# zhen6618/EPRecon

Measured on AMD Instinct MI355X. Metric: fragments_per_sec, higher is better.
Workload: dtype f32

## Files before the change

### eprecon_amd/_lib.py

```python
import ctypes
import os

import torch

_HERE = os.path.dirname(os.path.abspath(__file__))
LIB_PATH = os.environ.get("EPRECON_LIB_PATH") or os.path.join(_HERE, "libeprecon_hip.so")

_c = ctypes
_vp, _i, _i64, _f, _sz = _c.c_void_p, _c.c_int, _c.c_int64, _c.c_float, _c.c_size_t

SIGNATURES = {
    "eprecon_abi_version": (_i, []),
    "eprecon_build_arch": (_c.c_char_p, []),
    "eprecon_back_project_workspace_bytes": (_sz, [_i64, _i, _i, _i, _i, _i, _i]),
    "eprecon_back_project_async": (_i, [_vp, _i64, _vp, _i, _f, _vp, _i, _vp, _i, _i, _i, _i, _i, _i,
                                        _vp, _vp, _vp, _vp, _vp, _vp, _vp, _vp, _sz, _vp]),
    "eprecon_back_project": (_i, [_vp, _i64, _vp, _i, _f, _vp, _i, _vp, _i, _i, _i, _i, _i, _i, _i,
                                  _vp, _vp, _vp, _vp, _vp, _vp, _vp, _vp, _vp, _sz, _vp]),
    "eprecon_profile_gather_kernel": (_c.c_char_p, []),
    "eprecon_hash_capacity": (_c.c_uint32, [_i64]),
    "eprecon_hash_table_bytes": (_sz, [_c.c_uint32]),
    "eprecon_hash_build_async": (_i, [_vp, _i64, _i, _vp, _c.c_uint32, _vp]),
    "eprecon_hash_build_dn_async": (_i, [_vp, _i64, _vp, _i, _vp, _c.c_uint32, _vp]),
    "eprecon_hash_query_async": (_i, [_vp, _c.c_uint32, _vp, _i64, _i, _vp, _vp]),
    "eprecon_hash_status": (_i, [_vp, _vp]),
    "eprecon_unique_workspace_bytes": (_sz, [_i64]),
    "eprecon_unique_coords_async": (_i, [_vp, _i64, _i, _vp, _c.c_uint32, _vp, _vp, _vp, _vp, _sz, _vp]),
    "eprecon_unique_coords_dn_async": (_i, [_vp, _i64, _vp, _i, _vp, _c.c_uint32, _vp, _vp, _vp, _vp, _sz, _vp]),
    "eprecon_unique_hierarchy_dn_async": (_i, [_vp, _i64, _vp, _i, _vp, _vp, _vp, _vp, _vp, _vp, _sz, _vp]),
    "eprecon_point_quantize_dn_async": (_i, [_vp, _i64, _vp, _f, _vp, _vp, _vp]),
    "eprecon_spvcnn_points_dn_async": (_i, [_vp, _i64, _vp, _i, _i, _vp, _i, _f, _vp, _f, _vp, _vp, _vp, _vp, _vp, _vp]),
    "eprecon_gru_stage_capacity": (_i64, [_vp, _i64, _i]),
    "eprecon_gru_stage_workspace_bytes": (_sz, [_i64]),
    "eprecon_gru_stage_begin_async": (_i, [_vp, _vp]),
    "eprecon_gru_stage_commit_async": (_i, [_vp, _vp, _vp, _vp]),
    "eprecon_kernel_map_async": (_i, [_vp, _c.c_uint32, _vp, _i64, _i, _i, _vp, _vp]),
    "eprecon_kernel_map_self_async": (_i, [_vp, _c.c_uint32, _vp, _i64, _i, _vp, _vp]),
    "eprecon_transpose_map_async": (_i, [_vp, _i64, _vp, _i, _vp, _vp]),
    "eprecon_sparse_conv_async": (_i, [_vp, _i64, _i, _vp, _i, _i64, _vp, _i, _i, _vp, _vp, _i, _i, _i, _vp]),
    "eprecon_conv_bn_partial_bytes": (_sz, [_i64, _i]),
    "eprecon_sparse_conv_fused_async": (_i, [_vp, _i64, _i, _vp, _i, _i64, _vp, _i, _i, _vp, _vp, _i, _vp, _i, _i, _i,
                                             _vp, _vp]),
    "eprecon_conv_desc_async": (_i, [_vp, _vp]),
    "eprecon_exclusive_scan_async": (_i, [_vp, _i64, _vp, _vp, _vp, _vp]),
    "eprecon_conv_desc_partial_rows": (_i64, [_vp]),
    "eprecon_bn_acc_words": (_sz, [_i]),
    "eprecon_conv_desc_takes_bn_acc": (_i, [_vp]),
    "eprecon_batchnorm_acc_affine_async": (_i, [_vp, _i, _i, _i, _f, _vp, _vp, _vp]),
    "eprecon_affine_rows_acc_async": (_i, [_vp, _i64, _i, _i, _vp, _i, _i, _f, _i, _vp, _i, _vp]),
    "eprecon_affine_rows_res_async": (_i, [_vp, _i64, _i, _i, _vp, _vp, _vp, _i, _i, _vp, _i, _vp]),
    "eprecon_batchnorm_finalize_affine_async": (_i, [_vp, _i64, _i64, _i, _vp, _vp, _f, _vp, _vp, _vp]),
    "eprecon_affine_rows_async": (_i, [_vp, _i64, _i, _i, _vp, _vp, _i, _vp, _i, _vp]),
    "eprecon_pixel_map_async": (_i, [_i, _i, _i, _i, _vp, _vp]),
    "eprecon_batchnorm_apply_workspace_bytes": (_sz, [_i]),
    "eprecon_batchnorm_apply_partials_async": (_i, [_vp, _i64, _i, _i, _vp, _i64, _i64, _vp, _vp, _f, _vp, _i, _i, _vp, _i,
                                                    _vp, _vp, _vp, _sz, _vp]),
    "eprecon_batchnorm_apply_partials_res_async": (_i, [_vp, _i64, _i, _i, _vp, _i64, _i64, _vp, _vp, _f, _vp, _i, _vp, _vp, _i,
                                                        _vp, _i, _vp, _sz, _vp]),
    "eprecon_batchnorm_workspace_bytes": (_sz, [_i64, _i]),
    "eprecon_batchnorm_train_async": (_i, [_vp, _i64, _i, _i, _vp, _vp, _f, _vp, _i, _i, _vp, _i, _vp, _vp,
                                           _vp, _sz, _vp]),
    "eprecon_rowwise_layernorm_async": (_i, [_vp, _i64, _i, _i, _vp, _i, _vp, _vp, _f, _i, _i, _vp, _i, _vp]),
    "eprecon_init_select_workspace_bytes": (_sz, [_i, _i]),
    "eprecon_init_select_async": (_i, [_vp, _vp, _i64, _f, _i, _i, _i, _vp, _vp, _vp, _sz, _vp]),
    "eprecon_upsample_async": (_i, [_vp, _i, _vp, _i64, _i, _i, _vp, _vp, _vp]),
    "eprecon_aligned_coords_async": (_i, [_vp, _i64, _vp, _i, _f, _vp, _vp, _vp]),
    "eprecon_point_quantize_async": (_i, [_vp, _i64, _f, _vp, _vp, _vp]),
    "eprecon_segment_workspace_bytes": (_sz, [_i64, _i64]),
    "eprecon_segment_lists_async": (_i, [_vp, _i64, _i64, _vp, _vp, _vp, _sz, _vp]),
    "eprecon_segment_mean_async": (_i, [_vp, _i, _vp, _vp, _i64, _i, _vp, _i, _vp]),
    "eprecon_sphash_async": (_i, [_vp, _i64, _vp, _vp]),
    "eprecon_sphash_order_workspace_bytes": (_sz, [_i64]),
    "eprecon_sphash_order_async": (_i, [_vp, _i64, _vp, _vp, _vp, _sz, _vp]),
    "eprecon_remap_index_async": (_i, [_vp, _i64, _vp, _vp, _i64, _vp, _vp]),
    "eprecon_trilinear_map_async": (_i, [_vp, _c.c_uint32, _vp, _i64, _i, _vp, _vp, _vp]),
    "eprecon_devoxelize_async": (_i, [_vp, _i, _vp, _vp, _i64, _i, _vp, _i, _i, _vp]),
    "eprecon_sparse_conv_wgrad_workspace_bytes": (_sz, [_i, _i64, _i, _i]),
    "eprecon_sparse_conv_wgrad_async": (_i, [_vp, _i, _vp, _i, _vp, _i, _i64, _i, _i, _vp, _vp, _sz, _vp]),
    "eprecon_invert_map_async": (_i, [_vp, _i, _i64, _i64, _vp, _vp]),
    "eprecon_devoxelize_backward_async": (_i, [_vp, _i, _vp, _vp, _i64, _i, _i64, _vp, _i, _vp]),
    "eprecon_gather_rows_scaled_async": (_i, [_vp, _i, _vp, _vp, _i64, _i, _vp, _i, _vp]),
    "eprecon_back_project_backward_async": (_i, [_vp, _i64, _vp, _i, _f, _vp, _vp, _i, _i, _i, _i, _i, _vp, _i, _vp, _vp, _vp]),
    "eprecon_back_project_backward_workspace_bytes": (_sz, [_i, _i, _i, _i, _i]),
    "eprecon_back_project_backward_det_async": (_i, [_vp, _i64, _vp, _i, _f, _vp, _vp, _i, _i, _i, _i, _i, _vp, _i, _vp, _vp, _vp, _sz,
                                                     _vp]),
    "eprecon_devoxelize_backward_csr_async": (_i, [_vp, _i, _vp, _vp, _vp, _i64, _i, _vp, _i, _vp]),
    "eprecon_devoxelize_gate_async": (_i, [_vp, _i, _vp, _vp, _i64, _i, _vp, _i, _i, _vp, _i, _vp, _i, _vp, _i, _vp]),
    "eprecon_devoxelize_gate_tail_async": (_i, [_vp, _i, _vp, _vp, _i64, _i, _vp, _i, _i, _vp, _i, _vp, _i, _vp, _i, _vp, _i, _vp, _i,
                                                _i, _vp]),
    "eprecon_fbv_union_workspace_bytes": (_sz, [_i]),
    "eprecon_fbv_union_async": (_i, [_vp, _vp, _i64, _i, _vp, _vp, _i64, _i, _i, _i, _i, _i, _vp, _vp, _vp, _vp, _vp,
                                     _vp, _vp, _sz, _vp]),
    "eprecon_map_set_fragment": (_i, [_vp, _i]),
    "eprecon_map_stamps_async": (_i, [_vp, _vp, _vp, _i, _c.c_int32, _vp]),
    "eprecon_map_select_boundary_async": (_i, [_vp, _vp, _i, _i, _i, _vp, _vp]),
    "eprecon_map_pack_boundary_async": (_i, [_vp, _vp, _i64, _vp]),
    "eprecon_map_merge_boundary": (_i, [_vp, _vp, _i64, _vp, _i, _vp, _vp]),
    "eprecon_map_create": (_i, [_i, _c.POINTER(_vp)]),
    "eprecon_map_destroy": (_i, [_vp]),
    "eprecon_map_reset": (_i, [_vp]),
    "eprecon_map_size": (_i64, [_vp]),
    "eprecon_map_channels": (_i, [_vp]),
    "eprecon_map_export_async": (_i, [_vp, _vp, _vp, _vp]),
    "eprecon_map_import_async": (_i, [_vp, _vp, _vp, _i64, _vp]),
    "eprecon_map_crop_union": (_i, [_vp, _vp, _vp, _i64, _i, _i, _i, _i, _vp, _vp, _vp, _vp, _vp, _vp]),
    "eprecon_map_gather_async": (_i, [_vp, _vp, _i64, _i, _i, _f, _vp, _i, _vp]),
    "eprecon_map_update_async": (_i, [_vp, _vp, _i64, _vp, _i, _vp]),
    "eprecon_map_target_fuse": (_i, [_vp, _vp, _vp, _i, _vp, _vp, _i64, _vp, _vp]),
    "eprecon_gather_rows_async": (_i, [_vp, _i, _vp, _i64, _i, _f, _vp, _i, _vp]),
    "eprecon_tsdf_integrate_async": (_i, [_vp, _vp, _vp, _vp, _f, _vp, _i, _i, _i, _vp, _vp, _f, _f, _i, _vp, _vp]),
    "eprecon_marching_cubes_table": (_i, [_vp]),
    "eprecon_marching_cubes_workspace_bytes": (_sz, [_i, _i, _i]),
    "eprecon_marching_cubes_count": (_i, [_vp, _i, _i, _i, _f, _vp, _vp, _sz, _vp]),
    "eprecon_marching_cubes_emit_async": (_i, [_vp, _i, _i, _i, _f, _vp, _vp, _vp, _vp, _vp, _vp, _vp, _vp, _vp]),
    "eprecon_marching_cubes_count_masked": (_i, [_vp, _vp, _i, _i, _i, _f, _vp, _vp, _sz, _vp]),
    "eprecon_marching_cubes_emit_masked_async": (_i, [_vp, _vp, _i, _i, _i, _f, _vp, _vp, _vp, _vp, _vp, _vp, _vp, _vp, _vp]),
    "eprecon_render_depth_workspace_bytes": (_sz, [_i64]),
    "eprecon_render_depth_async": (_i, [_vp, _i64, _vp, _i64, _vp, _i, _i, _i, _f, _f, _f, _i, _vp, _i64, _vp, _sz, _vp]),
    "eprecon_depth_metrics_workspace_bytes": (_sz, [_i]),
    "eprecon_depth_metrics_async": (_i, [_vp, _vp, _i, _i64, _vp, _vp, _sz, _vp]),
    "eprecon_point_bounds_async": (_i, [_vp, _i64, _vp, _vp, _vp]),
    "eprecon_voxel_down_sample_workspace_bytes": (_sz, [_i64, _i64]),
    "eprecon_voxel_down_sample": (_i, [_vp, _i64, _vp, _c.c_double, _vp, _vp, _vp, _i64, _vp, _sz, _vp]),
    "eprecon_nn_search_workspace_bytes": (_sz, [_i64, _i64]),
    "eprecon_nn_search_async": (_i, [_vp, _i64, _vp, _i64, _vp, _c.c_double, _vp, _vp, _vp, _vp, _sz, _vp]),
    "eprecon_nearest_voxel_async": (_i, [_vp, _c.c_uint32, _vp, _i64, _vp, _i64, _i, _vp, _vp]),
    "eprecon_upsample2x_nhwc_async": (_i, [_vp, _vp, _i, _i, _i, _i, _vp]),
    "eprecon_decoder_keys_async": (_i, [_vp, _i, _vp, _i, _vp, _vp, _vp, _i64, _i, _vp, _vp, _vp]),
    "eprecon_decoder_query_side_async": (_i, [_vp, _vp]),
    "eprecon_panoptic_stats_async": (_i, [_vp, _i64, _vp, _vp, _i, _i64, _vp, _vp, _vp, _vp]),
    "eprecon_panoptic_assign_async": (_i, [_vp, _vp, _vp, _i64, _vp, _vp]),
    "eprecon_masked_attention_workspace_bytes": (_sz, [_i64, _i, _i, _i]),
    "eprecon_masked_attention_async": (_i, [_vp, _i, _i, _vp, _i, _vp, _i, _i64, _vp, _i, _vp, _i64, _i, _i, _i, _f, _vp, _vp, _sz, _vp]),
    "eprecon_profile_enable": (_i, [_i]),
    "eprecon_profile_gather_ms": (_f, []),
    "eprecon_profile_conv_arm": (_i, [_i, _i, _i, _i64]),
    "eprecon_profile_conv_ms": (_f, [_c.POINTER(_i64), _c.POINTER(_c.c_char_p)]),
    "eprecon_profile_conv_pairs": (_i64, []),
    "eprecon_mlp4x_supported": (_i, [_i, _i]),
    "eprecon_spvcnn_forward_workspace_bytes": (_sz, [_vp]),
    "eprecon_spvcnn_forward_async": (_i, [_vp, _vp]),
    "eprecon_spvcnn_geometry_workspace_bytes": (_sz, [_i64, _i64, _i64]),
    "eprecon_spvcnn_geometry_async": (_i, [_vp, _vp]),
    "eprecon_gru_stage_finish_workspace_bytes": (_sz, [_i64, _i64, _i64]),
    "eprecon_gru_stage_finish_async": (_i, [_vp, _vp]),
    "eprecon_bn2d_views_chunks": (_i, [_i64, _i]),
    "eprecon_bn2d_views_workspace_bytes": (_sz, [_i, _i64, _i]),
    "eprecon_bn2d_views_stats_async": (_i, [_vp, _i, _i64, _i, _vp, _vp, _f, _vp, _vp, _sz, _vp]),
    "eprecon_bn2d_views_apply_async": (_i, [_vp, _i, _i64, _i, _vp, _i, _vp, _vp, _vp]),
    "eprecon_dwconv2d_nhwc_async": (_i, [_vp, _i, _i, _i, _i, _vp, _i, _i, _vp, _i, _i, _vp, _vp]),
    "eprecon_mlp4x_async": (_i, [_vp, _vp]),
    "eprecon_profile_conv_executed_pairs": (_i64, []),
    "eprecon_profile_last_conv_kernel": (_c.c_char_p, []),
    "eprecon_profile_mark_async": (_i, [_i, _vp]),
    "eprecon_conv_desc_workspace_bytes": (_sz, [_vp]),
    "eprecon_sparsify_workspace_bytes": (_sz, [_i64]),
    "eprecon_sparsify_async": (_i, [_vp, _i, _f, _vp, _vp, _vp, _i, _vp, _i, _i, _i, _i64, _i, _vp, _vp, _vp, _vp, _vp, _vp, _vp,
                                    _sz, _vp]),
    "eprecon_grid_rank_async": (_i, [_vp, _i64, _i, _i, _i, _i, _vp, _vp]),
    "eprecon_conv_pack_weight_floats": (_sz, [_i, _i, _i]),
    "eprecon_conv_pack_weight_async": (_i, [_vp, _i, _i, _i, _vp, _vp]),
    "eprecon_conv_pack_weight16_floats": (_sz, [_i, _i, _i]),
    "eprecon_conv_pack_weight16_async": (_i, [_vp, _i, _i, _i, _vp, _vp]),
    "eprecon_conv_pack_many_async": (_i, [_vp, _i, _vp]),
    "eprecon_nchw_to_nhwc_async": (_i, [_vp, _vp, _i, _i, _i, _vp]),
    "eprecon_views_to_rows_async": (_i, [_vp, _vp]),
}

EPRECON_OK, EPRECON_EMPTY = 0, 1
ABI_VERSION = 1


class EpreconError(RuntimeError):
    pass


_lib = None


def load():
    global _lib
    if _lib is not None:
        return _lib
    if not os.path.exists(LIB_PATH):
        raise EpreconError(
            f"{LIB_PATH} not found: build it with `python -m eprecon_amd.build` "
            "(hipcc --offload-arch=gfx950). eprecon_amd has no CPU fallback.")
    lib = ctypes.CDLL(LIB_PATH)
    for name, (res, args) in SIGNATURES.items():
        fn = getattr(lib, name)
        fn.restype = res
        fn.argtypes = args
    if lib.eprecon_abi_version() != ABI_VERSION:
        raise EpreconError("libeprecon_hip.so ABI version mismatch; rebuild")
    _lib = lib
    return lib


def check(rc, what):
    if rc == EPRECON_OK:
        return True
    if rc == EPRECON_EMPTY:
        return False
    if rc <= -1000:
        raise EpreconError(f"{what}: HIP error {-(rc + 1000)}")
    raise EpreconError(f"{what}: error {rc} "
                       "(-1 bad argument, -2 workspace too small, -3 unsupported size)")


def ptr(t):
    return None if t is None else t.data_ptr()


_raw_stream = getattr(torch._C, "_cuda_getCurrentRawStream", None)
_raw_device = getattr(torch._C, "_cuda_getDevice", None)


def current_stream():
    if _raw_stream is not None and _raw_device is not None:
        return _raw_stream(_raw_device()) or None
    return torch.cuda.current_stream().cuda_stream or None


class ViewsDesc(ctypes.Structure):
    _fields_ = [("src", (ctypes.c_void_p * 16) * 3), ("dst", ctypes.c_void_p * 3), ("channels", ctypes.c_int32 * 3),
                ("hw", ctypes.c_int32 * 3), ("levels", ctypes.c_int32), ("n_views", ctypes.c_int32)]


class ConvDesc(ctypes.Structure):
    _fields_ = [("x", ctypes.c_void_p), ("n_in", ctypes.c_int64), ("ld_x", ctypes.c_int),
                ("nbr", ctypes.c_void_p), ("kvol", ctypes.c_int), ("n_out", ctypes.c_int64),
                ("weight", ctypes.c_void_p), ("cin", ctypes.c_int), ("cout", ctypes.c_int),
                ("bias", ctypes.c_void_p),
                ("residual", ctypes.c_void_p), ("ld_res", ctypes.c_int),
                ("out", ctypes.c_void_p), ("ld_out", ctypes.c_int),
                ("relu", ctypes.c_int), ("accumulate", ctypes.c_int),
                ("in_scale", ctypes.c_void_p), ("in_shift", ctypes.c_void_p), ("in_relu", ctypes.c_int),
                ("res_scale", ctypes.c_void_p), ("res_shift", ctypes.c_void_p), ("res_relu", ctypes.c_int),
                ("bn_partial", ctypes.c_void_p), ("bn_ld", ctypes.c_int),
                ("ln", ctypes.c_int), ("ln_gamma", ctypes.c_void_p), ("ln_beta", ctypes.c_void_p),
                ("ln_eps", ctypes.c_float), ("ln_post_relu", ctypes.c_int),
                ("img_h", ctypes.c_int), ("img_w", ctypes.c_int), ("img_maps", ctypes.c_int),
                ("vox_rank", ctypes.c_void_p), ("grid_x", ctypes.c_int), ("grid_y", ctypes.c_int), ("grid_z", ctypes.c_int),
                ("packed_weight", ctypes.c_void_p), ("packed_weight16", ctypes.c_void_p),
                ("workspace", ctypes.c_void_p), ("workspace_bytes", ctypes.c_size_t),
                ("bn_acc", ctypes.c_void_p), ("bn_acc_ld", ctypes.c_int), ("bn_acc_c0", ctypes.c_int),
                ("bn_gamma", ctypes.c_void_p), ("bn_beta", ctypes.c_void_p),
                ("in_acc", ctypes.c_void_p), ("in_acc_ld", ctypes.c_int), ("in_acc_c0", ctypes.c_int),
                ("in_eps", ctypes.c_float), ("in_affine_scratch", ctypes.c_void_p)]


class GruStageDesc(ctypes.Structure):
    _fields_ = [("map", ctypes.c_void_p), ("target_map", ctypes.c_void_p),
                ("cur_coords", ctypes.c_void_p), ("cur_feat", ctypes.c_void_p), ("n_cur", ctypes.c_int64), ("ld_cur", ctypes.c_int),
                ("dim", ctypes.c_int), ("interval", ctypes.c_int), ("activity_mode", ctypes.c_int),
                ("rel", ctypes.c_int32 * 3),
                ("tsdf_gt", ctypes.c_void_p), ("occ_gt", ctypes.c_void_p),
                ("origin", ctypes.c_void_p), ("w2ac", ctypes.c_void_p),
                ("voxel_size", ctypes.c_float), ("resolution", ctypes.c_float),
                ("ch_voxel", ctypes.c_int), ("batch_index", ctypes.c_int),
                ("capacity", ctypes.c_int64),
                ("updated", ctypes.c_void_p), ("out_coords", ctypes.c_void_p), ("r_coords", ctypes.c_void_p),
                ("hx_voxel", ctypes.c_void_p), ("hx_image", ctypes.c_void_p), ("tsdf_target", ctypes.c_void_p),
                ("scaled1", ctypes.c_void_p), ("vox1", ctypes.c_void_p), ("inverse1", ctypes.c_void_p), ("uniq1", ctypes.c_void_p),
                ("table1", ctypes.c_void_p),
                ("scaled2", ctypes.c_void_p), ("vox2", ctypes.c_void_p), ("inverse2", ctypes.c_void_p), ("uniq2", ctypes.c_void_p),
                ("table2", ctypes.c_void_p),
                ("table_capacity", ctypes.c_uint32),
                ("counts", ctypes.c_void_p),
                ("workspace", ctypes.c_void_p), ("workspace_bytes", ctypes.c_size_t)]


class DecoderLayerDesc(ctypes.Structure):
    _PTRS_A = ["o_attn", "state_in", "query_pos", "cross_out_wt", "cross_out_b", "cross_ln_g", "cross_ln_b", "self_in_wt", "self_in_b",
               "self_out_wt", "self_out_b", "self_ln_g", "self_ln_b", "ffn1_wt", "ffn1_b", "ffn2_wt", "ffn2_b", "ffn_ln_g", "ffn_ln_b",
               "dec_ln_g", "dec_ln_b", "cls_wt", "cls_b", "m1_wt", "m1_b", "m2_wt", "m2_b", "m3_wt", "m3_b", "next_q_wt", "next_q_b"]
    _PTRS_B = ["state_out", "cls_out", "mask_embed_out", "next_q_out", "workspace"]
    _fields_ = ([(n, ctypes.c_int) for n in ("n_queries", "channels", "n_heads", "ffn_dim", "n_class_logits", "mask_hidden")]
                + [(n, ctypes.c_void_p) for n in _PTRS_A] + [("ln_eps", ctypes.c_float)] + [(n, ctypes.c_void_p) for n in _PTRS_B])


class GruFinishDesc(ctypes.Structure):
    _fields_ = ([(n, ctypes.c_int64) for n in ("n", "m1", "m2")]
                + [(n, ctypes.c_void_p) for n in ("inverse1", "inverse2", "uniq1", "uniq2", "table1", "table2")]
                + [("table_capacity", ctypes.c_uint32)] + [(n, ctypes.c_void_p) for n in ("scaled1", "scaled2")]
                + [("literal", ctypes.c_int)]
                + [(n, ctypes.c_void_p) for n in ("offsets1", "order1", "offsets2", "order2", "nbr1", "nbr2", "idx8_1", "weight8_1",
                                                  "idx8_2", "weight8_2", "perm1", "rank1", "perm2", "rank2", "workspace")]
                + [("workspace_bytes", ctypes.c_size_t)])


class SpvcnnGeometryDesc(ctypes.Structure):
    _fields_ = ([(n, ctypes.c_int64) for n in ("n", "n1", "n2", "n4")]
                + [(n, ctypes.c_void_p) for n in ("scaled", "vox", "inverse1", "coords1", "coords2", "coords4", "parent2", "parent4",
                                                  "table1", "table2", "table4")]
                + [(n, ctypes.c_uint32) for n in ("capacity1", "capacity2", "capacity4")]
                + [(n, ctypes.c_void_p) for n in ("offsets1", "order1", "idx4", "offsets4", "order4", "down12", "up21", "down24", "up42",
                                                  "k1", "k2", "k4", "idx8_1", "weight8_1", "idx8_4", "weight8_4", "workspace")]
                + [("workspace_bytes", ctypes.c_size_t)])


SPVCNN_CONVS = 27


class SpvcnnConv(ctypes.Structure):
    _fields_ = [(n, ctypes.c_void_p) for n in ("weight", "packed_weight", "packed_weight16")] + [(n, ctypes.c_int) for n in ("kvol", "cin", "cout")]


class SpvcnnBn(ctypes.Structure):
    _fields_ = [("gamma", ctypes.c_void_p), ("beta", ctypes.c_void_p), ("eps", ctypes.c_float)]


class SpvcnnForwardDesc(ctypes.Structure):
    _fields_ = ([(n, ctypes.c_int64) for n in ("n", "n1", "n2", "n4")] + [("cin", ctypes.c_int), ("cs", ctypes.c_int * 5)]
                + [("feat", ctypes.c_void_p), ("ld_feat", ctypes.c_int)]
                + [(n, ctypes.c_void_p) for n in ("offsets1", "order1", "offsets4", "order4", "k1", "k2", "k4", "down12", "up21", "down24",
                                                  "up42", "idx8_1", "weight8_1", "idx8_4", "weight8_4")]
                + [("conv", SpvcnnConv * SPVCNN_CONVS), ("bn", SpvcnnBn * SPVCNN_CONVS)]
                + [("out", ctypes.c_void_p), ("ld_out", ctypes.c_int), ("workspace", ctypes.c_void_p), ("workspace_bytes", ctypes.c_size_t)])


class Mlp4xHead(ctypes.Structure):
    _fields_ = ([(n, ctypes.c_void_p) for n in ("w1", "b1", "g1", "be1", "w2", "b2", "g2", "be2", "w3", "b3", "y")]
                + [("ld_y", ctypes.c_int64)])


class Mlp4xDesc(ctypes.Structure):
    _fields_ = [("x", ctypes.c_void_p), ("ld_x", ctypes.c_int64), ("n", ctypes.c_int64), ("channels", ctypes.c_int),
                ("out_channels", ctypes.c_int), ("heads", ctypes.c_int), ("residual", ctypes.c_int), ("eps1", ctypes.c_float),
                ("eps2", ctypes.c_float), ("head", Mlp4xHead * 2)]


SIDE_PAIR, SIDE_BRANCH_A, SIDE_BRANCH_B, SIDE_PANOPTIC, SIDE_EXCHANGE, SIDE_SETUP = range(6)
_SIDE_STREAMS = {}


def side_stream(device, role):
    index = device.index if device.index is not None else torch.cuda.current_device()
    key = (index, role)
    st = _SIDE_STREAMS.get(key)
    if st is None:
        st = _SIDE_STREAMS[key] = torch.cuda.Stream(device=torch.device("cuda", index))
    return st


_WORKSPACES = {}


def workspace(nbytes, device):
    key = (device.type, device.index, current_stream())
    buf = _WORKSPACES.get(key)
    if buf is None or buf.numel() < nbytes:
        buf = torch.empty(int(nbytes * 1.25) + 4096, dtype=torch.uint8, device=device)
        _WORKSPACES[key] = buf
    return buf


_DEFERRED = []
_DEFERRED_LOCK = __import__("threading").Lock()
_DEFERRED_MAX = 64


def defer_check(dev_value, expected, what):
    item = (dev_value, int(expected), what, current_stream())
    evicted = None
    with _DEFERRED_LOCK:
        _DEFERRED.append(item)
        if len(_DEFERRED) > _DEFERRED_MAX:
            evicted = _DEFERRED.pop(0)
    if evicted is not None:
        count_host_read()
        verify_deferred([evicted], evicted[0].to(torch.int32).tolist())


def requeue_deferred(items):
    if items:
        with _DEFERRED_LOCK:
            _DEFERRED[:0] = items


def take_deferred(stream="current"):
    st = current_stream() if stream == "current" else stream
    with _DEFERRED_LOCK:
        out = [it for it in _DEFERRED if stream is None or it[3] == st]
        _DEFERRED[:] = [it for it in _DEFERRED if not (stream is None or it[3] == st)]
    return out


def verify_deferred(items, host_values):
    for (_, expected, what, *_rest), got in zip(items, host_values):
        if int(got) != expected:
            raise EpreconError(f"{what}: expected {expected}, the device reports {int(got)} (EPRECON_ERR_ARG)")


def read_counts(counts):
    count_host_read()
    pending = take_deferred()
    flat = counts.reshape(-1)
    if pending:
        host = torch.cat([flat] + [t.reshape(1).to(flat.dtype) for t, *_ in pending]).tolist()
        verify_deferred(pending, host[flat.numel():])
        return host[:flat.numel()]
# ... 49 lines not shown
```

### eprecon_amd/csrc/conv_common.hpp

```cpp
#pragma once
#include "common.hpp"

namespace epconv {

struct ConvParams {
    const float *x;
    const int32_t *nbr;
    const float *w;
    const float *bias;
    float *out;
    int n_out, K, Cin, Cout, ld_x, ld_out;
    int64_t x_bytes;
    int relu;
    int accumulate;
    const float *res;
    int ld_res;
    float *bn_partial;
    int bn_ld;
    const float *in_scale, *in_shift;
    int in_relu;
    const float *res_scale, *res_shift;
    int res_relu;
    int ln;
    const float *ln_gamma, *ln_beta;
    float ln_eps;
    int ln_post_relu;
    int img_h, img_w, img_maps;
    int flex_partial;
    const int32_t *vox_rank;
    int gx, gy, gz;
    const float *wq;
    const float *wq16;
    int debug;
    int splitk_pipe;
    void *ws;
    size_t ws_bytes;
    long long *bn_acc;
    int bn_acc_ld, bn_acc_c0;
    const float *bn_gamma, *bn_beta;
    const long long *in_acc;
    int in_acc_ld, in_acc_c0;
    float in_eps;
};

constexpr int kBnCopies = 8, kBnWords = 7;
#ifndef EP_BN_ABL
#define EP_BN_ABL 0
#endif

__device__ __forceinline__ void bn_limbs(double x, long long &l0, long long &l1, long long &l2)
{
    const double v = x * 1099511627776.0;
    const double hi = floor(v * (1.0 / 1099511627776.0));
    l0 = (long long)(v - hi * 1099511627776.0);
    const long long h = (long long)hi;
    l1 = h & ((1ll << 40) - 1);
    l2 = h >> 40;
}

__device__ __forceinline__ void bn_acc_add(long long *acc, int ld, int c, int copy, float n, float mean, float m2)
{
    if (n <= 0.0f || (EP_BN_ABL & 1)) return;
    unsigned long long *a = reinterpret_cast<unsigned long long *>(acc) + ((size_t)copy * ld + c) * kBnWords;
    const double dn = (double)n, dm = (double)mean;
    long long l0, l1, l2;
    bn_limbs(dn * dm, l0, l1, l2);
    atomicAdd(a + 0, (unsigned long long)l0);
    if (EP_BN_ABL & 4) return;
    atomicAdd(a + 1, (unsigned long long)l1); atomicAdd(a + 2, (unsigned long long)l2);
    bn_limbs((double)m2 + dn * dm * dm, l0, l1, l2);
    atomicAdd(a + 3, (unsigned long long)l0); atomicAdd(a + 4, (unsigned long long)l1); atomicAdd(a + 5, (unsigned long long)l2);
    atomicAdd(a + 6, (unsigned long long)(long long)n);
}

__device__ __forceinline__ void bn_acc_affine(const long long *acc, int ld, int c, float eps, float &scale, float &shift)
{
    if (EP_BN_ABL & 2) { scale = 1.0f; shift = 0.0f; return; }
    long long w[kBnWords] = {0, 0, 0, 0, 0, 0, 0};
#pragma unroll 1
    for (int k = 0; k < kBnCopies; ++k) {
        const long long *a = acc + ((size_t)k * ld + c) * kBnWords;
#pragma unroll
        for (int j = 0; j < kBnWords; ++j) w[j] += a[j];
    }
    const double two40 = 1099511627776.0;
    const double s1 = ((double)w[2] * two40 + (double)w[1]) + (double)w[0] * (1.0 / two40);
    const double s2 = ((double)w[5] * two40 + (double)w[4]) + (double)w[3] * (1.0 / two40);
    const double n = (double)w[6];
    const float *gb = reinterpret_cast<const float *>(acc + (size_t)kBnCopies * ld * kBnWords);
    const double mean = n > 0.0 ? s1 / n : 0.0;
    double var = n > 0.0 ? s2 / n - mean * mean : 0.0;
    if (var < 0.0) var = 0.0;
    const float sc = gb[c] / sqrtf((float)var + eps);
    scale = sc;
    shift = gb[ld + c] - (float)mean * sc;
}

template <int THREADS, bool ACC = true>
__device__ __forceinline__ void stage_in_affine(const ConvParams &p, float *sAff, int cpad, int tid)
{
    if (!p.in_scale) return;
    for (int c = tid; c < cpad; c += THREADS) {
        float sc = 0.0f, sh = 0.0f;
        if (c < p.Cin) {
            if (ACC && p.in_acc) bn_acc_affine(p.in_acc, p.in_acc_ld, p.in_acc_c0 + c, p.in_eps, sc, sh);
            else { sc = p.in_scale[c]; sh = p.in_shift[c]; }
        }
        sAff[c] = sc;
        sAff[cpad + c] = sh;
    }
}

__device__ __forceinline__ void bn_acc_publish(const ConvParams &p, int col, int copy, bool first, float n, float mean, float m2)
{
    bn_acc_add(p.bn_acc, p.bn_acc_ld, p.bn_acc_c0 + col, copy & (kBnCopies - 1), n, mean, m2);
    if (first) {
        float *gb = reinterpret_cast<float *>(p.bn_acc + (size_t)kBnCopies * p.bn_acc_ld * kBnWords);
        gb[p.bn_acc_c0 + col] = p.bn_gamma ? p.bn_gamma[col] : 1.0f;
        gb[p.bn_acc_ld + p.bn_acc_c0 + col] = p.bn_beta ? p.bn_beta[col] : 0.0f;
    }
}

constexpr int kWaves = 4;
typedef float f32x4 __attribute__((ext_vector_type(4)));
typedef unsigned int u32x4 __attribute__((ext_vector_type(4)));

__device__ __forceinline__ void chan_merge(float &n_a, float &mean_a, float &m2_a, float n_b, float mean_b, float m2_b)
{
    if (n_b == 0.0f) return;
    if (n_a == 0.0f) {
        n_a = n_b; mean_a = mean_b; m2_a = m2_b;
        return;
    }
    const float n = n_a + n_b;
    const float d = mean_b - mean_a;
    mean_a = mean_a + d * (n_b / n);
    m2_a = m2_a + m2_b + d * d * (n_a * n_b / n);
    n_a = n;
}

__device__ __forceinline__ void bn_partial_store(const ConvParams &p, int row, int col, float n, float mean, float m2)
{
    const size_t plane = (size_t)p.Cout * p.bn_ld;
    float *dst = p.bn_partial + (size_t)col * p.bn_ld + row;
    dst[0] = n; dst[plane] = mean; dst[2 * plane] = m2;
}

template <int CT, bool ACC = false, int NW = kWaves>
__device__ __forceinline__ void tile16_epilogue(const ConvParams &p, const f32x4 (&acc)[CT], const int (&orow)[4], float *sStat,
                                                int partial_row)
{
    const int tid = threadIdx.x;
    const int lane = tid & 63, wave = tid >> 6;
    const int l16 = lane & 15, q = lane >> 4;
    float v[CT][4];
    bool colok[CT];
#pragma unroll
    for (int t = 0; t < CT; ++t) {
        const int col = 16 * t + l16;
        colok[t] = col < p.Cout;
        const float b = (p.bias && colok[t]) ? p.bias[col] : 0.0f;
        const float rs = (p.res_scale && colok[t]) ? p.res_scale[col] : 1.0f;
        const float rb = (p.res_scale && colok[t]) ? p.res_shift[col] : 0.0f;
#pragma unroll
        for (int j = 0; j < 4; ++j) {
            float val = 0.0f;
            if (colok[t] && orow[j] >= 0) {
                val = acc[t][j] + b;
                if (p.relu) val = fmaxf(val, 0.0f);
                if (p.res) {
                    float rv = p.res[(size_t)orow[j] * p.ld_res + col];
                    if (p.res_scale) {
                        rv = fmaf(rv, rs, rb);
                        if (p.res_relu) rv = fmaxf(rv, 0.0f);
                    }
                    val += rv;
                }
            }
            v[t][j] = val;
        }
    }
    if (p.ln) {
        const float inv_c = 1.0f / (float)p.Cout;
#pragma unroll
        for (int j = 0; j < 4; ++j) {
            float sum = 0.0f;
#pragma unroll
            for (int t = 0; t < CT; ++t) sum += v[t][j];
#pragma unroll
            for (int m = 8; m > 0; m >>= 1) sum += __shfl_xor(sum, m);
            const float mean = sum * inv_c;
            float sq = 0.0f;
#pragma unroll
            for (int t = 0; t < CT; ++t) {
                const float d = colok[t] ? v[t][j] - mean : 0.0f;
                v[t][j] = d;
                sq = fmaf(d, d, sq);
            }
#pragma unroll
            for (int m = 8; m > 0; m >>= 1) sq += __shfl_xor(sq, m);
            const float inv = 1.0f / sqrtf(sq * inv_c + p.ln_eps);
#pragma unroll
            for (int t = 0; t < CT; ++t) {
                const int col = 16 * t + l16;
                float y = fmaf(v[t][j] * inv, (p.ln_gamma && colok[t]) ? p.ln_gamma[col] : 1.0f, (p.ln_beta && colok[t]) ? p.ln_beta[col] : 0.0f);
                if (p.ln_post_relu) y = fmaxf(y, 0.0f);
                v[t][j] = y;
            }
        }
    }
#pragma unroll
    for (int t = 0; t < CT; ++t)
#pragma unroll
        for (int j = 0; j < 4; ++j)
            if (colok[t] && orow[j] >= 0) p.out[(size_t)orow[j] * p.ld_out + 16 * t + l16] = v[t][j];
    if (p.bn_partial || (ACC && p.bn_acc)) {
#pragma unroll
        for (int t = 0; t < CT; ++t) {
            float n = 0.0f, sum = 0.0f;
#pragma unroll
            for (int j = 0; j < 4; ++j)
                if (orow[j] >= 0) { n += 1.0f; sum += v[t][j]; }
            float mean = n > 0.0f ? sum / n : 0.0f, m2 = 0.0f;
#pragma unroll
            for (int j = 0; j < 4; ++j)
                if (orow[j] >= 0) { const float d = v[t][j] - mean; m2 = fmaf(d, d, m2); }
#pragma unroll
            for (int m = 16; m < 64; m <<= 1) {
                const float on = __shfl_xor(n, m), om = __shfl_xor(mean, m), oq = __shfl_xor(m2, m);
                const bool lower = (lane & m) == 0;
                float a_n = lower ? n : on, a_mean = lower ? mean : om, a_m2 = lower ? m2 : oq;
                chan_merge(a_n, a_mean, a_m2, lower ? on : n, lower ? om : mean, lower ? oq : m2);
                n = a_n; mean = a_mean; m2 = a_m2;
            }
            if (q == 0) {
                float *d = sStat + (wave * 3) * 16 * CT + 16 * t + l16;
                d[0] = n; d[16 * CT] = mean; d[2 * 16 * CT] = m2;
            }
        }
        __syncthreads();
        if (tid < 16 * CT && tid < p.Cout) {
            float a_n = 0.0f, a_mean = 0.0f, a_m2 = 0.0f;
#pragma unroll
            for (int w = 0; w < NW; ++w)
                chan_merge(a_n, a_mean, a_m2, sStat[(w * 3) * 16 * CT + tid], sStat[(w * 3 + 1) * 16 * CT + tid], sStat[(w * 3 + 2) * 16 * CT + tid]);
            if (p.bn_partial) bn_partial_store(p, partial_row, tid, a_n, a_mean, a_m2);
            if (ACC && p.bn_acc) bn_acc_publish(p, tid, partial_row, partial_row == 0, a_n, a_mean, a_m2);
        }
    }
}

bool direct16_ok(const ConvParams &p);
constexpr int kDirectRows = 128;
int launch_direct16(const ConvParams &p, hipStream_t st);
int direct16_partial_block_rows(const ConvParams &p);

constexpr int kT2MinRows = 40000;
bool tile2d16_ok(const ConvParams &p);
int64_t tile2d16_partial_rows(const ConvParams &p);
int launch_tile2d16(const ConvParams &p, hipStream_t st);

constexpr int kT2ShortMaxRows = 20000;
bool tile2d_short_list(const ConvParams &p);
bool tile2d_short_ok(const ConvParams &p);
int64_t tile2d_short_partial_rows(const ConvParams &p);
int launch_tile2d_short(const ConvParams &p, hipStream_t st);


}
```

### eprecon_amd/csrc/grid_ops.hip

```cpp
#include "common.hpp"

namespace {
using namespace ep;

constexpr int kSelThreads = 1024;

__global__ __launch_bounds__(256) void init_mark_kernel(const float *logit, const int4 *coords, int n, float thr,
                                                        int batch, int D, int cell, unsigned char *marks)
{
    const int i = blockIdx.x * 256 + threadIdx.x;
    if (i >= n) return;
    const int4 c = coords[i];
    if (c.x < 0 || c.x >= batch) return;
    const float sig = 1.0f / (1.0f + expf(-logit[i]));
    if (sig > thr) {
        const int x = c.y / cell, y = c.z / cell, z = c.w / cell;
        if (x >= 0 && x < D && y >= 0 && y < D && z >= 0 && z < D) marks[(size_t)c.x * D * D * D + (x * D + y) * D + z] = 1;
    }
}

__device__ __forceinline__ uint32_t box_columns(const uint32_t *vol, int D, int x, int y, bool erode, uint32_t zmask)
{
    uint32_t r = erode ? zmask : 0u;
    for (int dx = -1; dx <= 1; ++dx)
// ... 36 lines not shown
#pragma unroll
        for (int d = 1; d < kWave; d <<= 1) {
            const int t = __shfl_up(s, d);
            if (lane >= d) s += t;
        }
        if (lane == kWave - 1) sWave[wid] = s;
        __syncthreads();
        int off = written + s - mine, tot = 0;
        for (int k = 0; k < kSelThreads / kWave; ++k) {
            const int c = sWave[k];
            if (k < wid) off += c;
            tot += c;
        }
        uint32_t bits = fin;
        while (bits) {
            const int z = __ffs(bits) - 1;
            bits &= bits - 1;
            out_coords[off++] = make_int4(b, x * out_scale, y * out_scale, z * out_scale);
        }
        if (tid == 0) n_out_dev[1 + b] = tot;
        written += tot;
        __syncthreads();
    }
    if (tid == 0) n_out_dev[0] = written;
}

__global__ __launch_bounds__(256) void upsample_coords_kernel(const int4 *coords, int n, int interval,
                                                              int4 *up)
{
    const int e = blockIdx.x * 256 + threadIdx.x;
    if (e >= n * 8) return;
    const int i = e >> 3, k = e & 7;
    const int dx = (0xB2 >> k) & 1;
    const int dy = (0xD4 >> k) & 1;
    const int dz = (0xE8 >> k) & 1;
    int4 c = coords[i];
    c.y += dx * interval;
    c.z += dy * interval;
    c.w += dz * interval;
    up[e] = c;
}

__global__ __launch_bounds__(256) void upsample_feat_kernel(const float *feat, int n, int C, int ld,
                                                            float *up)
{
    const size_t e = (size_t)blockIdx.x * 256 + threadIdx.x;
    const size_t total = (size_t)n * 8 * C;
    if (e >= total) return;
    const int c = (int)(e % C);
    const size_t row = e / C;
    up[e] = feat[(row >> 3) * ld + c];
}

}

extern "C" {

size_t eprecon_init_select_workspace_bytes(int batch, int dim)
{
    return align_up((size_t)batch * dim * dim * dim, 256);
}

int eprecon_init_select_async(const float *logit, const int32_t *coords, int64_t n, float threshold,
                              int batch, int dim, int cell, int32_t *out_coords, int32_t *n_out_dev,
                              void *workspace, size_t workspace_bytes, void *stream)
{
    if (n < 0 || batch <= 0 || dim <= 0 || dim > 32 || cell <= 0 || !out_coords || !n_out_dev || !workspace ||
        (n > 0 && (!logit || !coords)))
        return EPRECON_ERR_ARG;
    if (workspace_bytes < eprecon_init_select_workspace_bytes(batch, dim)) return EPRECON_ERR_WORKSPACE;
    hipStream_t st = (hipStream_t)stream;
    const int cells = dim * dim * dim;
    unsigned char *marks = reinterpret_cast<unsigned char *>(workspace);
    EP_HIP_CHECK(hipMemsetAsync(marks, 0, (size_t)batch * cells, st));
    if (n > 0) {
        hipLaunchKernelGGL(init_mark_kernel, dim3((unsigned)ceil_div(n, 256)), dim3(256), 0, st, logit,
                           reinterpret_cast<const int4 *>(coords), (int)n, threshold, batch, dim, cell, marks);
        EP_LAUNCH_CHECK();
    }
    hipLaunchKernelGGL(init_select_kernel, dim3(1), dim3(kSelThreads), 0, st, (const unsigned char *)marks, batch,
                       dim, cell, reinterpret_cast<int4 *>(out_coords), n_out_dev);
    EP_LAUNCH_CHECK();
    return EPRECON_OK;
}

int eprecon_upsample_async(const float *feat, int ld_feat, const int32_t *coords, int64_t n, int channels,
                           int interval, float *up_feat, int32_t *up_coords, void *stream)
{
    if (n < 0 || channels < 0 || interval <= 0 || (n > 0 && (!coords || (!up_coords && channels == 0)))) return EPRECON_ERR_ARG;
    if (n == 0) return EPRECON_OK;
    hipStream_t st = (hipStream_t)stream;
    if (up_coords) {
        hipLaunchKernelGGL(upsample_coords_kernel, dim3((unsigned)ceil_div(n * 8, 256)), dim3(256), 0, st,
                           reinterpret_cast<const int4 *>(coords), (int)n, interval,
                           reinterpret_cast<int4 *>(up_coords));
        EP_LAUNCH_CHECK();
    }
    if (channels > 0) {
        if (!feat || !up_feat || ld_feat < channels) return EPRECON_ERR_ARG;
        const size_t total = (size_t)n * 8 * channels;
        hipLaunchKernelGGL(upsample_feat_kernel, dim3((unsigned)ceil_div((int64_t)total, 256)), dim3(256), 0,
                           st, feat, (int)n, channels, ld_feat, up_feat);
        EP_LAUNCH_CHECK();
    }
    return EPRECON_OK;
}

}

namespace {
__global__ __launch_bounds__(256) void upsample2x_nhwc_kernel(const float4 *in, float4 *out, int n, int h, int w,
                                                              int c4)
{
    const size_t e = (size_t)blockIdx.x * 256 + threadIdx.x;
    const size_t total = (size_t)n * 4 * h * w * c4;
    if (e >= total) return;
    const int c = (int)(e % c4);
    size_t r = e / c4;
    const int ox = (int)(r % (2 * w));
    r /= 2 * w;
    const int oy = (int)(r % (2 * h));
    const int img = (int)(r / (2 * h));
    const float sx = fmaxf(((float)ox + 0.5f) * 0.5f - 0.5f, 0.0f);
    const float sy = fmaxf(((float)oy + 0.5f) * 0.5f - 0.5f, 0.0f);
    const int x0 = (int)sx, y0 = (int)sy;
    const int x1 = min(x0 + 1, w - 1), y1 = min(y0 + 1, h - 1);
    const float lx = sx - (float)x0, ly = sy - (float)y0;
    const float4 *base = in + (size_t)img * h * w * c4;
    const float4 a = base[((size_t)y0 * w + x0) * c4 + c], b = base[((size_t)y0 * w + x1) * c4 + c];
    const float4 d = base[((size_t)y1 * w + x0) * c4 + c], f = base[((size_t)y1 * w + x1) * c4 + c];
    const float w00 = (1.0f - ly) * (1.0f - lx), w01 = (1.0f - ly) * lx, w10 = ly * (1.0f - lx), w11 = ly * lx;
    float4 o;
    o.x = w00 * a.x + w01 * b.x + w10 * d.x + w11 * f.x;
    o.y = w00 * a.y + w01 * b.y + w10 * d.y + w11 * f.y;
    o.z = w00 * a.z + w01 * b.z + w10 * d.z + w11 * f.z;
    o.w = w00 * a.w + w01 * b.w + w10 * d.w + w11 * f.w;
    out[e] = o;
}
}

extern "C" int eprecon_upsample2x_nhwc_async(const float *in, float *out, int n, int h, int w, int channels,
                                             void *stream)
{
    if (!in || !out || n <= 0 || h <= 0 || w <= 0 || channels <= 0 || channels % 4) return EPRECON_ERR_ARG;
    const size_t total = (size_t)n * 4 * h * w * (channels / 4);
    hipLaunchKernelGGL(upsample2x_nhwc_kernel, dim3((unsigned)ceil_div((int64_t)total, 256)), dim3(256), 0,
                       (hipStream_t)stream, reinterpret_cast<const float4 *>(in), reinterpret_cast<float4 *>(out), n, h,
                       w, channels / 4);
    EP_LAUNCH_CHECK();
    return EPRECON_OK;
}

namespace {
constexpr int kSpTile = 256;
constexpr int kSpMaxBatch = 32;

__global__ __launch_bounds__(kSpTile) void sparsify_count_kernel(const float *occ, int ld_occ, float thr, const unsigned char *tgt,
                                                                const int4 *coords, int n, int batch, int *tile_tot, int *counts)
{
    const int row = blockIdx.x * kSpTile + threadIdx.x;
    const bool keep = row < n && occ[(size_t)row * ld_occ] > thr;
    const unsigned long long m = __ballot(keep);
    __shared__ int sTot[kSpTile / 64];
    __shared__ int sCnt[2 * kSpMaxBatch];
    if (threadIdx.x < 2 * kSpMaxBatch) sCnt[threadIdx.x] = 0;
    if ((threadIdx.x & 63) == 0) sTot[threadIdx.x >> 6] = __popcll(m);
    __syncthreads();
    const int b = keep ? coords[row].x : -1;
    const bool t = keep && (!tgt || tgt[row]);
    for (int bb = 0; bb < batch; ++bb) {
        const unsigned long long mb = __ballot(b == bb), mt = __ballot(b == bb && t);
        if ((threadIdx.x & 63) == 0 && mb) {
            atomicAdd(&sCnt[bb], __popcll(mb));
            if (mt) atomicAdd(&sCnt[kSpMaxBatch + bb], __popcll(mt));
        }
    }
    __syncthreads();
    if (threadIdx.x < batch) {
        if (sCnt[threadIdx.x]) atomicAdd(counts + 1 + threadIdx.x, sCnt[threadIdx.x]);
        if (sCnt[kSpMaxBatch + threadIdx.x]) atomicAdd(counts + 1 + batch + threadIdx.x, sCnt[kSpMaxBatch + threadIdx.x]);
    }
    if (threadIdx.x == 0) tile_tot[blockIdx.x] = sTot[0] + sTot[1] + sTot[2] + sTot[3];
}

__global__ __launch_bounds__(1024) void sparsify_scan_kernel(int *tile_tot, int ntiles, int *counts)
{
    __shared__ int sWave[16];
    __shared__ int sCarry;
    const int tid = threadIdx.x, lane = tid & 63, wave = tid >> 6;
    if (tid == 0) sCarry = 0;
    __syncthreads();
    for (int base = 0; base < ntiles; base += 1024) {
        const int i = base + tid;
        const int v = i < ntiles ? tile_tot[i] : 0;
        int incl = v;
#pragma unroll
        for (int d = 1; d < 64; d <<= 1) {
            const int o = __shfl_up(incl, d);
            if (lane >= d) incl += o;
        }
        if (lane == 63) sWave[wave] = incl;
        __syncthreads();
        int woff = 0;
        for (int w = 0; w < wave; ++w) woff += sWave[w];
        const int carry = sCarry;
        if (i < ntiles) tile_tot[i] = carry + woff + incl - v;
        __syncthreads();
        if (tid == 1023) sCarry = carry + woff + incl;
        __syncthreads();
    }
    if (tid == 0) counts[0] = sCarry;
}

__global__ __launch_bounds__(kSpTile) void sparsify_compact_kernel(const float *occ, int ld_occ, float thr, const int4 *coords,
                                                                  const float *tsdf, int ld_tsdf, const float *feat, int ld_feat,
                                                                  int c_all, int c_feat, int n, const int *tile_off, int4 *out_coords,
                                                                  float *out_tsdf, float *out_occ, float *out_all, float *out_feat)
{
    const int row = blockIdx.x * kSpTile + threadIdx.x;
    const int lane = threadIdx.x & 63, wave = threadIdx.x >> 6;
    const float o = row < n ? occ[(size_t)row * ld_occ] : 0.0f;
    const bool keep = row < n && o > thr;
    const unsigned long long m = __ballot(keep);
    __shared__ int sTot[kSpTile / 64];
    if (lane == 0) sTot[wave] = __popcll(m);
    __syncthreads();
    int base = tile_off[blockIdx.x];
    for (int w = 0; w < wave; ++w) base += sTot[w];
    const int dst = base + __popcll(m & ((1ull << lane) - 1ull));
    const float t = keep ? tsdf[(size_t)row * ld_tsdf] : 0.0f;
    if (keep) {
        out_coords[dst] = coords[row];
        out_tsdf[dst] = t;
        out_occ[dst] = o;
        out_feat[(size_t)dst * (c_feat + 2) + c_feat] = t;
        out_feat[(size_t)dst * (c_feat + 2) + c_feat + 1] = o;
    }
    unsigned long long rest = m;
    while (rest) {
        const int l = __ffsll((long long)rest) - 1;
        rest &= rest - 1;
        const int src = blockIdx.x * kSpTile + wave * 64 + l;
        const int d = __shfl(dst, l);
        for (int c = lane; c < c_all; c += 64) {
            const float v = feat[(size_t)src * ld_feat + c];
            out_all[(size_t)d * c_all + c] = v;
            if (c < c_feat) out_feat[(size_t)d * (c_feat + 2) + c] = v;
        }
    }
}
}

extern "C" size_t eprecon_sparsify_workspace_bytes(int64_t n)
{
    return align_up((size_t)(ceil_div(n > 0 ? n : 1, (int64_t)kSpTile) + 1) * sizeof(int), 256);
}

extern "C" int eprecon_sparsify_async(const float *occ, int ld_occ, float threshold, const unsigned char *target,
                                      const int32_t *coords, const float *tsdf, int ld_tsdf, const float *feat_all, int ld_feat,
                                      int c_all, int c_feat, int64_t n, int batch, int32_t *out_coords, float *out_tsdf,
                                      float *out_occ, float *out_all, float *out_feat, int32_t *counts, void *workspace,
                                      size_t workspace_bytes, void *stream)
{
    if (n < 0 || n > 0x7fffffff || batch <= 0 || batch > kSpMaxBatch || c_all <= 0 || c_feat < 0 || c_feat > c_all || ld_occ < 1 || ld_tsdf < 1 ||
        ld_feat < c_all || !counts || !workspace || (n > 0 && (!occ || !coords || !tsdf || !feat_all || !out_coords || !out_tsdf ||
                                                               !out_occ || !out_all || !out_feat)))
        return EPRECON_ERR_ARG;
    if (workspace_bytes < eprecon_sparsify_workspace_bytes(n)) return EPRECON_ERR_WORKSPACE;
    hipStream_t st = (hipStream_t)stream;
    EP_HIP_CHECK(hipMemsetAsync(counts, 0, (size_t)(1 + 2 * batch) * sizeof(int32_t), st));
    if (n == 0) return EPRECON_OK;
    int *tile_tot = reinterpret_cast<int *>(workspace);
    const int ntiles = (int)ceil_div(n, (int64_t)kSpTile);
    hipLaunchKernelGGL(sparsify_count_kernel, dim3(ntiles), dim3(kSpTile), 0, st, occ, ld_occ, threshold, target,
                       reinterpret_cast<const int4 *>(coords), (int)n, batch, tile_tot, counts);
    EP_LAUNCH_CHECK();
    hipLaunchKernelGGL(sparsify_scan_kernel, dim3(1), dim3(1024), 0, st, tile_tot, ntiles, counts);
    EP_LAUNCH_CHECK();
    hipLaunchKernelGGL(sparsify_compact_kernel, dim3(ntiles), dim3(kSpTile), 0, st, occ, ld_occ, threshold,
                       reinterpret_cast<const int4 *>(coords), tsdf, ld_tsdf, feat_all, ld_feat, c_all, c_feat, (int)n,
                       (const int *)tile_tot, reinterpret_cast<int4 *>(out_coords), out_tsdf, out_occ, out_all, out_feat);
    EP_LAUNCH_CHECK();
    return EPRECON_OK;
}
```

### eprecon_amd/csrc/sparse_conv.hip

```cpp
#include <stdio.h>
#include <stdlib.h>
#include <string.h>

#include "common.hpp"
#include "conv_common.hpp"

namespace {
using namespace ep;
using namespace epconv;

typedef float f32x16 __attribute__((ext_vector_type(16)));


template <int TN>
__device__ __forceinline__ void stage_weights(float *dst, const float *w, int row0, int row_end, int stride,
                                              int ncols, int rows, int tid)
{
    const int total = rows * TN;
    if (stride == TN && ncols >= TN && (reinterpret_cast<uintptr_t>(w) & 15) == 0) {
        const float4 *src = reinterpret_cast<const float4 *>(w + (size_t)row0 * stride);
        float4 *d4 = reinterpret_cast<float4 *>(dst);
        const int valid4 = max(0, min(rows, row_end - row0)) * (TN / 4);
#pragma unroll 4
        for (int e = tid; e < total / 4; e += 256) d4[e] = e < valid4 ? src[min(e, max(valid4 - 1, 0))] : make_float4(0.f, 0.f, 0.f, 0.f);
// ... 1725 lines not shown
    }
    conv_epilogue<1>(p, acc, LinearRows{(int)blockIdx.x * kWideRows + wave * 32, p.n_out}, 32 * t, r32, half, wave, sStat,
                     (int)blockIdx.x, (int)gridDim.y);
}

size_t wide_workspace_bytes(const ConvParams &p)
{
    const int ntt = (p.Cout + 31) / 32;
    return (size_t)wide_splits(p.n_out) * (size_t)ceil_div(p.n_out, kWideRows) * kWaves * ntt * 1024 * sizeof(float);
}

bool wide_shape_ok(const ConvParams &p)
{
    const char *e = getenv("EPRECON_CONV_WIDEK");
    if (e && e[0] == '0') return false;
    if (p.K != 27 || !p.nbr || !p.wq || (reinterpret_cast<uintptr_t>(p.wq) & 15) != 0) return false;
    if (p.Cin < 96 || p.Cin % 4 != 0 || p.Cout <= 64 || p.Cout > 128) return false;
    if (p.ld_x % 4 != 0 || (reinterpret_cast<uintptr_t>(p.x) & 15) != 0) return false;
    if (p.in_scale && ((reinterpret_cast<uintptr_t>(p.in_scale) & 15) != 0 || (reinterpret_cast<uintptr_t>(p.in_shift) & 15) != 0))
        return false;
    if (p.accumulate || p.ln) return false;
    return p.n_out >= 4096 && p.n_out <= 40000;
}
bool wide_ok(const ConvParams &p) { return wide_shape_ok(p) && p.ws && p.ws_bytes >= wide_workspace_bytes(p); }

template <int NTT>
int launch_wide_t(const ConvParams &p, hipStream_t st)
{
    const int nsplit = wide_splits(p.n_out);
    const int blocks = (int)ceil_div(p.n_out, kWideRows);
    const int kmax = (p.K + nsplit - 1) / nsplit + 1;
    const size_t lds = (size_t)2 * kWideSlabF4 * sizeof(float4) + (size_t)kmax * kWideRows * sizeof(int) +
                       (size_t)2 * ((p.Cin + 3) & ~3) * sizeof(float) + 16;
    float *partial = reinterpret_cast<float *>(p.ws);
    hipLaunchKernelGGL((spconv_wide_kernel<NTT>), dim3((unsigned)blocks, (unsigned)nsplit), dim3(256), lds, st, p, nsplit, partial);
    EP_LAUNCH_CHECK();
    const size_t lds2 = (size_t)max(kWaves * 3 * 32 * NTT, 3 * 256) * sizeof(float);
    hipLaunchKernelGGL((spconv_wide_reduce_kernel<NTT>), dim3((unsigned)blocks, (unsigned)NTT), dim3(256), lds2, st, p, nsplit, (const float *)partial);
    EP_LAUNCH_CHECK();
    return EPRECON_OK;
}
int launch_wide(const ConvParams &p, hipStream_t st) { return (p.Cout + 31) / 32 == 3 ? launch_wide_t<3>(p, st) : launch_wide_t<4>(p, st); }

bool splitk_ok(const ConvParams &p)
{
    const char *e = getenv("EPRECON_CONV_SPLITK");
    if ((e && e[0] == '0') || p.accumulate) return false;
    if (p.bn_partial && !p.flex_partial) return false;
    const int nt_full = (p.Cout + 31) / 32;
    if (p.ln && nt_full > 1) return false;
    const int cin_pad = (p.Cin + 7) / 8 * 8;
    const int64_t wg128 = ceil_div(p.n_out, kRowsPerBlock) * nt_full;
    const int stages = p.K * ((p.Cin + 31) / 32);
    constexpr int max_wg = 256, narrow_wg = 256;
    if (cin_pad <= 64) return wg128 <= narrow_wg && stages >= 8;
    return wg128 <= max_wg && stages >= 8;
}

struct ConvProf {
    bool armed = false, recorded = false;
    int K = 0, cin = 0, cout = 0;
    int64_t min_rows = 0, rows = 0;
    const char *kernel = "";
    hipEvent_t start = nullptr, stop = nullptr;
    unsigned long long *pairs_dev = nullptr;
} g_conv_prof;

__global__ void count_map_pairs_kernel(const int32_t *nbr, size_t total, unsigned long long *out)
{
    unsigned long long c = 0;
    for (size_t e = (size_t)blockIdx.x * blockDim.x + threadIdx.x; e < total; e += (size_t)gridDim.x * blockDim.x) c += nbr[e] >= 0;
    for (int m = 32; m > 0; m >>= 1) c += __shfl_xor(c, m);
    if ((threadIdx.x & 63) == 0 && c) atomicAdd(out, c);
}
__global__ void count_grid_pairs_kernel(const int32_t *rank, int gx, int gy, int gz, unsigned long long *out)
{
    unsigned long long c = 0;
    const int total = gx * gy * gz;
    for (int e = blockIdx.x * blockDim.x + threadIdx.x; e < total; e += gridDim.x * blockDim.x) {
        if (rank[e] < 0) continue;
        const int z = e % gz, y = (e / gz) % gy, x = e / (gz * gy);
        for (int k = 0; k < 27; ++k) {
            const int xx = x + k % 3 - 1, yy = y + (k / 3) % 3 - 1, zz = z + k / 9 - 1;
            if (xx >= 0 && xx < gx && yy >= 0 && yy < gy && zz >= 0 && zz < gz) c += rank[(xx * gy + yy) * gz + zz] >= 0;
        }
    }
    for (int m = 32; m > 0; m >>= 1) c += __shfl_xor(c, m);
    if ((threadIdx.x & 63) == 0 && c) atomicAdd(out, c);
}
__global__ void count_map_groups_kernel(const int32_t *nbr, int n, int K, unsigned long long *out)
{
    const int groups = (n + 31) / 32;
    unsigned long long c = 0;
    for (int e = blockIdx.x * blockDim.x + threadIdx.x; e < K * groups; e += gridDim.x * blockDim.x) {
        const int k = e / groups, g = e - k * groups;
        const int rows = min(32, n - 32 * g);
        bool any = false;
        for (int i = 0; i < rows; ++i) any |= nbr[(size_t)k * n + 32 * g + i] >= 0;
        if (any) c += rows;
    }
    for (int m = 32; m > 0; m >>= 1) c += __shfl_xor(c, m);
    if ((threadIdx.x & 63) == 0 && c) atomicAdd(out, c);
}
const char *g_last_conv_kernel = "";

int conv_dispatch_inner(ConvParams &p, int64_t n_in, hipStream_t st);

int conv_dispatch(ConvParams &p, int64_t n_in, hipStream_t st)
{
    ConvProf &g = g_conv_prof;
    const bool hit = g.armed && p.K == g.K && p.Cin == g.cin && p.Cout == g.cout && p.n_out >= g.min_rows;
    static FILE *const layer_log = getenv("EPRECON_CONV_LOG") ? fopen(getenv("EPRECON_CONV_LOG"), "a") : nullptr;
    if (layer_log) {
        const int rc = conv_dispatch_inner(p, n_in, st);
        fprintf(layer_log, "%d %d %d %d %s ln=%d stats=%d acc=%d\n", p.n_out, p.K, p.Cin, p.Cout, g_last_conv_kernel, p.ln ? 1 : 0,
                p.bn_partial ? 1 : 0, p.accumulate ? 1 : 0);
        fflush(layer_log);
        return rc;
    }
    if (!hit) return conv_dispatch_inner(p, n_in, st);
    EP_HIP_CHECK(hipEventRecord(g.start, st));
    const int rc = conv_dispatch_inner(p, n_in, st);
    EP_HIP_CHECK(hipEventRecord(g.stop, st));
    g.armed = false;
    g.recorded = rc == EPRECON_OK;
    g.rows = p.n_out;
    g.kernel = g_last_conv_kernel;
    if (g.pairs_dev) {
        EP_HIP_CHECK(hipMemsetAsync(g.pairs_dev, 0, 2 * sizeof(unsigned long long), st));
        bool narrow;
        if (conv3d_tile_ok(p, &narrow))
            hipLaunchKernelGGL(count_grid_pairs_kernel, dim3(256), dim3(256), 0, st, p.vox_rank, p.gx, p.gy, p.gz, g.pairs_dev);
        else if (p.nbr) {
            hipLaunchKernelGGL(count_map_pairs_kernel, dim3(256), dim3(256), 0, st, p.nbr, (size_t)p.K * p.n_out, g.pairs_dev);
            if (!strcmp(g.kernel, "spconv_direct16_kernel"))
                hipLaunchKernelGGL(count_map_groups_kernel, dim3(256), dim3(256), 0, st, p.nbr, p.n_out, p.K, g.pairs_dev + 1);
        } else
            EP_HIP_CHECK(hipMemcpyAsync(g.pairs_dev, &g.rows, sizeof(unsigned long long), hipMemcpyHostToDevice, st));
        EP_LAUNCH_CHECK();
    }
    return rc;
}

int conv_dispatch_inner(ConvParams &p, int64_t n_in, hipStream_t st)
{
    {
        const int kind = conv3d_kind(p);
        if (kind != kD3None) {
            g_last_conv_kernel = kind == kD3Narrow ? "conv3d_tile_narrow_kernel" : "conv3d_tile16_kernel";
            return kind == kD3Tile16 ? launch_conv3d_16(p, st) : launch_conv3d_single_column(p, st);
        }
        if (!p.nbr && p.K != 1) return EPRECON_ERR_ARG;
    }
    if (tile2d16_ok(p)) {
        g_last_conv_kernel = "conv2d_tile16_kernel";
        return launch_tile2d16(p, st);
    }
    if (tile2d_short_ok(p)) {
        g_last_conv_kernel = "conv2d_tile_short_kernel";
        return launch_tile2d_short(p, st);
    }
    const bool direct2d = p.K == 9 && direct16_ok(p) && !tile2d_short_list(p);
    if (!direct2d) {
        int nt, nch;
        int64_t blocks;
        if (conv2d_tile_ok(p, &nt, &nch, &blocks)) {
            g_last_conv_kernel = "conv2d_tile_kernel";
            switch (nch) {
                case 1: return launch_conv2d_tile<1>(p, st);
                case 2: return launch_conv2d_tile<2>(p, st);
                case 3: return launch_conv2d_tile<3>(p, st);
                case 4: return launch_conv2d_tile<4>(p, st);
                default: return launch_conv2d_tile<5>(p, st);
            }
        }
    }
    const bool vec4 = (p.ld_x % 4 == 0) && ((reinterpret_cast<uintptr_t>(p.x) & 15) == 0) &&
                      (p.Cin % 4 == 0 || p.ld_x >= ((p.Cin + 3) & ~3));
    const int nblk = (int)ceil_div(p.n_out, kRowsPerBlock);
    const int nt_full = (p.Cout + 31) / 32;
    if (p.ln && (nt_full > 4 || p.bn_partial || p.accumulate)) return EPRECON_ERR_UNSUPPORTED;
    if (wide_ok(p)) {
        g_last_conv_kernel = "spconv_wide_kernel";
        return launch_wide(p, st);
    }
    if (!direct2d && splitk_ok(p)) {
        g_last_conv_kernel = "spconv_splitk_kernel";
        return vec4 ? launch_splitk_v<true>(p, st) : launch_splitk_v<false>(p, st);
    }
    if (direct16_ok(p) && !tile2d_short_list(p)) {
        g_last_conv_kernel = "spconv_direct16_kernel";
        return launch_direct16(p, st);
    }
    const bool split = nblk < 256 && nt_full > 1 && !p.ln;
    const int cin_pad = (p.Cin + 7) / 8 * 8;
    if (cin_pad <= 64 && (p.Cout <= 64 || split)) {
        g_last_conv_kernel = "spconv_resident_kernel";
        return (nt_full == 1 || split) ? launch_resident<1>(p, vec4, cin_pad, st) : launch_resident<2>(p, vec4, cin_pad, st);
    }
    if (cin_pad > 64 && vec4 && (p.K == 27 || p.K == 8) && !(p.ln && nt_full > 2)) {
        g_last_conv_kernel = "spconv_resident_kernel(wide)";
        const bool two = nt_full >= 2 && (p.ln || (int64_t)nblk * ((nt_full + 1) / 2) >= 256);
        return two ? launch_resident<2>(p, vec4, cin_pad, st) : launch_resident<1>(p, vec4, cin_pad, st);
    }
    g_last_conv_kernel = "spconv_mfma_kernel";
    if (nt_full == 1 || split) return launch_conv<1>(p, vec4, st);
    if (nt_full == 2) return launch_conv<2>(p, vec4, st);
    if (nt_full == 3) return launch_conv<3>(p, vec4, st);
    return launch_conv<4>(p, vec4, st);
}

}

__global__ void profile_mark_kernel() {}
extern "C" int eprecon_profile_mark_async(int id, void *stream)
{
    hipStream_t st = static_cast<hipStream_t>(stream);
    hipLaunchKernelGGL(profile_mark_kernel, dim3((unsigned)id + 1), dim3(64), 0, st);
    EP_LAUNCH_CHECK();
    return EPRECON_OK;
}

extern "C" int eprecon_profile_conv_arm(int kvol, int cin, int cout, int64_t min_rows)
{
    ConvProf &g = g_conv_prof;
    if (!g.start) {
        EP_HIP_CHECK(hipEventCreate(&g.start));
        EP_HIP_CHECK(hipEventCreate(&g.stop));
        EP_HIP_CHECK(hipMalloc(&g.pairs_dev, 2 * sizeof(unsigned long long)));
    }
    g.K = kvol; g.cin = cin; g.cout = cout; g.min_rows = min_rows;
    g.armed = true;
    g.recorded = false;
    return EPRECON_OK;
}

extern "C" float eprecon_profile_conv_ms(int64_t *rows_out, const char **kernel_out)
{
    ConvProf &g = g_conv_prof;
    if (!g.recorded || hipEventSynchronize(g.stop) != hipSuccess) return -1.0f;
    float ms = -1.0f;
    if (hipEventElapsedTime(&ms, g.start, g.stop) != hipSuccess) return -1.0f;
    if (rows_out) *rows_out = g.rows;
    if (kernel_out) *kernel_out = g.kernel;
    return ms;
}

extern "C" const char *eprecon_profile_last_conv_kernel(void) { return g_last_conv_kernel; }

extern "C" int64_t eprecon_profile_conv_pairs(void)
{
    ConvProf &g = g_conv_prof;
    if (!g.recorded || !g.pairs_dev || hipEventSynchronize(g.stop) != hipSuccess) return -1;
    unsigned long long v = 0;
    if (hipMemcpy(&v, g.pairs_dev, sizeof(v), hipMemcpyDeviceToHost) != hipSuccess) return -1;
    return (int64_t)v;
}

extern "C" int64_t eprecon_profile_conv_executed_pairs(void)
{
    ConvProf &g = g_conv_prof;
    if (!g.recorded || !g.pairs_dev || hipEventSynchronize(g.stop) != hipSuccess) return -1;
    unsigned long long v = 0;
    if (hipMemcpy(&v, g.pairs_dev + 1, sizeof(v), hipMemcpyDeviceToHost) != hipSuccess) return -1;
    return (int64_t)v;
}

extern "C" size_t eprecon_conv_pack_weight_floats(int kvol, int cin, int cout)
{
    if (kvol <= 0 || cin <= 0 || cout <= 0) return 0;
    int nt, ncb;
    d3_columns(cout, &nt, &ncb);
    return (size_t)ncb * kvol * ((cin + 7) / 8) * 2 * nt * 32 * 4;
}

extern "C" int eprecon_conv_pack_weight_async(const float *weight, int kvol, int cin, int cout, float *packed, void *stream)
{
    if (!weight || !packed || kvol <= 0 || cin <= 0 || cout <= 0) return EPRECON_ERR_ARG;
    int nt, ncb;
    d3_columns(cout, &nt, &ncb);
    const size_t total = eprecon_conv_pack_weight_floats(kvol, cin, cout);
    hipLaunchKernelGGL(pack_weights_kernel, dim3((unsigned)min((size_t)1024, (total + 255) / 256)), dim3(256), 0, (hipStream_t)stream,
                       weight, kvol, cin, cout, (cin + 7) / 8, nt, ncb, packed);
    EP_LAUNCH_CHECK();
    return EPRECON_OK;
}

extern "C" size_t eprecon_conv_pack_weight16_floats(int kvol, int cin, int cout)
{
    if (kvol <= 0 || cin <= 0 || cout <= 0 || cout > 80) return 0;
    const int rem = cout - 16 * ((cout + 15) / 16 - 1);
    return (size_t)kvol * ((cin + 15) / 16) * ((cout + 15) / 16) * 256 + (rem <= 8 ? (size_t)kvol * ((cin + 15) / 16) * 128 : 0);
}

extern "C" int eprecon_conv_pack_weight16_async(const float *weight, int kvol, int cin, int cout, float *packed, void *stream)
{
    if (!weight || !packed || kvol <= 0 || cin <= 0 || cout <= 0 || cout > 80) return EPRECON_ERR_ARG;
    const size_t total = eprecon_conv_pack_weight16_floats(kvol, cin, cout);
    hipLaunchKernelGGL(pack_weights16_kernel, dim3((unsigned)min((size_t)1024, (total + 255) / 256)), dim3(256), 0, (hipStream_t)stream,
                       weight, kvol, cin, cout, (cin + 15) / 16, (cout + 15) / 16, packed);
    EP_LAUNCH_CHECK();
    return EPRECON_OK;
}

extern "C" int eprecon_conv_pack_many_async(const eprecon_pack_job *jobs_dev, int njobs, void *stream)
{
    if (njobs < 0 || (njobs > 0 && !jobs_dev) || njobs > 65535) return EPRECON_ERR_ARG;
    if (njobs == 0) return EPRECON_OK;
    hipLaunchKernelGGL(pack_many_kernel, dim3(32, (unsigned)njobs), dim3(256), 0, (hipStream_t)stream, jobs_dev);
    EP_LAUNCH_CHECK();
    return EPRECON_OK;
}

extern "C" size_t eprecon_conv_bn_partial_bytes(int64_t n_out, int cout)
{
    return (size_t)ep::ceil_div(n_out > 0 ? n_out : 1, (int64_t)128) * 3 * (size_t)(cout > 0 ? cout : 1) * sizeof(float);
}

static int conv_check_and_run(ConvParams &p, int64_t n_in, int64_t n_out, void *stream)
{
    if (!p.x || !p.w || !p.out || n_in < 0 || n_out < 0 || p.K <= 0 || p.K > 64 || p.Cin <= 0 || p.Cout <= 0 ||
        p.ld_x < p.Cin || p.ld_out < p.Cout || (p.res && p.ld_res < p.Cout))
        return EPRECON_ERR_ARG;
    if (!p.nbr && !p.vox_rank && p.K != 1) return EPRECON_ERR_ARG;
    if (!p.nbr && n_in != n_out) return EPRECON_ERR_ARG;
    if ((p.in_scale == nullptr) != (p.in_shift == nullptr) || (p.res_scale == nullptr) != (p.res_shift == nullptr))
        return EPRECON_ERR_ARG;
    if (p.Cout > 4096 || n_out > 0x7fffffff) return EPRECON_ERR_UNSUPPORTED;
    if (n_out == 0) return EPRECON_OK;
    p.n_out = (int)n_out;
    p.x_bytes = n_in > 0 ? ((n_in - 1) * (int64_t)p.ld_x + ((p.Cin + 3) & ~3)) * 4 : 0;
    return conv_dispatch(p, n_in, (hipStream_t)stream);
}

static void params_from_desc(ConvParams &p, const eprecon_conv_desc *d)
{
    p.x = d->x; p.nbr = d->nbr; p.w = d->weight; p.bias = d->bias; p.out = d->out;
    p.K = d->kvol; p.Cin = d->cin; p.Cout = d->cout; p.ld_x = d->ld_x; p.ld_out = d->ld_out;
    p.relu = d->relu; p.accumulate = d->accumulate;
    p.res = d->residual; p.ld_res = d->ld_res; p.bn_partial = d->bn_partial; p.bn_ld = d->bn_ld;
    p.in_scale = d->in_scale; p.in_shift = d->in_shift; p.in_relu = d->in_relu;
    p.res_scale = d->res_scale; p.res_shift = d->res_shift; p.res_relu = d->res_relu;
    p.ln = d->ln; p.ln_gamma = d->ln_gamma; p.ln_beta = d->ln_beta; p.ln_eps = d->ln_eps;
    p.ln_post_relu = d->ln_post_relu;
    p.img_h = d->img_h; p.img_w = d->img_w; p.img_maps = d->img_maps;
    p.vox_rank = d->vox_rank; p.gx = d->grid_x; p.gy = d->grid_y; p.gz = d->grid_z; p.wq = d->packed_weight;
    p.wq16 = d->packed_weight16;
    p.ws = d->workspace; p.ws_bytes = d->workspace_bytes;
    p.flex_partial = 1;
    p.bn_acc = d->bn_acc; p.bn_acc_ld = d->bn_acc_ld; p.bn_acc_c0 = d->bn_acc_c0; p.bn_gamma = d->bn_gamma; p.bn_beta = d->bn_beta;
    p.in_acc = d->in_acc; p.in_acc_ld = d->in_acc_ld; p.in_acc_c0 = d->in_acc_c0; p.in_eps = d->in_eps;
}

extern "C" int eprecon_batchnorm_acc_affine_async(const long long *acc, int acc_ld, int acc_c0, int channels, float eps,
                                                  float *scale_out, float *shift_out, void *stream);

static bool bn_acc_family(const ConvParams &p) { return conv3d_kind(p) == 0; }

extern "C" size_t eprecon_bn_acc_words(int ld)
{
    return ld > 0 ? (size_t)epconv::kBnCopies * ld * epconv::kBnWords + (size_t)(2 * ld + 1) / 2 : 0;
}

extern "C" int eprecon_conv_desc_takes_bn_acc(const eprecon_conv_desc *d)
{
    if (!d || d->n_out <= 0) return 0;
    ConvParams p = {};
    params_from_desc(p, d);
    p.n_out = (int)d->n_out;
    return !p.ln && !p.accumulate && bn_acc_family(p) ? 1 : 0;
}

extern "C" int64_t eprecon_conv_desc_partial_rows(const eprecon_conv_desc *d);

extern "C" int eprecon_conv_desc_async(const eprecon_conv_desc *d, void *stream)
{
    if (!d) return EPRECON_ERR_ARG;
    ConvParams p = {};
    params_from_desc(p, d);
    p.n_out = (int)(d->n_out > 0 && d->n_out <= 0x7fffffff ? d->n_out : 0);
    if (p.bn_partial) {
        const int64_t rows = eprecon_conv_desc_partial_rows(d);
        if (p.bn_ld == 0) p.bn_ld = (int)(rows > 0 ? rows : 1);
        if (p.bn_ld < rows) return EPRECON_ERR_ARG;
    }
    if (p.bn_acc && (p.bn_acc_ld <= 0 || p.bn_acc_c0 < 0 || p.bn_acc_c0 + p.Cout > p.bn_acc_ld || p.ln || p.accumulate || !bn_acc_family(p)))
        return EPRECON_ERR_ARG;
    if (p.in_acc) {
        if (p.in_scale || p.in_shift || p.in_acc_ld <= 0 || p.in_acc_c0 < 0 || p.in_acc_c0 + p.Cin > p.in_acc_ld) return EPRECON_ERR_ARG;
        if (bn_acc_family(p)) {
            p.in_scale = p.in_shift = reinterpret_cast<const float *>(p.in_acc);
        } else {
            if (!d->in_affine_scratch) return EPRECON_ERR_ARG;
            const int rc = eprecon_batchnorm_acc_affine_async(p.in_acc, p.in_acc_ld, p.in_acc_c0, p.Cin, p.in_eps, d->in_affine_scratch,
                                                              d->in_affine_scratch + p.Cin, stream);
            if (rc != EPRECON_OK) return rc;
            p.in_scale = d->in_affine_scratch;
            p.in_shift = d->in_affine_scratch + p.Cin;
            p.in_acc = nullptr;
        }
    }
    return conv_check_and_run(p, d->n_in, d->n_out, stream);
}

extern "C" size_t eprecon_conv_desc_workspace_bytes(const eprecon_conv_desc *d)
{
    if (!d || d->n_out <= 0 || d->n_out > 0x7fffffff) return 0;
    ConvParams p = {};
    params_from_desc(p, d);
    p.n_out = (int)d->n_out;
    return wide_shape_ok(p) ? wide_workspace_bytes(p) : 0;
}

extern "C" int64_t eprecon_conv_desc_partial_rows(const eprecon_conv_desc *d)
{
    if (!d || d->n_out <= 0) return 0;
    ConvParams p = {};
    params_from_desc(p, d);
    p.n_out = (int)d->n_out;
    int nt, nch;
    int64_t blocks;
    if (const int kind = conv3d_kind(p)) return d3_tiles_kind(p, kind);
    p.x_bytes = d->n_in > 0 ? ((d->n_in - 1) * (int64_t)p.ld_x + ((p.Cin + 3) & ~3)) * 4 : 0;
    if (tile2d16_ok(p)) return tile2d16_partial_rows(p);
    if (tile2d_short_ok(p)) return tile2d_short_partial_rows(p);
    if (p.K == 9 && direct16_ok(p) && !tile2d_short_list(p)) return ep::ceil_div(d->n_out, (int64_t)direct16_partial_block_rows(p));
    if (conv2d_tile_ok(p, &nt, &nch, &blocks)) return blocks;
    if (wide_ok(p)) return ep::ceil_div(d->n_out, (int64_t)kWideRows);
    if (splitk_ok(p)) return ep::ceil_div(d->n_out, (int64_t)32);
    if (direct16_ok(p) && !tile2d_short_list(p)) return ep::ceil_div(d->n_out, (int64_t)direct16_partial_block_rows(p));
    return ep::ceil_div(d->n_out, (int64_t)kRowsPerBlock);
}

extern "C" int eprecon_sparse_conv_fused_async(const float *x, int64_t n_in, int ld_x, const int32_t *nbr,
                                               int kvol, int64_t n_out, const float *weight, int cin,
                                               int cout, const float *bias, const float *residual,
                                               int ld_res, float *out, int ld_out, int relu,
                                               int accumulate, float *bn_partial, void *stream)
{
    ConvParams p = {};
    p.x = x; p.nbr = nbr; p.w = weight; p.bias = bias; p.out = out;
    p.K = kvol; p.Cin = cin; p.Cout = cout; p.ld_x = ld_x; p.ld_out = ld_out;
    p.relu = relu; p.accumulate = accumulate;
    p.res = residual; p.ld_res = ld_res; p.bn_partial = bn_partial;
    p.bn_ld = (int)ep::ceil_div(n_out > 0 ? n_out : 1, (int64_t)kRowsPerBlock);
    return conv_check_and_run(p, n_in, n_out, stream);
}

extern "C" int eprecon_sparse_conv_async(const float *x, int64_t n_in, int ld_x, const int32_t *nbr,
                                         int kvol, int64_t n_out, const float *weight, int cin,
                                         int cout, const float *bias, float *out, int ld_out,
                                         int relu, int accumulate, void *stream)
{
    return eprecon_sparse_conv_fused_async(x, n_in, ld_x, nbr, kvol, n_out, weight, cin, cout, bias, nullptr, 0,
                                           out, ld_out, relu, accumulate, nullptr, stream);
}
```

### eprecon_amd/csrc/sparse_conv_direct_impl.hpp

```cpp
#pragma once
#include <stdlib.h>

#include <atomic>
#include <type_traits>

#include "common.hpp"
#include "conv_common.hpp"

namespace epconv {
namespace {
using namespace ep;

constexpr int kRT = 2;

#ifndef EP_DIRECT_ABL
#define EP_DIRECT_ABL 0
#endif

__device__ __forceinline__ float relu_nc(float x)
{
    float r;
    asm("v_max_f32 %0, 0, %1" : "=v"(r) : "v"(x));
    return r;
}
__device__ __forceinline__ float relu_sel(float x, unsigned mask)
{
    const unsigned r = __float_as_uint(relu_nc(x)), b = __float_as_uint(x);
    return __uint_as_float((r & mask) | (b & ~mask));
}

typedef __bf16 bf16x8 __attribute__((ext_vector_type(8)));
typedef __bf16 bf16x2 __attribute__((ext_vector_type(2)));
typedef short s16x4 __attribute__((ext_vector_type(4)));
typedef float f32x2 __attribute__((ext_vector_type(2)));
struct BfQuad { unsigned hi[2], lo[2]; };
__device__ __forceinline__ BfQuad bf_split(const float4 &v)
{
    const unsigned b0 = __float_as_uint(v.x), b1 = __float_as_uint(v.y), b2 = __float_as_uint(v.z), b3 = __float_as_uint(v.w);
    BfQuad r;
    r.hi[0] = __builtin_amdgcn_perm(b1, b0, 0x07060302u);
    r.hi[1] = __builtin_amdgcn_perm(b3, b2, 0x07060302u);
    const f32x2 r01 = {v.x - __uint_as_float(b0 & 0xffff0000u), v.y - __uint_as_float(b1 & 0xffff0000u)};
    const f32x2 r23 = {v.z - __uint_as_float(b2 & 0xffff0000u), v.w - __uint_as_float(b3 & 0xffff0000u)};
    r.lo[0] = __builtin_bit_cast(unsigned, __builtin_convertvector(r01, bf16x2));
    r.lo[1] = __builtin_bit_cast(unsigned, __builtin_convertvector(r23, bf16x2));
    return r;
}
__device__ __forceinline__ f32x4 bf_mfma32(const unsigned (&a0)[2], const unsigned (&a1)[2], const unsigned (&b0)[2],
                                           const unsigned (&b1)[2], f32x4 acc)
{
    union { bf16x8 v; unsigned u[4]; } a, b;
    a.u[0] = a0[0]; a.u[1] = a0[1]; a.u[2] = a1[0]; a.u[3] = a1[1];
    b.u[0] = b0[0]; b.u[1] = b0[1]; b.u[2] = b1[0]; b.u[3] = b1[1];
    return __builtin_amdgcn_mfma_f32_16x16x32_bf16(a.v, b.v, acc, 0, 0, 0);
}
__device__ __forceinline__ f32x4 bf_mfma16(const unsigned (&a0)[2], const unsigned (&b0)[2], f32x4 acc)
{
    union { s16x4 v; unsigned u[2]; } a, b;
    a.u[0] = a0[0]; a.u[1] = a0[1];
    b.u[0] = b0[0]; b.u[1] = b0[1];
    return __builtin_amdgcn_mfma_f32_16x16x16bf16_1k(a.v, b.v, acc, 0, 0, 0);
}

template <int CT, bool PERWAVE = false>
__device__ __forceinline__ void direct_epilogue(const ConvParams &p, f32x4 (&acc)[kRT][CT], int row0, float *sStat, int block = 0)
{
    constexpr int RT = kRT, NR = 4 * kRT;
    const int tid = threadIdx.x;
    const int lane = tid & 63, wave = PERWAVE ? 0 : tid >> 6;
    const int l16 = lane & 15, q = lane >> 4;
    int orow[NR];
#pragma unroll
    for (int rt = 0; rt < RT; ++rt)
#pragma unroll
        for (int j = 0; j < 4; ++j) {
            const int row = row0 + wave * 16 * RT + 16 * rt + 4 * q + j;
            orow[4 * rt + j] = row < p.n_out ? row : -1;
        }
    float v[CT][NR];
    bool colok[CT];
#pragma unroll
    for (int t = 0; t < CT; ++t) {
        const int col = 16 * t + l16;
        colok[t] = col < p.Cout;
        const float b = (p.bias && colok[t]) ? p.bias[col] : 0.0f;
        const float rs = (p.res_scale && colok[t]) ? p.res_scale[col] : 1.0f;
        const float rb = (p.res_scale && colok[t]) ? p.res_shift[col] : 0.0f;
#pragma unroll
        for (int r = 0; r < NR; ++r) {
            float val = 0.0f;
            if (colok[t] && orow[r] >= 0) {
                val = acc[r >> 2][t][r & 3] + b;
                if (p.relu) val = fmaxf(val, 0.0f);
                if (p.res) {
                    float rv = p.res[(size_t)orow[r] * p.ld_res + col];
                    if (p.res_scale) {
                        rv = fmaf(rv, rs, rb);
                        if (p.res_relu) rv = fmaxf(rv, 0.0f);
                    }
                    val += rv;
                }
            }
            v[t][r] = val;
        }
    }
    if (p.ln) {
        const float inv_c = 1.0f / (float)p.Cout;
#pragma unroll
        for (int r = 0; r < NR; ++r) {
            float sum = 0.0f;
#pragma unroll
            for (int t = 0; t < CT; ++t) sum += v[t][r];
#pragma unroll
            for (int m = 8; m > 0; m >>= 1) sum += __shfl_xor(sum, m);
            const float mean = sum * inv_c;
            float sq = 0.0f;
#pragma unroll
            for (int t = 0; t < CT; ++t) {
                const float d = colok[t] ? v[t][r] - mean : 0.0f;
                v[t][r] = d;
                sq = fmaf(d, d, sq);
            }
#pragma unroll
            for (int m = 8; m > 0; m >>= 1) sq += __shfl_xor(sq, m);
            const float inv = 1.0f / sqrtf(sq * inv_c + p.ln_eps);
#pragma unroll
            for (int t = 0; t < CT; ++t) {
                const int col = 16 * t + l16;
                float y = fmaf(v[t][r] * inv, (p.ln_gamma && colok[t]) ? p.ln_gamma[col] : 1.0f, (p.ln_beta && colok[t]) ? p.ln_beta[col] : 0.0f);
                if (p.ln_post_relu) y = fmaxf(y, 0.0f);
                v[t][r] = y;
            }
        }
    }
#pragma unroll
    for (int t = 0; t < CT; ++t)
#pragma unroll
        for (int r = 0; r < NR; ++r)
            if (colok[t] && orow[r] >= 0) p.out[(size_t)orow[r] * p.ld_out + 16 * t + l16] = v[t][r];
    if (p.bn_partial || p.bn_acc) {
#pragma unroll
        for (int t = 0; t < CT; ++t) {
            float n = 0.0f, sum = 0.0f;
#pragma unroll
            for (int r = 0; r < NR; ++r)
                if (orow[r] >= 0) { n += 1.0f; sum += v[t][r]; }
            float mean = n > 0.0f ? sum / n : 0.0f, m2 = 0.0f;
#pragma unroll
            for (int r = 0; r < NR; ++r)
                if (orow[r] >= 0) { const float d = v[t][r] - mean; m2 = fmaf(d, d, m2); }
#pragma unroll
            for (int m = 16; m < 64; m <<= 1) {
                const float on = __shfl_xor(n, m), om = __shfl_xor(mean, m), oq = __shfl_xor(m2, m);
                const bool lower = (lane & m) == 0;
                float a_n = lower ? n : on, a_mean = lower ? mean : om, a_m2 = lower ? m2 : oq;
                chan_merge(a_n, a_mean, a_m2, lower ? on : n, lower ? om : mean, lower ? oq : m2);
                n = a_n; mean = a_mean; m2 = a_m2;
            }
            if constexpr (PERWAVE) {
                if (q == 0 && colok[t]) {
                    if (p.bn_partial) bn_partial_store(p, block, 16 * t + l16, n, mean, m2);
                    if (p.bn_acc) bn_acc_publish(p, 16 * t + l16, block, block == 0, n, mean, m2);
                }
                continue;
            }
            if (q == 0) {
                float *d = sStat + (wave * 3) * 16 * CT + 16 * t + l16;
                d[0] = n; d[16 * CT] = mean; d[2 * 16 * CT] = m2;
            }
        }
        if constexpr (PERWAVE) return;
        __syncthreads();
        if (tid < 16 * CT && tid < p.Cout) {
            float a_n = 0.0f, a_mean = 0.0f, a_m2 = 0.0f;
#pragma unroll
            for (int w = 0; w < kWaves; ++w)
                chan_merge(a_n, a_mean, a_m2, sStat[(w * 3) * 16 * CT + tid], sStat[(w * 3 + 1) * 16 * CT + tid], sStat[(w * 3 + 2) * 16 * CT + tid]);
            if (p.bn_partial) bn_partial_store(p, (int)blockIdx.x, tid, a_n, a_mean, a_m2);
            if (p.bn_acc) bn_acc_publish(p, tid, (int)blockIdx.x, blockIdx.x == 0, a_n, a_mean, a_m2);
        }
    }
}
// ... 923 lines not shown
```

### eprecon_amd/dense2d.py

```python
import ctypes
import os

import torch

from . import _lib
from . import sparse as SP


class PixelGrid:
    _cache = {}

    def __init__(self, maps, height, width, device):
        self.maps, self.height, self.width, self.device = maps, height, width, device
        self.n = maps * height * width
        self._nbr = {}

    @classmethod
    def get(cls, maps, height, width, device):
        key = (maps, height, width, str(device))
        g = cls._cache.get(key)
        if g is None:
            g = cls._cache[key] = cls(maps, height, width, device)
        return g

    def kernel_map(self, ksize):
        if ksize == 1:
            return None
        nbr = self._nbr.get(ksize)
        if nbr is None:
            nbr = torch.empty((ksize * ksize, self.n), dtype=torch.int32, device=self.device)
            _lib.check(_lib.load().eprecon_pixel_map_async(self.maps, self.height, self.width, ksize,
                                                           _lib.ptr(nbr), _lib.current_stream()),
                       "eprecon_pixel_map_async")
            self._nbr[ksize] = nbr
        return nbr


def rows_of(x):
    v, c, h, w = x.shape
    return x.permute(0, 2, 3, 1).reshape(v * h * w, c)


def maps_of(rows, maps, height, width):
    return rows.view(maps, height, width, rows.shape[1]).permute(0, 3, 1, 2)


def packed_weight(conv):
    w = conv.weight
    tag = (w._version, w.data_ptr(), w.device)
    cached = getattr(conv, "_eprecon_packed", None)
    if cached is None or cached[0] != tag:
        co, ci, kh, kw = w.shape
        assert kh == kw and kh % 2 == 1 and conv.stride == (1, 1) and conv.dilation == (1, 1) and conv.groups == 1
        cached = (tag, w.detach().permute(2, 3, 1, 0).reshape(kh * kw, ci, co).contiguous())
        conv._eprecon_packed = cached
    return cached[1]


DIRECT_2D_MIN_ROWS = 40000
K1_DIRECT_2D_MIN_ROWS = 20000
SHORT_2D_MAX_ROWS = 20000
SHORT_2D_MAX_COUT = 80


BN_ACC = os.environ.get("EPRECON_BN_ACC", "0") == "1"


class BnArena:

    def __init__(self, device, words=1 << 19):
        self.buf = torch.zeros(words, dtype=torch.int64, device=device)
        self.offset = 0
        self.high = words

    def begin(self):
        if self.high:
            self.buf[:self.high].zero_()
        self.offset = 0
        self.high = 0

    def take(self, words):
        words = (words + 1) & ~1
        if self.offset + words > self.buf.numel():
            raise _lib.EpreconError("BatchNorm accumulator arena exhausted (eprecon_amd.dense2d.BnArena)")
        t = self.buf[self.offset:self.offset + words]
        self.offset += words
        self.high = max(self.high, self.offset)
        return t


_ARENA = None


class bn_pass:

    def __init__(self, arena):
        self.arena = arena

    def __enter__(self):
        global _ARENA
        self.prev, _ARENA = _ARENA, self.arena
        if self.arena is not None:
            self.arena.begin()
        return self.arena

    def __exit__(self, *exc):
        global _ARENA
        _ARENA = self.prev
        return False


class AccSlice:
    __slots__ = ("block", "ld", "c0", "c")

    def __init__(self, block, ld, c0, c):
        self.block, self.ld, self.c0, self.c = block, ld, c0, c

    @classmethod
    def new(cls, channels):
        words = int(_lib.load().eprecon_bn_acc_words(channels))
        return cls(_ARENA.take(words), channels, 0, channels)

    def part(self, a, b):
        return AccSlice(self.block, self.ld, self.c0 + a, b - a)


class Act:
    __slots__ = ("rows", "scale", "shift", "relu", "acc", "eps")

    def __init__(self, rows, scale=None, shift=None, relu=False, acc=None, eps=1e-5):
        self.rows, self.scale, self.shift, self.relu, self.acc, self.eps = rows, scale, shift, relu, acc, eps

    def affine(self):
        if self.acc is not None and self.scale is None:
            a = torch.empty((2, self.acc.c), dtype=torch.float32, device=self.rows.device)
            _lib.check(_lib.load().eprecon_batchnorm_acc_affine_async(
                self.acc.block.data_ptr(), self.acc.ld, self.acc.c0, self.acc.c, float(self.eps), a[0].data_ptr(), a[1].data_ptr(),
                _lib.current_stream()), "eprecon_batchnorm_acc_affine_async")
            self.scale, self.shift = a[0], a[1]
        return self.scale, self.shift


def _dptr(t):
    return None if t is None else t.data_ptr()


def conv_bn_act(conv, bn, x, grid, out=None, aff=None, relu=True, pre_relu=False, residual=None):
    return conv_bn_launch(packed_weight(conv), conv.bias, bn.weight, bn.bias, bn.eps, conv.kernel_size[0], x, grid,
                          out=out, aff=aff, relu=relu, pre_relu=pre_relu, residual=residual)


def conv_bn_launch(w, bias, gamma, beta, eps, k, x, grid, out=None, aff=None, relu=True, pre_relu=False,
                   residual=None):
    lib = _lib.load()
    kvol, cin, cout = w.shape
    rows = x.rows
    n = rows.shape[0]
    dev = rows.device
    assert rows.shape[1] == cin and rows.dtype == torch.float32 and rows.stride(1) == 1
    nbr = grid.kernel_map(k)
    if out is None:
        out = torch.empty((n, cout), dtype=torch.float32, device=dev)
    d = _lib.ConvDesc()
    d.x, d.n_in, d.ld_x = rows.data_ptr(), n, rows.stride(0)
    d.nbr, d.kvol, d.n_out = _dptr(nbr), kvol, n
    d.weight, d.cin, d.cout = w.data_ptr(), cin, cout
    d.bias = _dptr(bias)
    if residual is not None:
        assert residual.rows.shape == (n, cout)
        d.residual, d.ld_res = residual.rows.data_ptr(), residual.rows.stride(0)
        r_scale, r_shift = residual.affine()
        d.res_scale, d.res_shift, d.res_relu = _dptr(r_scale), _dptr(r_shift), int(residual.relu)
    d.out, d.ld_out = out.data_ptr(), out.stride(0)
    d.relu, d.accumulate = int(pre_relu), 0
    if x.acc is not None and x.scale is None:
        assert x.acc.c == cin
        d.in_acc, d.in_acc_ld, d.in_acc_c0, d.in_eps = x.acc.block.data_ptr(), x.acc.ld, x.acc.c0, float(x.eps)
    else:
        d.in_scale, d.in_shift = _dptr(x.scale), _dptr(x.shift)
    d.in_relu = int(x.relu)
    if k == 3:
        d.img_h, d.img_w, d.img_maps = grid.height, grid.width, grid.maps
        if n < DIRECT_2D_MIN_ROWS:
            pq = SP.packed_weight(w)
            d.packed_weight = pq.data_ptr()
            if n < SHORT_2D_MAX_ROWS and cout <= SHORT_2D_MAX_COUT:
                d.packed_weight16 = SP.packed_weight16(w).data_ptr()
        if cout <= SP.DIRECT_MAX_COUT and n >= DIRECT_2D_MIN_ROWS:
            pw = SP.packed_weight16(w)
            d.packed_weight16 = pw.data_ptr()
    elif k == 1 and cout <= SP.DIRECT_MAX_COUT and n >= K1_DIRECT_2D_MIN_ROWS:
        pw = SP.packed_weight16(w)
        d.packed_weight16 = pw.data_ptr()
    if _ARENA is not None and (aff is None or isinstance(aff, AccSlice)) and lib.eprecon_conv_desc_takes_bn_acc(ctypes.byref(d)):
        acc = aff if aff is not None else AccSlice.new(cout)
        assert acc.c == cout
        d.bn_acc, d.bn_acc_ld, d.bn_acc_c0 = acc.block.data_ptr(), acc.ld, acc.c0
        d.bn_gamma, d.bn_beta = _dptr(gamma), _dptr(beta)
        _lib.check(lib.eprecon_conv_desc_async(ctypes.byref(d), _lib.current_stream()), "eprecon_conv_desc_async")
        return Act(out, relu=relu, acc=acc, eps=eps)
    if aff is None:
        a = torch.empty((2, cout), dtype=torch.float32, device=dev)
        aff = (a[0], a[1])
    assert not isinstance(aff, AccSlice), "an accumulator slice was handed to a launch that cannot produce into it"
    partial = SP.bn_summaries(lib.eprecon_conv_desc_partial_rows(ctypes.byref(d)), cout, dev)
    nblk, ld = SP.summary_layout(partial)
    d.bn_partial, d.bn_ld = partial.data_ptr(), ld
    _lib.check(lib.eprecon_conv_desc_async(ctypes.byref(d), _lib.current_stream()), "eprecon_conv_desc_async")
    _lib.check(lib.eprecon_batchnorm_finalize_affine_async(
        partial.data_ptr(), nblk, ld, cout, _dptr(gamma), _dptr(beta), float(eps),
        aff[0].data_ptr(), aff[1].data_ptr(), _lib.current_stream()), "eprecon_batchnorm_finalize_affine_async")
    return Act(out, aff[0], aff[1], relu)


def materialize(act, out=None):
    if act.scale is None and act.acc is None:
        if out is not None and out.data_ptr() != act.rows.data_ptr():
            out.copy_(act.rows)
            return out
        return act.rows
    rows = act.rows
    n, c = rows.shape
    if out is None:
        out = torch.empty((n, c), dtype=torch.float32, device=rows.device)
    if act.scale is None and c <= 512:
        _lib.check(_lib.load().eprecon_affine_rows_acc_async(
            rows.data_ptr(), n, c, rows.stride(0), act.acc.block.data_ptr(), act.acc.ld, act.acc.c0, float(act.eps), int(act.relu),
            out.data_ptr(), out.stride(0), _lib.current_stream()), "eprecon_affine_rows_acc_async")
        return out
    act.affine()
    _lib.check(_lib.load().eprecon_affine_rows_async(
        rows.data_ptr(), n, c, rows.stride(0), act.scale.data_ptr(), act.shift.data_ptr(), int(act.relu),
        out.data_ptr(), out.stride(0), _lib.current_stream()), "eprecon_affine_rows_async")
    return out


def conv_bn(conv, bn, x, grid, out=None, relu=True, pre_relu=False, pre_residual=None):
    res = Act(pre_residual) if pre_residual is not None else None
    return materialize(conv_bn_act(conv, bn, Act(x), grid, relu=relu, pre_relu=pre_relu, residual=res), out=out)
```

### eprecon_amd/modules.py

```python
import math

import torch
import torch.nn as nn
import torch.nn.functional as F

from . import autograd as AG
from . import dense2d as D2
from . import sparse as SP


def recording():
    return torch.is_grad_enabled()

_SET_CACHE = []
_SET_CACHE_MAX = 8
_SET_CACHE_LOCK = __import__("threading").Lock()


def voxel_set_for(coords, stride=1):
    key = (coords.data_ptr(), coords.shape[0], coords._version, int(stride), coords.device)
    with _SET_CACHE_LOCK:
        for k, ref, vs in _SET_CACHE:
            if k == key and ref is coords:
                return vs
# ... 105 lines not shown
class Spares3dELAN(nn.Module):

    def __init__(self, dim):
        super().__init__()
        h = dim // 2
        self.conv1 = SubMconv3dBlock(dim, dim, 1, 1, 0)
        self.conv2 = SubMconv3dBlock(dim, dim, 1, 1, 0)
        self.conv3 = SubMconv3dBlock(dim, h, 3, 1, 1)
        self.conv4 = SubMconv3dBlock(h, h, 3, 1, 1)
        self.conv5 = SubMconv3dBlock(h, h, 3, 1, 1)
        self.conv6 = SubMconv3dBlock(h, h, 3, 1, 1)
        self.conv7 = SubMconv3dBlock(dim * 4, dim, 1, 1, 0)
        self.dim = dim

    def run(self, x, vset):
        d, h = self.dim, self.dim // 2
        n = x.shape[0]
        if recording():
            x1, x2 = self.conv1.run(x, vset), self.conv2.run(x, vset)
            x3 = self.conv3.run(x2, vset)
            x4 = self.conv4.run(x3, vset)
            x5 = self.conv5.run(x4, vset)
            x6 = self.conv6.run(x5, vset)
            return self.conv7.run(torch.cat([x1, x2, x3, x4, x5, x6], dim=1), vset)
        cat = torch.empty((n, 4 * d), dtype=torch.float32, device=x.device)
        self.conv1.run(x, vset, out=cat[:, 0:d])
        self.conv2.run(x, vset, out=cat[:, d:2 * d])
        self.conv3.run(cat[:, d:2 * d], vset, out=cat[:, 2 * d:2 * d + h])
        self.conv4.run(cat[:, 2 * d:2 * d + h], vset, out=cat[:, 2 * d + h:3 * d])
        self.conv5.run(cat[:, 2 * d + h:3 * d], vset, out=cat[:, 3 * d:3 * d + h])
        self.conv6.run(cat[:, 3 * d:3 * d + h], vset, out=cat[:, 3 * d + h:4 * d])
        return self.conv7.run(cat, vset)

    def forward(self, voxel_features_o, voxel_coords_bxyz, batch_size, spitial_shape):
        return self.run(voxel_features_o.contiguous(), voxel_set_for(voxel_coords_bxyz))


class SparseConv3d_Residual(nn.Module):

    def __init__(self, dim, Kernel):
        super().__init__()
        self.SConv3d = SparseSubMConv3d(dim, dim, Kernel)
        self.norm = _RowLayerNorm(dim)

    def run(self, x, vset):
        return self.SConv3d.run_ln(x, vset, self.norm, relu=True, residual=x)

    def forward(self, x, coords, spitial_shape, bs):
        return self.run(x.contiguous(), voxel_set_for(coords))


class TrainBatchNorm1d(nn.BatchNorm1d):

    def run(self, x, residual=None, relu=False, out=None):
        if recording():
            y = F.batch_norm(x, self.running_mean, self.running_var, self.weight, self.bias, True, self.momentum, self.eps)
            y = y + residual if residual is not None else y
            y = F.relu(y) if relu else y
            return y if out is None else out.copy_(y)
        return SP.batchnorm_train(x, self.weight, self.bias, self.eps, residual, relu, out)

    def run_partials(self, x, partial, residual=None, relu=False, out=None):
        return SP.batchnorm_apply_partials(x, partial, self.weight, self.bias, self.eps, residual, relu, out)

    def pending_affine(self, partial):
        return SP.bn_affine(partial, self.weight, self.bias, self.eps)


def _rows(x):
    n, c, h, w = x.shape
    return x.permute(0, 2, 3, 1).reshape(n * h * w, c)


def _hip_bn_ok(x):
    return (x.is_cuda and not torch.is_grad_enabled() and x.dim() == 4 and x.shape[1] <= 256
            and x.is_contiguous(memory_format=torch.channels_last) and x.dtype == torch.float32)


def bn2d_train(bn, x, relu=False):
    if _hip_bn_ok(x):
        rows = _rows(x)
        SP.batchnorm_train(rows, bn.weight, bn.bias, bn.eps, relu=relu, out=rows)
        return x
    y = bn(x)
    return F.relu(y) if relu else y


def upsample2x_bilinear(x):
    if x.is_cuda and not torch.is_grad_enabled() and x.shape[1] % 4 == 0 and x.dtype == torch.float32 \
            and x.is_contiguous(memory_format=torch.channels_last):
        from . import _lib
        n, c, h, w = x.shape
        out = torch.empty((n, c, 2 * h, 2 * w), dtype=x.dtype, device=x.device,
                          memory_format=torch.channels_last)
        _lib.check(_lib.load().eprecon_upsample2x_nhwc_async(_lib.ptr(x), _lib.ptr(out), n, h, w, c,
                                                             _lib.current_stream()), "eprecon_upsample2x_nhwc_async")
        return out
    return F.interpolate(x, scale_factor=2, mode="bilinear")
class Conv2d_Block(nn.Module):

    def __init__(self, C_in, C_out, Kernel):
        super().__init__()
        self.conv = nn.Conv2d(C_in, C_out, Kernel, padding="same")
        self.bn = nn.BatchNorm2d(C_out)
        self.act = nn.ReLU()

    def forward(self, x):
        return bn2d_train(self.bn, self.conv(x), relu=True)

    def run_act(self, x, grid, out=None, aff=None):
        return D2.conv_bn_act(self.conv, self.bn, x, grid, out=out, aff=aff, relu=True)

    def run_rows(self, x, grid, out=None):
        return D2.materialize(self.run_act(D2.Act(x), grid), out=out)


class Conv2d_Residual_Block(nn.Module):

    def __init__(self, C, Kernel):
        super().__init__()
        self.conv = nn.Conv2d(C, C, Kernel, padding="same")
        self.bn = nn.BatchNorm2d(C)
        self.relu = nn.ReLU()

    def forward(self, x):
        return bn2d_train(self.bn, x + self.relu(self.conv(x)))

    def run_act(self, x, grid):
        return D2.conv_bn_act(self.conv, self.bn, x, grid, relu=False, pre_relu=True, residual=x)

    def run_rows(self, x, grid, out=None):
        return D2.materialize(self.run_act(D2.Act(x), grid), out=out)


class ELAN(nn.Module):

    def __init__(self, dim):
        super().__init__()
        h = dim // 2
        self.conv1 = Conv2d_Block(dim, dim, 1)
        self.conv2 = Conv2d_Block(dim, dim, 1)
        self.conv3 = Conv2d_Block(dim, h, 3)
        self.conv4 = Conv2d_Block(h, h, 3)
        self.conv5 = Conv2d_Block(h, h, 3)
        self.conv6 = Conv2d_Block(h, h, 3)
        self.conv7 = Conv2d_Block(dim * 4, dim, 1)

    def forward(self, x):
        parts = [self.conv1(x), self.conv2(x)]
        for layer in (self.conv3, self.conv4, self.conv5, self.conv6):
            parts.append(layer(parts[-1]))
        return self.conv7(torch.cat(parts, dim=1))

    def run_act(self, x, grid):
        d = x.rows.shape[1]
        h = d // 2
        dev = x.rows.device
        cat = torch.empty((x.rows.shape[0], 4 * d), dtype=torch.float32, device=dev)
        if D2._ARENA is not None:
            acc = D2.AccSlice.new(4 * d)
            eps = self.conv1.bn.eps
            part = lambda a, b: D2.Act(cat[:, a:b], relu=True, acc=acc.part(a, b), eps=eps)
            sl = lambda a, b: dict(out=cat[:, a:b], aff=acc.part(a, b))
        else:
            aff = torch.empty((2, 4 * d), dtype=torch.float32, device=dev)
            part = lambda a, b: D2.Act(cat[:, a:b], aff[0, a:b], aff[1, a:b], True)
            sl = lambda a, b: dict(out=cat[:, a:b], aff=(aff[0, a:b], aff[1, a:b]))
        self.conv1.run_act(x, grid, **sl(0, d))
        self.conv2.run_act(x, grid, **sl(d, 2 * d))
        self.conv3.run_act(part(d, 2 * d), grid, **sl(2 * d, 2 * d + h))
        self.conv4.run_act(part(2 * d, 2 * d + h), grid, **sl(2 * d + h, 3 * d))
        self.conv5.run_act(part(2 * d + h, 3 * d), grid, **sl(3 * d, 3 * d + h))
        self.conv6.run_act(part(3 * d, 3 * d + h), grid, **sl(3 * d + h, 4 * d))
        return self.conv7.run_act(part(0, 4 * d), grid)

    def run_rows(self, x, grid, out=None):
        return D2.materialize(self.run_act(D2.Act(x), grid), out=out)


class Fusion_Block(nn.Module):

    def __init__(self, C):
        super().__init__()
        self.conv1 = nn.Conv2d(C, C, 3, padding="same")
        self.bn1 = nn.BatchNorm2d(C)
        self.relu = nn.ReLU()
        self.conv2 = nn.Conv2d(C, C, 1, padding="same")
        self.bn2 = nn.BatchNorm2d(C)
        self.ELAN = ELAN(C)

    def forward(self, x):
        x = bn2d_train(self.bn1, self.conv1(x), relu=True)
        x = bn2d_train(self.bn2, self.conv2(x), relu=True)
        return self.ELAN(x)

    def run_rows(self, x, grid, out=None):
        a = D2.conv_bn_act(self.conv1, self.bn1, D2.Act(x), grid, relu=True)
        a = D2.conv_bn_act(self.conv2, self.bn2, a, grid, relu=True)
        return D2.materialize(self.ELAN.run_act(a, grid), out=out)


def _ln_rows(norm, y, residual=None, pre_relu=False, post_relu=False):
    if y.is_cuda and not torch.is_grad_enabled() and y.dim() == 2 and y.dtype == torch.float32 and y.is_contiguous() \
            and (residual is None or (residual.is_contiguous() and residual.dtype == torch.float32)):
        return SP.rowwise_layernorm(y, norm.weight, norm.bias, norm.eps, residual, pre_relu, post_relu, out=y)
    t = F.relu(y) if pre_relu else y
    if residual is not None:
        t = t + residual
    t = norm(t)
    return F.relu(t) if post_relu else t


_FUSED_HEADS = __import__("os").environ.get("EPRECON_FUSED_HEADS", "1") == "1"


def fused_heads_ok(mod, x):
    return (_FUSED_HEADS and not torch.is_grad_enabled() and x.is_cuda and x.dim() == 2 and x.dtype == torch.float32
            and x.stride(1) == 1 and x.shape[1] == mod.linear1.in_features
            and SP.mlp4x_supported(mod.linear1.in_features, mod.linear3.out_features))


def linear4x_pair(mod_a, mod_b, x):
    if fused_heads_ok(mod_a, x) and mod_a.linear3.out_features == mod_b.linear3.out_features \
            and mod_a.linear1.in_features == mod_b.linear1.in_features:
        ya, yb = SP.mlp4x([mod_a, mod_b], x)
        return ya, yb
    return mod_a(x), mod_b(x)


class Linear4xTrans(nn.Module):

    def __init__(self, C_in, C_out):
        super().__init__()
        self.linear1 = nn.Linear(C_in, C_in * 4)
        self.norm1 = nn.LayerNorm(C_in * 4)
        self.relu = nn.ReLU()
        self.linear2 = nn.Linear(C_in * 4, C_in)
        self.norm2 = nn.LayerNorm(C_in)
        self.linear3 = nn.Linear(C_in, C_out)
        self.use_residual = C_in == C_out
        for lin in (self.linear1, self.linear2, self.linear3):
            nn.init.xavier_uniform_(lin.weight)
            nn.init.zeros_(lin.bias)

    def forward(self, x):
        if recording() and x.is_cuda and x.dim() == 2 and x.dtype == torch.float32:
            lin = lambda layer, t: AG.sparse_conv(t, layer.weight.t(), None, layer.bias)
        else:
            lin = lambda layer, t: layer(t)
        if fused_heads_ok(self, x):
            return SP.mlp4x([self], x)[0]
        h = _ln_rows(self.norm1, lin(self.linear1, x), post_relu=True)
        h = _ln_rows(self.norm2, lin(self.linear2, h), post_relu=True)
        y = lin(self.linear3, h)
        return y + h if self.use_residual else y


class Linear_Residual(nn.Module):

    def __init__(self, dim):
        super().__init__()
        self.linear = nn.Linear(dim, dim)
        self.activation = nn.ReLU()
        self.norm = nn.LayerNorm(dim)

    def forward(self, x):
        return _ln_rows(self.norm, self.linear(x), residual=x, pre_relu=True)


class Panoptic_Feat_Fusion(nn.Module):

    def __init__(self, self_channel, panoptic_channel, ch_initialization):
        super().__init__()
        self.img2panoptic_0 = nn.Linear(ch_initialization[2], panoptic_channel)
        self.occ2panoptic_0 = nn.Linear(self_channel, panoptic_channel)
        self.pre_fusion = nn.Linear(panoptic_channel * 2, panoptic_channel)
        self.pre_fusion_0 = Linear_Residual(panoptic_channel)
        self.pre_fusion_1 = Linear_Residual(panoptic_channel)
        self.mask_feat_extraction_0 = SparseConv3d_Residual(panoptic_channel, 3)
        self.mask_feat_extraction_1 = SparseConv3d_Residual(panoptic_channel, 3)
        self.mask_feat_extraction_2 = SparseConv3d_Residual(panoptic_channel, 3)

    def generate_mask_features(self, panoptic_feats, coords_b, coords_xyz, batch_size, spitial_shape):
        coords = torch.cat([coords_b.unsqueeze(1), coords_xyz], dim=1).to(torch.int32).contiguous()
        vset = SP.VoxelSet(coords, 1)
        x = panoptic_feats.contiguous()
        for layer in (self.mask_feat_extraction_0, self.mask_feat_extraction_1, self.mask_feat_extraction_2):
            x = layer.run(x, vset)
        return x


from .tensor import PointTensor, SparseTensor
from .torchsparse_utils import devoxelize_gate, initial_voxelize, point_to_voxel, voxel_to_point

__all__ = ["SPVCNN", "SConv3d", "ConvGRU"]


def _linear_wt(lin):
    hit = getattr(lin, "_wt_cache", None)
    tag = (lin.weight._version, lin.weight.data_ptr())
    if hit is None or hit[0] != tag or hit[1].device != lin.weight.device:
        hit = (tag, lin.weight.detach().t().contiguous())
        lin._wt_cache = hit
    return hit[1]


class Conv3d(nn.Module):

    def __init__(self, inc, outc, kernel_size=3, stride=1, dilation=1, transposed=False):
        super().__init__()
        assert dilation == 1 and (kernel_size, stride) in ((1, 1), (3, 1), (2, 2))
        self.kernel_size, self.stride, self.transposed = kernel_size, stride, transposed
        kvol = kernel_size ** 3
        shape = (inc, outc) if kvol == 1 else (kvol, inc, outc)
        self.kernel = nn.Parameter(torch.empty(shape))
        std = 1.0 / math.sqrt((outc if transposed else inc) * kvol)
        with torch.no_grad():
            self.kernel.uniform_(-std, std)

    def run(self, feats, nbr, out=None):
        if recording():
            y = AG.sparse_conv(feats, self.kernel, nbr)
            return y if out is None else out.copy_(y)
        return SP.sparse_conv(feats, self.kernel, nbr, None, out=out)

    def run_stats(self, feats, nbr, out=None, in_affine=None):
        return SP.conv_stats(feats, self.kernel, nbr, in_affine=in_affine, out=out)


class BasicConvolutionBlock(nn.Module):

    def __init__(self, inc, outc, ks=3, stride=1, dilation=1):
        super().__init__()
        self.net = nn.Sequential(Conv3d(inc, outc, ks, stride, dilation), TrainBatchNorm1d(outc), nn.ReLU(True))

    def run(self, feats, nbr, out=None):
        if recording():
            return self.net[1].run(self.net[0].run(feats, nbr), relu=True)
        y, partial = self.net[0].run_stats(feats, nbr, out=out)
        return self.net[1].run_partials(y, partial, relu=True, out=y)


class BasicDeconvolutionBlock(nn.Module):

    def __init__(self, inc, outc, ks=3, stride=1):
        super().__init__()
        self.net = nn.Sequential(Conv3d(inc, outc, ks, stride, transposed=True), TrainBatchNorm1d(outc),
                                 nn.ReLU(True))

    def run(self, feats, nbr, out=None):
        if recording():
            return self.net[1].run(self.net[0].run(feats, nbr), relu=True)
# ... 315 lines not shown
```

### eprecon_amd/occupancy_initialization.py

```python
import os

import torch
import torch.nn as nn
import torch.nn.functional as F

from . import _lib
from . import back_project as BP
from .back_project import Back_Project, get_img_feats
from . import dense2d as D2
from . import sparse as SP
from .config import INIT_MIN_VALID
from .modules import (Conv2d_Block, Conv2d_Residual_Block, Fusion_Block, SparseSubMConv3d, Spares3dELAN,
                      TrainBatchNorm1d, _RowLayerNorm, upsample2x_bilinear)


class Occupancy_Initialization(nn.Module):
    def __init__(self, ch_initialization_all, ch_initialization_down, n_views):
        super().__init__()
        ch_all = sum(ch_initialization_all[:3])
        d = ch_initialization_down
        self.self_fusion_1x = Fusion_Block(ch_initialization_all[0])
        self.self_fusion_2x = Fusion_Block(ch_initialization_all[1])
        self.self_fusion_4x = Fusion_Block(ch_initialization_all[2])
        self.pool4x = nn.AvgPool2d(2)
        self.fusion_down = Conv2d_Block(ch_all, d, 1)
        self.post_fusion_1 = Conv2d_Residual_Block(d, 3)
        self.post_fusion_2 = Conv2d_Residual_Block(d, 3)
        self.post_fusion_3 = Conv2d_Residual_Block(d, 3)
        self.post_fusion_4 = Conv2d_Residual_Block(d, 3)

        self.similary_1 = Spares3dELAN(d)
        self.norm0 = TrainBatchNorm1d(d)
        self.subm1 = SparseSubMConv3d(d, d, 3)
        self.norm1 = _RowLayerNorm(d)
        self.subm2 = SparseSubMConv3d(d, d, 3)
        self.norm2 = _RowLayerNorm(d)
        self.subm3 = SparseSubMConv3d(d, d, 3)
        self.norm3 = _RowLayerNorm(d)
        self.subm4 = SparseSubMConv3d(d, 1, 3)
        self.norm4 = TrainBatchNorm1d(1)
        self.use_hip_graph = os.environ.get("EPRECON_NO_GRAPH", "0") != "1"
        self._graphs = {}
        self.use_hip_conv = os.environ.get("EPRECON_MIOPEN_CONV2D", "0") != "1"
        self._channels_last = False
        self._side_streams = None
        self._bn_arena = None

    def feat_fusion_pre(self, feats_1x, feats_2x, feats_4x):
        if feats_1x.is_cuda and not torch.is_grad_enabled() and self.use_hip_conv:
            return self._feat_fusion_rows(feats_1x, feats_2x, feats_4x)
        if feats_1x.is_cuda and not torch.is_grad_enabled():
            if not self._channels_last:
                for mod in (self.self_fusion_1x, self.self_fusion_2x, self.self_fusion_4x, self.fusion_down,
                            self.post_fusion_1, self.post_fusion_2, self.post_fusion_3, self.post_fusion_4):
                    mod.to(memory_format=torch.channels_last)
                self._channels_last = True
            feats_1x, feats_2x, feats_4x = (t.contiguous(memory_format=torch.channels_last)
                                            for t in (feats_1x, feats_2x, feats_4x))
        f1 = upsample2x_bilinear(self.self_fusion_1x(feats_1x))
        f2 = self.self_fusion_2x(feats_2x)
        f4 = self.pool4x(self.self_fusion_4x(feats_4x))
        x = self.fusion_down(torch.cat([f1, f2, f4], dim=1))
        for blk in (self.post_fusion_1, self.post_fusion_2, self.post_fusion_3, self.post_fusion_4):
            x = blk(x)
        return x

    def _feat_fusion_rows(self, feats_1x, feats_2x, feats_4x):
        return self._fusion_on_rows([D2.rows_of(t.float().contiguous(memory_format=torch.channels_last))
                                     for t in (feats_1x, feats_2x, feats_4x)], [tuple(t.shape) for t in (feats_1x, feats_2x, feats_4x)])

    def _fusion_on_rows(self, rows, shapes):
        dev = rows[0].device
        grids = [D2.PixelGrid.get(v, h, w, dev) for v, c, h, w in shapes]
        g1, g2, g4 = grids
        c1, c2, c4 = (r.shape[1] for r in rows)
        cat = torch.empty((g2.n, c1 + c2 + c4), dtype=torch.float32, device=dev)
        main = torch.cuda.current_stream()
        if self._side_streams is None:
            self._side_streams = (_lib.side_stream(dev, _lib.SIDE_BRANCH_A), _lib.side_stream(dev, _lib.SIDE_BRANCH_B))
        s1, s4 = self._side_streams
        if D2.BN_ACC and self._bn_arena is None:
            self._bn_arena = D2.BnArena(dev)
        with D2.bn_pass(self._bn_arena if D2.BN_ACC else None):
            s1.wait_stream(main)
            s4.wait_stream(main)
            with torch.cuda.stream(s4):
                f4 = self.self_fusion_4x.run_rows(rows[2], g4)
                cat[:, c1 + c2:] = D2.rows_of(self.pool4x(D2.maps_of(f4, g4.maps, g4.height, g4.width)))
            with torch.cuda.stream(s1):
                f1 = self.self_fusion_1x.run_rows(rows[0], g1)
                up = upsample2x_bilinear(D2.maps_of(f1, g1.maps, g1.height, g1.width))
                cat[:, 0:c1] = D2.rows_of(up)
            self.self_fusion_2x.run_rows(rows[1], g2, out=cat[:, c1:c1 + c2])
            main.wait_stream(s1)
            main.wait_stream(s4)
            a = self.fusion_down.run_act(D2.Act(cat), g2)
            for blk in (self.post_fusion_1, self.post_fusion_2, self.post_fusion_3, self.post_fusion_4):
                a = blk.run_act(a, g2)
            return D2.maps_of(D2.materialize(a), g2.maps, g2.height, g2.width)

    def _fusion_graphed(self, views):
        key = tuple(tuple(v[0].shape) + (len(v),) for v in views) + (views[0][0].device,)
        direct = self.use_hip_conv and len(views[0]) <= 16 and all(
            m.dtype == torch.float32 and m.is_contiguous() for v in views for m in v)
        key = key + (direct,)
        entry = self._graphs.get(key)
        if entry is None:
            shapes = [(len(v),) + tuple(v[0].shape) for v in views]
            if direct:
                static_in = [torch.empty((n * h * w, c), dtype=torch.float32, device=views[0][0].device) for n, c, h, w in shapes]
                self._views_to_rows(views, static_in)
                run = lambda: self._fusion_on_rows(static_in, shapes)
            else:
                static_in = [torch.stack(v) for v in views]
                run = lambda: self.feat_fusion_pre(*static_in)
            side = _lib.side_stream(static_in[0].device, _lib.SIDE_SETUP)
            side.wait_stream(torch.cuda.current_stream())
            with torch.cuda.stream(side):
                for _ in range(3):
                    run()
            torch.cuda.current_stream().wait_stream(side)
            graph = torch.cuda.CUDAGraph()
            with torch.cuda.graph(graph, capture_error_mode="thread_local"):
                static_out = run()
            entry = (graph, static_in, static_out)
            self._graphs[key] = entry
        graph, static_in, static_out = entry
        if direct:
            self._views_to_rows(views, static_in)
        else:
            for s_, v in zip(static_in, views):
                torch.stack(v, out=s_)
        graph.replay()
        return static_out

    @staticmethod
    def _views_to_rows(views, rows):
        import ctypes
        d = _lib.ViewsDesc()
        d.levels, d.n_views = len(views), len(views[0])
        for l, (v, r) in enumerate(zip(views, rows)):
            c, h, w = v[0].shape
            d.channels[l], d.hw[l], d.dst[l] = c, h * w, r.data_ptr()
            for i, m in enumerate(v):
                d.src[l][i] = m.data_ptr()
        _lib.check(_lib.load().eprecon_views_to_rows_async(ctypes.byref(d), _lib.current_stream()), "eprecon_views_to_rows_async")

    def sparse_stack(self, var, vset):
        x = self.norm0.run(var)
        x = self.similary_1.run(x, vset)
        for conv, norm in ((self.subm1, self.norm1), (self.subm2, self.norm2), (self.subm3, self.norm3)):
            x = conv.run_ln(x, vset, norm, relu=True, residual=x)
        if torch.is_grad_enabled():
            return self.norm4.run(self.subm4.run(x, vset))
        y, partial = self.subm4.run_stats(x, vset)
        return self.norm4.run_partials(y, partial, out=y)

    def forward(self, coords, origin, voxel_size, features_all, KRcam, shape, stage, min_view_number, between=None):
        bs = features_all[0][0].shape[0]
        dev = features_all[0][0].device
        graphed = self.use_hip_graph and not torch.is_grad_enabled() and dev.type == "cuda"
        per_batch = []
        for b in range(bs):
            views = [[f[l][b] for f in features_all] for l in (2, 1, 0)]
            if graphed:
                fused_b = self._fusion_graphed(views)
                per_batch.append(fused_b if bs == 1 else fused_b.clone())
            else:
                per_batch.append(self.feat_fusion_pre(*[torch.stack(v) for v in views]))
        fused = per_batch[0].unsqueeze(1) if bs == 1 else torch.stack(per_batch, dim=1)
        if between is not None and dev.type == "cuda" and not torch.is_grad_enabled():
            pend = BP.run_async(coords, origin, voxel_size, fused, KRcam, min_view_number, BP.MODE_VARIANCE,
                                min_valid_per_batch=INIT_MIN_VALID, want_mean=True)
            between()
            res = pend.result()
            if res is not None:
                res["var"] = res.pop("feats")
        else:
            res = BP.view_variance(coords, origin, voxel_size, fused, KRcam, min_view_number,
                                   min_valid=INIT_MIN_VALID)
        if res is None:
            return None
        interval = 2 ** (2 - stage)
        coord_valid = res["coords"]
        parts = []
        start = 0
        self.dense_checks = []
        for b in range(bs):
            nb = res["n_valid_per_batch"][b]
            seg = slice(start, start + nb)
            vset = SP.VoxelSet(coord_valid[seg], interval, dims=shape)
            parts.append(self.sparse_stack(res["var"][seg], vset))
            start += nb
        occ = parts[0] if bs == 1 else torch.cat(parts)
        out_coords = coord_valid if coords.dtype == torch.int32 else coord_valid.to(coords.dtype)
        return [occ, out_coords, res["count"]]
```

### eprecon_amd/sparse.py

```python
import ctypes

import torch

from . import _lib


import os

def _dense3d_level():
    return int(os.environ.get("EPRECON_CONV_DENSE3D", "2"))


def _ld(t):
    assert t.dim() == 2 and t.stride(1) == 1, "row-major 2-D tensor expected"
    return t.stride(0)


class HashGrid:

    def __init__(self, n, device):
        lib = _lib.load()
        self.capacity = int(lib.eprecon_hash_capacity(int(n)))
        self.mem = torch.empty(int(lib.eprecon_hash_table_bytes(self.capacity)), dtype=torch.uint8,
                               device=device)
# ... 111 lines not shown
            return 0
        if cout == 1 and not ln:
            return 1
        if level < 2 or accumulate:
            return 0
        if cout <= 32 and cin % 16 == 0 and not (ln and stats):
            return 2
        return 0

    def takes(self, x, cin, cout, accumulate=False, ln=False, stats=False):
        return self.kind(x, cin, cout, accumulate, ln, stats) != 0


_PACK_REGISTRY = {}
_PACK_TABLE = {"key": None, "jobs": None, "entries": None}


def _register_pack(owner, kind, shape, source_ptr):
    import weakref
    if source_ptr != owner.data_ptr():
        return
    slot = _PACK_REGISTRY.setdefault(id(owner), {})
    if kind not in slot or slot[kind][0]() is not owner or slot[kind][1] != tuple(shape):
        slot[kind] = (weakref.ref(owner), tuple(shape))
        _PACK_TABLE["key"] = None


def repack_registered():
    import numpy as np
    entries = []
    for oid in list(_PACK_REGISTRY):
        slot = _PACK_REGISTRY[oid]
        for kind in list(slot):
            ref, shape = slot[kind]
            owner = ref()
            hit = getattr(owner, "_d3_pack" if kind == 0 else "_d3_pack16", None) if owner is not None else None
            if owner is None or hit is None or not owner.is_cuda or (kind == 1 and hit[0][2] != shape):
                del slot[kind]
                _PACK_TABLE["key"] = None
                continue
            entries.append((owner, kind, shape, hit[1]))
        if not slot:
            del _PACK_REGISTRY[oid]
    stale = [e for e in entries if (e[0]._version, e[0].data_ptr()) != getattr(e[0], "_d3_pack" if e[1] == 0 else "_d3_pack16")[0][:2]]
    if not stale:
        return 0
    key = tuple((o.data_ptr(), k, s, p.data_ptr()) for o, k, s, p in stale)
    if _PACK_TABLE["key"] != key:
        job = np.zeros(len(stale), dtype=np.dtype([("weight", "<u8"), ("packed", "<u8"), ("kvol", "<i4"), ("cin", "<i4"),
                                                   ("cout", "<i4"), ("kind", "<i4")]))
        for i, (o, k, s, p) in enumerate(stale):
            job[i] = (o.data_ptr(), p.data_ptr(), s[0], s[1], s[2], k)
        _PACK_TABLE["jobs"] = torch.from_numpy(job.view(np.uint8).copy()).to(stale[0][0].device)
        _PACK_TABLE["key"] = key
    lib = _lib.load()
    _lib.check(lib.eprecon_conv_pack_many_async(_lib.ptr(_PACK_TABLE["jobs"]), len(stale), _lib.current_stream()),
               "eprecon_conv_pack_many_async")
    for o, k, s, p in stale:
        if k == 0:
            o._d3_pack = ((o._version, o.data_ptr()), p)
        else:
            o._d3_pack16 = ((o._version, o.data_ptr(), s), p)
    return len(stale)


def packed_weight(weight):
    hit = getattr(weight, "_d3_pack", None)
    tag = (weight._version, weight.data_ptr())
    if hit is None or hit[0] != tag or hit[1].device != weight.device:
        lib = _lib.load()
        kvol, cin, cout = weight.shape
        w = weight.detach().contiguous()
        packed = torch.empty(int(lib.eprecon_conv_pack_weight_floats(kvol, cin, cout)), dtype=torch.float32, device=weight.device)
        _lib.check(lib.eprecon_conv_pack_weight_async(_lib.ptr(w), kvol, cin, cout, _lib.ptr(packed), _lib.current_stream()),
                   "eprecon_conv_pack_weight_async")
        hit = (tag, packed)
        weight._d3_pack = hit
        _register_pack(weight, 0, (kvol, cin, cout), w.data_ptr())
    return hit[1]


def packed_weight16(weight, owner=None):
    owner = weight if owner is None else owner
    hit = getattr(owner, "_d3_pack16", None)
    tag = (owner._version, owner.data_ptr(), tuple(weight.shape))
    if hit is None or hit[0] != tag or hit[1].device != weight.device:
        lib = _lib.load()
        kvol, cin, cout = weight.shape
        w = weight.detach().contiguous()
        packed = torch.empty(int(lib.eprecon_conv_pack_weight16_floats(kvol, cin, cout)), dtype=torch.float32, device=weight.device)
        _lib.check(lib.eprecon_conv_pack_weight16_async(_lib.ptr(w), kvol, cin, cout, _lib.ptr(packed), _lib.current_stream()),
                   "eprecon_conv_pack_weight16_async")
        hit = (tag, packed)
        owner._d3_pack16 = hit
        _register_pack(owner, 1, (kvol, cin, cout), w.data_ptr())
    return hit[1]


def voxel_hierarchy(vox, levels=3, points=None):
    n = vox.shape[0]
    summary = torch.empty(2 * levels, dtype=torch.int32, device=vox.device)
    uniqs, invs, grids = unique_hierarchy_queued(vox, levels, summary=summary)
    host = _lib.read_counts(summary)
    sizes = []
    for lvl in range(levels):
        check_hash_status(host[2 * lvl])
        sizes.append(host[2 * lvl + 1])
    if points is not None and levels == 3 and n > 0 and sizes[0] > 0:
        return _hierarchy_with_geometry(vox, points, grids, uniqs, invs, sizes)
    base = VoxelSet(uniqs[0][:sizes[0]], 1, grid=grids[0])
    cur = base
    for lvl in range(1, levels):
        coarse, _, _ = cur.downsample(pre=(uniqs[lvl][:sizes[lvl]], invs[lvl][:sizes[lvl - 1]], grids[lvl]))
        cur = coarse
    return (base, invs[0]) if points is None else (base, invs[0], None)


def _hierarchy_with_geometry(vox, points, grids, uniqs, invs, sizes):
    lib = _lib.load()
    dev = vox.device
    n = vox.shape[0]
    n1, n2, n4 = sizes
    c1, c2, c4 = uniqs[0][:n1], uniqs[1][:n2], uniqs[2][:n4]
    i32 = lambda *shape: torch.empty(shape, dtype=torch.int32, device=dev)
    t = {"offsets1": i32(n1 + 1), "order1": i32(n), "idx4": i32(n), "offsets4": i32(n4 + 1), "order4": i32(n),
         "down12": i32(8, n2), "up21": i32(8, n1), "down24": i32(8, n4), "up42": i32(8, n2),
         "k1": i32(27, n1), "k2": i32(27, n2), "k4": i32(27, n4), "idx8_1": i32(n, 8), "idx8_4": i32(n, 8),
         "weight8_1": torch.empty((n, 8), dtype=torch.float32, device=dev),
         "weight8_4": torch.empty((n, 8), dtype=torch.float32, device=dev)}
    d = _lib.SpvcnnGeometryDesc()
    d.n, d.n1, d.n2, d.n4 = n, n1, n2, n4
    d.scaled, d.vox, d.inverse1 = points.data_ptr(), vox.data_ptr(), invs[0].data_ptr()
    d.coords1, d.coords2, d.coords4 = c1.data_ptr(), c2.data_ptr(), c4.data_ptr()
    d.parent2, d.parent4 = invs[1].data_ptr(), invs[2].data_ptr()
    d.table1, d.table2, d.table4 = (g.mem.data_ptr() for g in grids)
    d.capacity1, d.capacity2, d.capacity4 = (g.capacity for g in grids)
    for name, buf in t.items():
        setattr(d, name, buf.data_ptr())
    ws = _lib.workspace(lib.eprecon_spvcnn_geometry_workspace_bytes(n, n1, n4), dev)
    d.workspace, d.workspace_bytes = ws.data_ptr(), ws.numel()
    _lib.check(lib.eprecon_spvcnn_geometry_async(ctypes.byref(d), _lib.current_stream()), "eprecon_spvcnn_geometry_async")
    s1, s2, s4 = VoxelSet(c1, 1, grid=grids[0]), VoxelSet(c2, 2, grid=grids[1]), VoxelSet(c4, 4, grid=grids[2])
    s1._k3, s2._k3, s4._k3 = t["k1"], t["k2"], t["k4"]
    s1._down, s2._down = (s2, t["down12"], t["up21"]), (s4, t["down24"], t["up42"])
    return s1, invs[0], t


def clear_packed_weights(module):
    for p_ in module.parameters():
        for attr in ("_d3_pack", "_d3_pack16"):
            if hasattr(p_, attr):
                delattr(p_, attr)
    for m in module.modules():
        for attr in ("_wt_cache", "_eprecon_packed", "_eprecon_merged", "_native", "_native_params"):
            if hasattr(m, attr):
                delattr(m, attr)


K1_DIRECT_MIN_ROWS = 20000


def _resolve_map(nbr, x, weight, desc, accumulate=False, ln=False, stats=False, owner=None):
    if isinstance(nbr, DenseMap):
        kvol, cin, cout = weight.shape
        kind = nbr.kind(x, cin, cout, accumulate, ln, stats) if kvol == 27 else 0
        if kind:
            desc.vox_rank = nbr.rank.data_ptr()
            desc.grid_x, desc.grid_y, desc.grid_z = nbr.dims
            keep = [nbr.rank]
            if kind == 2:
                pw = packed_weight16(weight)
                desc.packed_weight16 = pw.data_ptr()
                keep.append(pw)
            desc.nbr = None
            return keep
        nbr = nbr.vset.kernel_map(3)
    desc.nbr = None if nbr is None else nbr.data_ptr()
    keep = [nbr]
    if nbr is None and weight.shape[0] == 1 and weight.shape[2] <= DIRECT_MAX_COUT and not accumulate and x.is_cuda \
            and x.shape[0] >= K1_DIRECT_MIN_ROWS:
        pw = packed_weight16(weight, owner)
        desc.packed_weight16 = pw.data_ptr()
        keep.append(pw)
    if nbr is not None and weight.shape[0] == 27 and weight.shape[2] <= DIRECT_MAX_COUT \
            and not accumulate and x.is_cuda:
        pw = packed_weight16(weight)
        desc.packed_weight16 = pw.data_ptr()
        keep.append(pw)
    if nbr is not None and weight.shape[0] == 27 and not accumulate and x.is_cuda:
        pw = packed_weight(weight)
        desc.packed_weight = pw.data_ptr()
        keep.append(pw)
    return keep


class VoxelSet:

    def __init__(self, coords, stride=1, grid=None, dims=None):
        assert coords.dtype == torch.int32 and coords.dim() == 2 and coords.shape[1] == 4
        self.coords = coords.contiguous()
        self.stride = int(stride)
        self.dims = None if dims is None else tuple(int(d) for d in dims)
        self._grid = grid
        self._k3 = None
        self._down = None
        self._dense = None

    def conv_map(self, ksize=3):
        assert ksize == 3
        if self.dims is not None and self.n >= DENSE_MIN_FILL * self.dims[0] * self.dims[1] * self.dims[2] \
                and _dense3d_level() > 0 and self.coords.is_cuda:
            if self._dense is None:
                self._dense = DenseMap(self, self.dims)
            return self._dense
        return self.kernel_map(3)

    @property
    def n(self):
        return self.coords.shape[0]

    @property
    def grid(self):
        if self._grid is None:
            self._grid = HashGrid(self.n, self.coords.device).build(self.coords)
        return self._grid

    def kernel_map(self, ksize=3):
        assert ksize == 3
        if self._k3 is None:
            lib = _lib.load()
            nbr = torch.empty((27, self.n), dtype=torch.int32, device=self.coords.device)
            _lib.check(lib.eprecon_kernel_map_async(_lib.ptr(self.grid.mem), self.grid.capacity,
                                                    _lib.ptr(self.coords), self.n, 3, self.stride,
                                                    _lib.ptr(nbr), _lib.current_stream()),
                       "eprecon_kernel_map_async")
            self._k3 = nbr
        return self._k3

    def downsample(self, pre=None):
        if self._down is None:
            lib = _lib.load()
            q = 2 * self.stride
            uniq, parent, cgrid = pre if pre is not None else unique_coords(self.coords, quantum=q)
            coarse = VoxelSet(uniq, q, grid=cgrid)
            m = coarse.n
            down = torch.empty((8, m), dtype=torch.int32, device=self.coords.device)
            _lib.check(lib.eprecon_kernel_map_async(_lib.ptr(self.grid.mem), self.grid.capacity,
                                                    _lib.ptr(coarse.coords), m, 2, self.stride,
                                                    _lib.ptr(down), _lib.current_stream()),
                       "eprecon_kernel_map_async")
            up = torch.empty((8, self.n), dtype=torch.int32, device=self.coords.device)
            _lib.check(lib.eprecon_transpose_map_async(_lib.ptr(self.coords), self.n, _lib.ptr(parent),
                                                       self.stride, _lib.ptr(up), _lib.current_stream()),
                       "eprecon_transpose_map_async")
            self._down = (coarse, down, up)
        return self._down


def _attach_workspace(desc, device):
    need = int(_lib.load().eprecon_conv_desc_workspace_bytes(ctypes.byref(desc)))
    if not need:
        return None
    ws = _lib.workspace(need, device)
    desc.workspace, desc.workspace_bytes = ws.data_ptr(), ws.numel()
    return ws


def sparse_conv(x, weight, nbr=None, bias=None, out=None, relu=False, accumulate=False):
    lib = _lib.load()
    w_owner = weight
    if weight.dim() == 2:
        weight = weight.unsqueeze(0)
    kvol, cin, cout = weight.shape
    weight = weight.contiguous()
    n_out = x.shape[0] if nbr is None else nbr.shape[1]
    assert x.shape[1] == cin and x.dtype == torch.float32
    if isinstance(nbr, DenseMap) or (kvol == 27 and nbr is not None and x.is_cuda) or \
            (kvol == 1 and nbr is None and x.is_cuda and cout <= DIRECT_MAX_COUT and not accumulate and n_out >= K1_DIRECT_MIN_ROWS):
        return sparse_conv_fused(x, w_owner, nbr, bias, out, relu, None, accumulate)[0]
    if nbr is not None:
        assert nbr.dtype == torch.int32 and nbr.shape[0] == kvol and nbr.is_contiguous()
    if out is None:
        out = torch.empty((n_out, cout), dtype=torch.float32, device=x.device)
    assert out.shape == (n_out, cout)
    _lib.check(lib.eprecon_sparse_conv_async(_lib.ptr(x), x.shape[0], _ld(x), _lib.ptr(nbr), kvol, n_out,
                                             _lib.ptr(weight), cin, cout, _lib.ptr(bias), _lib.ptr(out),
                                             _ld(out), int(relu), int(accumulate), _lib.current_stream()),
               "eprecon_sparse_conv_async")
    return out


def bn_summaries(rows, cout, device):
    return torch.empty((3, cout, max(int(rows), 1)), dtype=torch.float32, device=device).permute(2, 0, 1)


def summary_layout(partial):
    nblk, three, c = partial.shape
    s0, s1, s2 = partial.stride()
    assert three == 3 and partial.dtype == torch.float32 and s0 == 1 and s2 >= nblk and s1 == c * s2, \
        "BatchNorm summaries must be the channel-major view bn_summaries() returns"
    return nblk, s2


def sparse_conv_fused(x, weight, nbr=None, bias=None, out=None, relu=False, residual=None, accumulate=False,
                      bn_partial=False):
    lib = _lib.load()
    w_owner = weight
# ... 244 lines not shown
```

### include/eprecon_hip.h

```cpp
#ifndef EPRECON_HIP_H
#define EPRECON_HIP_H

#include <stddef.h>
#include <stdint.h>

#ifdef __cplusplus
extern "C" {
#endif

#define EPRECON_OK 0
#define EPRECON_EMPTY 1
#define EPRECON_ERR_ARG (-1)
#define EPRECON_ERR_WORKSPACE (-2)
#define EPRECON_ERR_UNSUPPORTED (-3)
#define EPRECON_ERR_HIP_BASE (-1000)

#define EPRECON_ABI_VERSION 1
int eprecon_abi_version(void);
const char *eprecon_build_arch(void);

#define EPRECON_BP_MEAN 0
#define EPRECON_BP_MEAN_DEPTH 1
#define EPRECON_BP_VARIANCE 2

#define EPRECON_LAYOUT_NCHW 0
#define EPRECON_LAYOUT_NHWC 1

size_t eprecon_back_project_workspace_bytes(int64_t n, int batch, int n_views, int channels,
                                            int height, int width, int feats_layout);

int eprecon_back_project_async(const int32_t *coords, int64_t n, const float *origin, int batch,
                               float voxel_size, const float *feats, int feats_layout,
                               const float *krcam, int n_views, int channels, int height,
                               int width, int min_view, int mode, float *out_feats,
                               float *out_mean, int32_t *out_coords, float *count,
                               float *out_grid, uint8_t *out_mask, int32_t *n_valid_dev,
                               void *workspace, size_t workspace_bytes, void *stream);

int eprecon_back_project(const int32_t *coords, int64_t n, const float *origin, int batch,
                         float voxel_size, const float *feats, int feats_layout,
                         const float *krcam, int n_views, int channels, int height, int width,
                         int min_view, int mode, int min_valid_per_batch, float *out_feats,
                         float *out_mean, int32_t *out_coords, float *count, float *out_grid,
                         uint8_t *out_mask, int32_t *n_valid_dev, int32_t *n_valid_host,
                         void *workspace, size_t workspace_bytes, void *stream);

int eprecon_profile_enable(int on);
float eprecon_profile_gather_ms(void);
const char *eprecon_profile_gather_kernel(void);

int eprecon_profile_conv_arm(int kvol, int cin, int cout, int64_t min_rows);
float eprecon_profile_conv_ms(int64_t *rows_out, const char **kernel_out);
int64_t eprecon_profile_conv_pairs(void);
int64_t eprecon_profile_conv_executed_pairs(void);
const char *eprecon_profile_last_conv_kernel(void);
int eprecon_profile_mark_async(int id, void *stream);

int eprecon_nchw_to_nhwc_async(const float *in, float *out, int maps, int channels, int hw,
                               void *stream);
typedef struct eprecon_views_desc {
    const float *src[3][16];
    float *dst[3];
    int32_t channels[3]; int32_t hw[3];
    int32_t levels; int32_t n_views;
} eprecon_views_desc;
int eprecon_views_to_rows_async(const eprecon_views_desc *desc, void *stream);

uint32_t eprecon_hash_capacity(int64_t n);
size_t eprecon_hash_table_bytes(uint32_t capacity);
int eprecon_hash_build_async(const int32_t *coords, int64_t n, int quantum, void *table,
                             uint32_t capacity, void *stream);
int eprecon_hash_build_dn_async(const int32_t *coords, int64_t n_cap, const int32_t *n_dev, int quantum, void *table,
                                uint32_t capacity, void *stream);
int eprecon_hash_query_async(const void *table, uint32_t capacity, const int32_t *queries, int64_t m,
                             int quantum, int32_t *out_index, void *stream);
int eprecon_hash_status(const void *table, void *stream);

size_t eprecon_unique_workspace_bytes(int64_t n);
int eprecon_exclusive_scan_async(const int32_t *in, int64_t n, int32_t *out, int32_t *total, int32_t *scratch, void *stream);
int eprecon_unique_coords_async(const int32_t *coords, int64_t n, int quantum, void *table,
                                uint32_t capacity, int32_t *inverse, int32_t *unique_coords,
                                int32_t *n_unique_dev, void *workspace, size_t workspace_bytes,
                                void *stream);

int eprecon_unique_coords_dn_async(const int32_t *coords, int64_t n_cap, const int32_t *n_dev, int quantum, void *table,
                                   uint32_t capacity, int32_t *inverse, int32_t *unique_coords, int32_t *n_unique_dev,
                                   void *workspace, size_t workspace_bytes, void *stream);
int eprecon_unique_hierarchy_dn_async(const int32_t *coords, int64_t n_cap, const int32_t *n_dev, int levels, void *const *tables,
                                      const uint32_t *capacities, int32_t *const *inverse, int32_t *const *unique_coords,
                                      int32_t *summary, void *workspace, size_t workspace_bytes, void *stream);

int eprecon_kernel_map_self_async(const void *table, uint32_t capacity, const int32_t *coords, int64_t n, int stride, int32_t *nbr,
                                  void *stream);
int eprecon_kernel_map_async(const void *table, uint32_t capacity, const int32_t *coords, int64_t n,
                             int ksize, int stride, int32_t *nbr, void *stream);
int eprecon_transpose_map_async(const int32_t *fine_coords, int64_t n, const int32_t *parent,
                                int fine_stride, int32_t *up_map, void *stream);
int eprecon_sparse_conv_async(const float *x, int64_t n_in, int ld_x, const int32_t *nbr, int kvol,
                              int64_t n_out, const float *weight, int cin, int cout, const float *bias,
                              float *out, int ld_out, int relu, int accumulate, void *stream);
size_t eprecon_conv_bn_partial_bytes(int64_t n_out, int cout);
int eprecon_sparse_conv_fused_async(const float *x, int64_t n_in, int ld_x, const int32_t *nbr, int kvol,
                                    int64_t n_out, const float *weight, int cin, int cout,
                                    const float *bias, const float *residual, int ld_res, float *out,
                                    int ld_out, int relu, int accumulate, float *bn_partial, void *stream);
typedef struct eprecon_conv_desc {
    const float *x; int64_t n_in; int ld_x;
    const int32_t *nbr; int kvol; int64_t n_out;
    const float *weight; int cin; int cout;
    const float *bias;
    const float *residual; int ld_res;
    float *out; int ld_out;
    int relu; int accumulate;
    const float *in_scale; const float *in_shift; int in_relu;
    const float *res_scale; const float *res_shift; int res_relu;
    float *bn_partial; int bn_ld;
    int ln; const float *ln_gamma; const float *ln_beta; float ln_eps; int ln_post_relu;
    int img_h; int img_w; int img_maps;
    const int32_t *vox_rank; int grid_x; int grid_y; int grid_z;
    const float *packed_weight;
    const float *packed_weight16;
    void *workspace; size_t workspace_bytes;
    long long *bn_acc; int bn_acc_ld; int bn_acc_c0; const float *bn_gamma; const float *bn_beta;
    const long long *in_acc; int in_acc_ld; int in_acc_c0; float in_eps; float *in_affine_scratch;
} eprecon_conv_desc;
size_t eprecon_bn_acc_words(int ld);
int eprecon_conv_desc_takes_bn_acc(const eprecon_conv_desc *desc);
int eprecon_batchnorm_acc_affine_async(const long long *acc, int acc_ld, int acc_c0, int channels, float eps, float *scale_out,
                                       float *shift_out, void *stream);
int eprecon_affine_rows_acc_async(const float *x, int64_t n, int channels, int ld_x, const long long *acc, int acc_ld, int acc_c0,
                                  float eps, int relu, float *out, int ld_out, void *stream);
int eprecon_conv_desc_async(const eprecon_conv_desc *desc, void *stream);
size_t eprecon_conv_desc_workspace_bytes(const eprecon_conv_desc *desc);
int64_t eprecon_conv_desc_partial_rows(const eprecon_conv_desc *desc);
int eprecon_batchnorm_finalize_affine_async(const float *partial, int64_t nblk, int64_t ld, int channels, const float *gamma,
                                            const float *beta, float eps, float *scale_out, float *shift_out,
                                            void *stream);
int eprecon_affine_rows_async(const float *x, int64_t n, int channels, int ld_x, const float *scale,
                              const float *shift, int relu, float *out, int ld_out, void *stream);
int eprecon_affine_rows_res_async(const float *x, int64_t n, int channels, int ld_x, const float *scale,
                                  const float *shift, const float *residual, int ld_res, int relu, float *out,
                                  int ld_out, void *stream);
int eprecon_pixel_map_async(int maps, int height, int width, int ksize, int32_t *nbr, void *stream);
int eprecon_grid_rank_async(const int32_t *coords, int64_t n, int stride, int grid_x, int grid_y, int grid_z, int32_t *rank,
                            void *stream);
size_t eprecon_conv_pack_weight_floats(int kvol, int cin, int cout);
int eprecon_conv_pack_weight_async(const float *weight, int kvol, int cin, int cout, float *packed, void *stream);
size_t eprecon_conv_pack_weight16_floats(int kvol, int cin, int cout);
int eprecon_conv_pack_weight16_async(const float *weight, int kvol, int cin, int cout, float *packed, void *stream);
typedef struct eprecon_pack_job {
    const float *weight; float *packed;
    int32_t kvol; int32_t cin; int32_t cout; int32_t kind;
} eprecon_pack_job;
int eprecon_conv_pack_many_async(const eprecon_pack_job *jobs, int njobs, void *stream);

size_t eprecon_batchnorm_workspace_bytes(int64_t n, int channels);
int eprecon_batchnorm_train_async(const float *x, int64_t n, int channels, int ld_x, const float *gamma,
                                  const float *beta, float eps, const float *residual, int ld_res,
                                  int relu, float *out, int ld_out, float *mean_out, float *var_out,
                                  void *workspace, size_t workspace_bytes, void *stream);
size_t eprecon_batchnorm_apply_workspace_bytes(int channels);
int eprecon_batchnorm_apply_partials_async(const float *x, int64_t n, int channels, int ld_x,
                                           const float *partial, int64_t nblk, int64_t ld, const float *gamma,
                                           const float *beta, float eps, const float *residual,
                                           int ld_res, int relu, float *out, int ld_out, float *mean_out,
                                           float *var_out, void *workspace, size_t workspace_bytes,
                                           void *stream);
int eprecon_batchnorm_apply_partials_res_async(const float *x, int64_t n, int channels, int ld_x, const float *partial,
                                               int64_t nblk, int64_t ld, const float *gamma, const float *beta, float eps,
                                               const float *residual, int ld_res, const float *res_scale,
                                               const float *res_shift, int relu, float *out, int ld_out, void *workspace,
                                               size_t workspace_bytes, void *stream);
int eprecon_rowwise_layernorm_async(const float *x, int64_t n, int channels, int ld_x,
                                    const float *residual, int ld_res, const float *gamma,
                                    const float *beta, float eps, int pre_relu, int post_relu,
                                    float *out, int ld_out, void *stream);

size_t eprecon_init_select_workspace_bytes(int batch, int dim);
int eprecon_init_select_async(const float *logit, const int32_t *coords, int64_t n, float threshold,
                              int batch, int dim, int cell, int32_t *out_coords, int32_t *n_out_dev,
                              void *workspace, size_t workspace_bytes, void *stream);
size_t eprecon_sparsify_workspace_bytes(int64_t n);
int eprecon_sparsify_async(const float *occ, int ld_occ, float threshold, const unsigned char *target,
                           const int32_t *coords, const float *tsdf, int ld_tsdf, const float *feat_all, int ld_feat,
                           int c_all, int c_feat, int64_t n, int batch, int32_t *out_coords, float *out_tsdf,
                           float *out_occ, float *out_all, float *out_feat, int32_t *counts, void *workspace,
                           size_t workspace_bytes, void *stream);
int eprecon_upsample_async(const float *feat, int ld_feat, const int32_t *coords, int64_t n, int channels,
                           int interval, float *up_feat, int32_t *up_coords, void *stream);

int eprecon_aligned_coords_async(const int32_t *coords, int64_t n, const float *origin, int batch,
                                 float voxel_size, const float *world_to_aligned_camera, float *out_xyzb,
                                 void *stream);
int eprecon_point_quantize_async(const float *points_xyzb, int64_t n, float resolution, float *scaled_xyzb,
                                 int32_t *voxel_bxyz, void *stream);
int eprecon_spvcnn_points_dn_async(const int32_t *src_coords, int64_t cap_src, const int32_t *n_src_dev, int children,
                                   int interval, const float *origin, int batch, float voxel_size,
                                   const float *world_to_aligned_camera, float resolution, int32_t *up_coords, float *r_coords,
                                   float *scaled_xyzb, int32_t *voxel_bxyz, int32_t *n_points_dev, void *stream);
int eprecon_point_quantize_dn_async(const float *points_xyzb, int64_t n_cap, const int32_t *n_dev, float resolution,
                                    float *scaled_xyzb, int32_t *voxel_bxyz, void *stream);
size_t eprecon_segment_workspace_bytes(int64_t n, int64_t m);
int eprecon_segment_lists_async(const int32_t *idx, int64_t n, int64_t m, int32_t *offsets, int32_t *order,
                                void *workspace, size_t workspace_bytes, void *stream);
int eprecon_segment_mean_async(const float *feat, int ld_feat, const int32_t *offsets, const int32_t *order,
                               int64_t m, int channels, float *out, int ld_out, void *stream);
int eprecon_sphash_async(const int32_t *coords, int64_t n, int64_t *out_hash, void *stream);
size_t eprecon_sphash_order_workspace_bytes(int64_t n);
int eprecon_sphash_order_async(const int32_t *coords, int64_t n, int32_t *perm_out, int32_t *rank_out, void *workspace,
                               size_t workspace_bytes, void *stream);
int eprecon_remap_index_async(const int32_t *idx, int64_t n, const int32_t *rank_old, const int32_t *perm_new,
                              int64_t m_new, int32_t *out, void *stream);
int eprecon_trilinear_map_async(const void *table, uint32_t capacity, const float *points_xyzb, int64_t n,
                                int stride, int32_t *idx8, float *weight8, void *stream);
int eprecon_devoxelize_async(const float *voxel_feat, int ld_feat, const int32_t *idx8, const float *weight8,
                             int64_t n, int channels, float *out, int ld_out, int accumulate, void *stream);

#define EPRECON_GATE_SIGMOID 1
#define EPRECON_GATE_SIGMOID_MUL 2
#define EPRECON_GATE_GRU_MIX 3
int eprecon_devoxelize_gate_async(const float *voxel_feat, int ld_feat, const int32_t *idx8, const float *weight8,
                                  int64_t n, int channels, const float *skip, int ld_skip, int mode, const float *h,
                                  int ld_h, const float *zgate, int ld_z, float *out, int ld_out, void *stream);

int eprecon_devoxelize_gate_tail_async(const float *voxel_feat, int ld_feat, const int32_t *idx8, const float *weight8,
                                       int64_t n, int channels, const float *skip, int ld_skip, int mode, const float *h,
                                       int ld_h, const float *zgate, int ld_z, float *out, int ld_out, const float *tail_src,
                                       int ld_tail_src, float *tail_dst, int ld_tail_dst, int tail_channels, void *stream);

size_t eprecon_fbv_union_workspace_bytes(int dim);
int eprecon_fbv_union_async(const int32_t *cur_coords, const float *cur_feat, int64_t n_cur, int ld_cur,
                            const int32_t *glob_coords, const float *glob_feat, int64_t n_glob, int ld_glob,
                            int channels, int dim, int interval, int activity_mode,
                            const int32_t *relative_origin_host, int32_t *updated, int32_t *src_cur, int32_t *src_glob, uint8_t *glob_valid,
                            int32_t *n_out_dev, void *workspace, size_t workspace_bytes, void *stream);
int eprecon_gather_rows_async(const float *feat, int ld_feat, const int32_t *src, int64_t n, int channels,
                              float fill, float *out, int ld_out, void *stream);

int eprecon_map_create(int channels, void **out_handle);
int eprecon_map_destroy(void *handle);
int eprecon_map_reset(void *handle);
int64_t eprecon_map_size(const void *handle);
int eprecon_map_channels(const void *handle);
int eprecon_map_export_async(const void *handle, int32_t *coords_out, float *feats_out, void *stream);
int eprecon_map_import_async(void *handle, const int32_t *coords, const float *feats, int64_t n, void *stream);
int eprecon_map_crop_union(void *handle, const int32_t *cur_coords, const float *cur_feat, int64_t n_cur, int ld_cur,
                           int dim, int interval, int activity_mode, const int32_t *relative_origin_host,
                           int32_t *updated, int32_t *src_cur, int32_t *src_glob, int64_t *counts_host, void *stream);
int eprecon_map_gather_async(const void *handle, const int32_t *src_glob, int64_t n, int col0, int channels, float fill,
                             float *out, int ld_out, void *stream);
int eprecon_map_update_async(void *handle, const int32_t *updated, int64_t n, const float *values, int ld_values,
                             void *stream);
int eprecon_map_target_fuse(void *handle, const float *tsdf_gt, const uint8_t *occ_gt, int dim,
                            const int32_t *relative_origin_host, const int32_t *updated, int64_t n, float *tsdf_target_out,
                            void *stream);
typedef struct eprecon_gru_stage_desc {
    void *map;
    void *target_map;
    const int32_t *cur_coords;
    const float *cur_feat;
    int64_t n_cur; int ld_cur;
    int dim; int interval; int activity_mode;
    int32_t rel[3];
    const float *tsdf_gt; const uint8_t *occ_gt;
    const float *origin;
    const float *w2ac;
    float voxel_size;
    float resolution;
    int ch_voxel;
    int batch_index;
    int64_t capacity;
    int32_t *updated;
    int32_t *out_coords;
    float *r_coords;
    float *hx_voxel;
    float *hx_image;
    float *tsdf_target;
    float *scaled1; int32_t *vox1; int32_t *inverse1; int32_t *uniq1; void *table1;
    float *scaled2; int32_t *vox2; int32_t *inverse2; int32_t *uniq2; void *table2;
    uint32_t table_capacity;
// ... 26 lines not shown
                                 void *workspace, size_t workspace_bytes, void *stream);
int eprecon_marching_cubes_emit_async(const float *volume, int dx, int dy, int dz, float level, float *verts, float *normals,
                                      int32_t *faces, const int32_t *label_a, const int32_t *label_b, int32_t *vert_label_a,
                                      int32_t *vert_label_b, const void *workspace, void *stream);
int eprecon_marching_cubes_count_masked(const float *volume, const float *weight, int dx, int dy, int dz, float level,
                                        int64_t *counts_host, void *workspace, size_t workspace_bytes, void *stream);
int eprecon_marching_cubes_emit_masked_async(const float *volume, const float *weight, int dx, int dy, int dz, float level,
                                             float *verts, float *normals, int32_t *faces, const int32_t *label_a,
                                             const int32_t *label_b, int32_t *vert_label_a, int32_t *vert_label_b,
                                             const void *workspace, void *stream);

size_t eprecon_render_depth_workspace_bytes(int64_t queue_capacity);
int eprecon_render_depth_async(const float *verts, int64_t n_verts, const int32_t *faces, int64_t n_faces, const double *cams,
                               int n_views, int height, int width, float pixel_center, float znear, float zfar, int cull_back,
                               float *depth_out, int64_t queue_capacity, void *workspace, size_t workspace_bytes, void *stream);

size_t eprecon_depth_metrics_workspace_bytes(int n_frames);
int eprecon_depth_metrics_async(const float *pred, const float *trgt, int n_frames, int64_t n_pix, double *sums_out,
                                void *workspace, size_t workspace_bytes, void *stream);

int eprecon_point_bounds_async(const float *points, int64_t n, float *out, float *workspace, void *stream);

size_t eprecon_voxel_down_sample_workspace_bytes(int64_t n, int64_t slab_cells);
int eprecon_voxel_down_sample(const float *points, int64_t n, const double *min_bound_host, double voxel,
                              const int64_t *dims_host, float *out, int64_t *n_out_host, int64_t slab_cells, void *workspace,
                              size_t workspace_bytes, void *stream);

size_t eprecon_nn_search_workspace_bytes(int64_t n_ref, int64_t n_cells);
int eprecon_nn_search_async(const float *ref, int64_t n_ref, const float *query, int64_t n_query, const double *lo_host,
                            double cell, const int32_t *dims_host, int64_t *idx_out, float *dist_out, void *workspace,
                            size_t workspace_bytes, void *stream);

int eprecon_nearest_voxel_async(const void *table, uint32_t capacity, const int32_t *ref_coords,
                                int64_t m, const int32_t *query_coords, int64_t n, int quantum,
                                int32_t *out_index, void *stream);

int eprecon_decoder_keys_async(const int32_t *coords, int ld_coords, const float *feats, int ld_feats, const float *level_embed,
                               const float *gauss_b, const float *extent_host, int64_t n, int channels, float *src_out,
                               float *keys_out, void *stream);
size_t eprecon_masked_attention_workspace_bytes(int64_t n_keys, int n_queries, int n_heads, int head_dim);
int eprecon_masked_attention_async(const float *q, int q_stride_head, int q_stride_query, const float *k, int ld_k, const float *v, int ld_v, int64_t n_keys,
                                   const float *mask_logits_t, int ld_mask, const int32_t *mask_rows, int64_t n_mask_rows,
                                   int n_queries, int n_heads, int head_dim, float scale, float *out, void *workspace,
                                   size_t workspace_bytes, void *stream);

typedef struct eprecon_decoder_layer_desc {
    int n_queries; int channels; int n_heads; int ffn_dim; int n_class_logits; int mask_hidden;
    const float *o_attn;
    const float *state_in;
    const float *query_pos;
    const float *cross_out_wt; const float *cross_out_b; const float *cross_ln_g; const float *cross_ln_b;
    const float *self_in_wt; const float *self_in_b; const float *self_out_wt; const float *self_out_b;
    const float *self_ln_g; const float *self_ln_b;
    const float *ffn1_wt; const float *ffn1_b; const float *ffn2_wt; const float *ffn2_b; const float *ffn_ln_g; const float *ffn_ln_b;
    const float *dec_ln_g; const float *dec_ln_b; const float *cls_wt; const float *cls_b;
    const float *m1_wt; const float *m1_b; const float *m2_wt; const float *m2_b; const float *m3_wt; const float *m3_b;
    const float *next_q_wt; const float *next_q_b;
    float ln_eps;
    float *state_out;
    float *cls_out;
    float *mask_embed_out;
    float *next_q_out;
    float *workspace;
} eprecon_decoder_layer_desc;
int eprecon_decoder_query_side_async(const eprecon_decoder_layer_desc *desc, void *stream);

int eprecon_panoptic_stats_async(const float *mask_logits, int64_t ld, const float *scores, const int32_t *keep, int n_queries,
                                 int64_t n, int32_t *owner_out, uint8_t *confident_out, int32_t *counts_out, void *stream);
int eprecon_panoptic_assign_async(const int32_t *owner, const uint8_t *confident, const int32_t *idmap, int64_t n, int32_t *seg_out,
                                  void *stream);

typedef struct eprecon_mlp4x_head {
    const float *w1; const float *b1; const float *g1; const float *be1;
    const float *w2; const float *b2; const float *g2; const float *be2;
    const float *w3; const float *b3;
    float *y; int64_t ld_y;
} eprecon_mlp4x_head;
typedef struct eprecon_mlp4x_desc {
    const float *x; int64_t ld_x; int64_t n;
    int channels; int out_channels; int heads; int residual;
    float eps1; float eps2;
    eprecon_mlp4x_head head[2];
} eprecon_mlp4x_desc;
int eprecon_mlp4x_supported(int channels, int out_channels);
int eprecon_mlp4x_async(const eprecon_mlp4x_desc *desc, void *stream);

int eprecon_bn2d_views_chunks(int64_t rows_per_view, int channels);
size_t eprecon_bn2d_views_workspace_bytes(int views, int64_t rows_per_view, int channels);
int eprecon_bn2d_views_stats_async(const float *x, int views, int64_t rows_per_view, int channels, const float *gamma,
                                   const float *beta, float eps, float *affine_out, void *workspace,
                                   size_t workspace_bytes, void *stream);
int eprecon_bn2d_views_apply_async(const float *x, int views, int64_t rows_per_view, int channels, const float *affine, int relu,
                                   const float *residual, float *out, void *stream);
int eprecon_dwconv2d_nhwc_async(const float *x, int n, int height, int width, int channels, const float *weight_taps, int ksize,
                                int stride, const float *affine, int imgs_per_view, int relu, float *out, void *stream);

typedef struct eprecon_gru_finish_desc {
    int64_t n; int64_t m1; int64_t m2;
    const int32_t *inverse1; const int32_t *inverse2;
    const int32_t *uniq1; const int32_t *uniq2;
    const void *table1; const void *table2; uint32_t table_capacity;
    const float *scaled1; const float *scaled2;
    int literal;
    int32_t *offsets1; int32_t *order1; int32_t *offsets2; int32_t *order2;
    int32_t *nbr1; int32_t *nbr2;
    int32_t *idx8_1; float *weight8_1; int32_t *idx8_2; float *weight8_2;
    int32_t *perm1; int32_t *rank1; int32_t *perm2; int32_t *rank2;
    void *workspace; size_t workspace_bytes;
} eprecon_gru_finish_desc;
size_t eprecon_gru_stage_finish_workspace_bytes(int64_t n, int64_t m1, int64_t m2);
int eprecon_gru_stage_finish_async(const eprecon_gru_finish_desc *desc, void *stream);

#define EPRECON_SPVCNN_CONVS 27
typedef struct eprecon_spvcnn_conv {
    const float *weight; const float *packed_weight; const float *packed_weight16;
    int kvol; int cin; int cout;
} eprecon_spvcnn_conv;
typedef struct eprecon_spvcnn_bn {
    const float *gamma; const float *beta; float eps;
} eprecon_spvcnn_bn;
typedef struct eprecon_spvcnn_forward_desc {
    int64_t n, n1, n2, n4;
    int cin; int cs[5];
    const float *feat; int ld_feat;
    const int32_t *offsets1, *order1, *offsets4, *order4;
    const int32_t *k1, *k2, *k4, *down12, *up21, *down24, *up42;
    const int32_t *idx8_1; const float *weight8_1; const int32_t *idx8_4; const float *weight8_4;
    eprecon_spvcnn_conv conv[EPRECON_SPVCNN_CONVS];
    eprecon_spvcnn_bn bn[EPRECON_SPVCNN_CONVS];
    float *out; int ld_out;
    void *workspace; size_t workspace_bytes;
} eprecon_spvcnn_forward_desc;
size_t eprecon_spvcnn_forward_workspace_bytes(const eprecon_spvcnn_forward_desc *desc);
int eprecon_spvcnn_forward_async(const eprecon_spvcnn_forward_desc *desc, void *stream);

typedef struct eprecon_spvcnn_geometry_desc {
    int64_t n; int64_t n1; int64_t n2; int64_t n4;
    const float *scaled; const int32_t *vox; const int32_t *inverse1;
    const int32_t *coords1; const int32_t *coords2; const int32_t *coords4;
    const int32_t *parent2; const int32_t *parent4;
    const void *table1; const void *table2; const void *table4;
    uint32_t capacity1; uint32_t capacity2; uint32_t capacity4;
    int32_t *offsets1; int32_t *order1; int32_t *idx4; int32_t *offsets4; int32_t *order4;
    int32_t *down12; int32_t *up21; int32_t *down24; int32_t *up42;
    int32_t *k1; int32_t *k2; int32_t *k4;
    int32_t *idx8_1; float *weight8_1; int32_t *idx8_4; float *weight8_4;
    void *workspace; size_t workspace_bytes;
} eprecon_spvcnn_geometry_desc;
size_t eprecon_spvcnn_geometry_workspace_bytes(int64_t n, int64_t n1, int64_t n4);
int eprecon_spvcnn_geometry_async(const eprecon_spvcnn_geometry_desc *desc, void *stream);

int eprecon_upsample2x_nhwc_async(const float *in, float *out, int n, int h, int w, int channels,
                                  void *stream);

size_t eprecon_sparse_conv_wgrad_workspace_bytes(int kvol, int64_t n_out, int cin, int cout);
int eprecon_sparse_conv_wgrad_async(const float *x, int ld_x, const float *dy, int ld_dy, const int32_t *nbr, int kvol,
                                    int64_t n_out, int cin, int cout, float *dweight, void *workspace,
                                    size_t workspace_bytes, void *stream);
int eprecon_invert_map_async(const int32_t *nbr, int kvol, int64_t n_out, int64_t n_in, int32_t *inv, void *stream);
int eprecon_devoxelize_backward_async(const float *dout, int ld_out, const int32_t *idx8, const float *weight8, int64_t n,
                                      int channels, int64_t n_voxels, float *dvoxel_feat, int ld_feat, void *stream);
int eprecon_devoxelize_backward_csr_async(const float *dout, int ld_out, const float *weight8, const int32_t *offsets,
                                          const int32_t *order, int64_t n_voxels, int channels, float *dvoxel_feat, int ld_feat,
                                          void *stream);
int eprecon_gather_rows_scaled_async(const float *src, int ld_src, const int32_t *idx, const float *scale, int64_t n,
                                     int channels, float *dst, int ld_dst, void *stream);
int eprecon_back_project_backward_async(const int32_t *coords_valid, int64_t n_valid, const float *origin, int batch,
                                        float voxel_size, const float *feats_nhwc, const float *krcam, int n_views,
                                        int channels, int height, int width, int mode, const float *dout, int ld_dout,
                                        const float *dmean, float *dfeats_nhwc, void *stream);
size_t eprecon_back_project_backward_workspace_bytes(int batch, int n_views, int channels, int height, int width);
int eprecon_back_project_backward_det_async(const int32_t *coords_valid, int64_t n_valid, const float *origin, int batch,
                                            float voxel_size, const float *feats_nhwc, const float *krcam, int n_views,
                                            int channels, int height, int width, int mode, const float *dout, int ld_dout,
                                            const float *dmean, float *dfeats_nhwc, void *workspace, size_t workspace_bytes,
                                            void *stream);

#ifdef __cplusplus
}
#endif
#endif
```

Measured before the change: 715.0.

## Add pointwise-stream 1x1 conv kernel, twin-layer merge, and fused affine pool/upsample joins

Adds a dedicated 1x1 (pointwise) conv kernel that streams rows with a DPP-based BN partial reduction, and routes eligible convs to it ahead of the tiled kernels. In ELAN blocks, conv1 and conv2 read the same input, so their weights are merged and run as one wider launch. The packed-weight limit on cout is raised to allow this. The feature-fusion joins now apply the pending BN affine and ReLU inside new pool2x and upsample2x row kernels, which removes separate materialize passes and intermediate tensors. The cost is extra code paths, extra eligibility checks, and float summation ordering that may differ slightly from before.

Result: faster. 769.1, median of 6 (+7.6%).

```diff
diff --git a/eprecon_amd/_lib.py b/eprecon_amd/_lib.py
--- a/eprecon_amd/_lib.py
+++ b/eprecon_amd/_lib.py
@@ -46,6 +46,7 @@
     "eprecon_conv_desc_partial_rows": (_i64, [_vp]),
     "eprecon_bn_acc_words": (_sz, [_i]),
     "eprecon_conv_desc_takes_bn_acc": (_i, [_vp]),
+    "eprecon_conv_desc_takes_pointwise_stream": (_i, [_vp]),
     "eprecon_batchnorm_acc_affine_async": (_i, [_vp, _i, _i, _i, _f, _vp, _vp, _vp]),
     "eprecon_affine_rows_acc_async": (_i, [_vp, _i64, _i, _i, _vp, _i, _i, _f, _i, _vp, _i, _vp]),
     "eprecon_affine_rows_res_async": (_i, [_vp, _i64, _i, _i, _vp, _vp, _vp, _i, _i, _vp, _i, _vp]),
@@ -126,6 +127,8 @@
     "eprecon_nn_search_async": (_i, [_vp, _i64, _vp, _i64, _vp, _c.c_double, _vp, _vp, _vp, _vp, _sz, _vp]),
     "eprecon_nearest_voxel_async": (_i, [_vp, _c.c_uint32, _vp, _i64, _vp, _i64, _i, _vp, _vp]),
     "eprecon_upsample2x_nhwc_async": (_i, [_vp, _vp, _i, _i, _i, _i, _vp]),
+    "eprecon_affine_pool2x_rows_async": (_i, [_vp, _i, _i, _i, _i, _i, _vp, _vp, _i, _vp, _i, _vp]),
+    "eprecon_affine_upsample2x_rows_async": (_i, [_vp, _i, _i, _i, _i, _i, _vp, _vp, _i, _vp, _i, _vp]),
     "eprecon_decoder_keys_async": (_i, [_vp, _i, _vp, _i, _vp, _vp, _vp, _i64, _i, _vp, _vp, _vp]),
     "eprecon_decoder_query_side_async": (_i, [_vp, _vp]),
     "eprecon_panoptic_stats_async": (_i, [_vp, _i64, _vp, _vp, _i, _i64, _vp, _vp, _vp, _vp]),
@@ -247,7 +250,8 @@
                 ("bn_acc", ctypes.c_void_p), ("bn_acc_ld", ctypes.c_int), ("bn_acc_c0", ctypes.c_int),
                 ("bn_gamma", ctypes.c_void_p), ("bn_beta", ctypes.c_void_p),
                 ("in_acc", ctypes.c_void_p), ("in_acc_ld", ctypes.c_int), ("in_acc_c0", ctypes.c_int),
-                ("in_eps", ctypes.c_float), ("in_affine_scratch", ctypes.c_void_p)]
+                ("in_eps", ctypes.c_float), ("in_affine_scratch", ctypes.c_void_p),
+                ("pointwise_stream", ctypes.c_int)]
 
 
 class GruStageDesc(ctypes.Structure):
diff --git a/eprecon_amd/csrc/conv_common.hpp b/eprecon_amd/csrc/conv_common.hpp
--- a/eprecon_amd/csrc/conv_common.hpp
+++ b/eprecon_amd/csrc/conv_common.hpp
@@ -41,6 +41,7 @@
     const long long *in_acc;
     int in_acc_ld, in_acc_c0;
     float in_eps;
+    int pointwise_stream;
 };
 
 constexpr int kBnCopies = 8, kBnWords = 7;
@@ -124,6 +125,18 @@
 constexpr int kWaves = 4;
 typedef float f32x4 __attribute__((ext_vector_type(4)));
 typedef unsigned int u32x4 __attribute__((ext_vector_type(4)));
+
+__device__ __forceinline__ float relu_nc(float x)
+{
+    float r;
+    asm("v_max_f32 %0, 0, %1" : "=v"(r) : "v"(x));
+    return r;
+}
+__device__ __forceinline__ float relu_sel(float x, unsigned mask)
+{
+    const unsigned r = __float_as_uint(relu_nc(x)), b = __float_as_uint(x);
+    return __uint_as_float((r & mask) | (b & ~mask));
+}
 
 __device__ __forceinline__ void chan_merge(float &n_a, float &mean_a, float &m2_a, float n_b, float mean_b, float m2_b)
 {
@@ -266,5 +279,8 @@
 int64_t tile2d_short_partial_rows(const ConvParams &p);
 int launch_tile2d_short(const ConvParams &p, hipStream_t st);
 
-
-}
+bool pointwise_stream_ok(const ConvParams &p);
+int64_t pointwise_stream_partial_rows(const ConvParams &p);
+int launch_pointwise_stream(const ConvParams &p, hipStream_t st);
+
+}
diff --git a/eprecon_amd/csrc/grid_ops.hip b/eprecon_amd/csrc/grid_ops.hip
--- a/eprecon_amd/csrc/grid_ops.hip
+++ b/eprecon_amd/csrc/grid_ops.hip
@@ -212,6 +212,102 @@
 }
 
 namespace {
+__device__ __forceinline__ float4 affine_quad(const float *p, const float4 sc, const float4 sh, int relu)
+{
+    const float4 v = *reinterpret_cast<const float4 *>(p);
+    float4 a = make_float4(fmaf(v.x, sc.x, sh.x), fmaf(v.y, sc.y, sh.y), fmaf(v.z, sc.z, sh.z), fmaf(v.w, sc.w, sh.w));
+    if (relu) a = make_float4(fmaxf(a.x, 0.0f), fmaxf(a.y, 0.0f), fmaxf(a.z, 0.0f), fmaxf(a.w, 0.0f));
+    return a;
+}
+
+__global__ __launch_bounds__(256) void affine_pool2x_rows_kernel(const float *x, int n, int h, int w, int c4, int ld_x,
+                                                                 const float *scale, const float *shift, int relu, float *out,
+                                                                 int ld_out)
+{
+    const int oh = h / 2, ow = w / 2;
+    const size_t e = (size_t)blockIdx.x * 256 + threadIdx.x;
+    if (e >= (size_t)n * oh * ow * c4) return;
+    const int c = (int)(e % c4);
+    size_t r = e / c4;
+    const int ox = (int)(r % ow), oy = (int)((r / ow) % oh), img = (int)(r / ((size_t)ow * oh));
+    const float4 sc = *reinterpret_cast<const float4 *>(scale + 4 * c), sh = *reinterpret_cast<const float4 *>(shift + 4 * c);
+    const float *p0 = x + (((size_t)img * h + 2 * oy) * w + 2 * ox) * ld_x + 4 * c, *p1 = p0 + (size_t)w * ld_x;
+    const float4 a = affine_quad(p0, sc, sh, relu), b = affine_quad(p0 + ld_x, sc, sh, relu);
+    const float4 d = affine_quad(p1, sc, sh, relu), f = affine_quad(p1 + ld_x, sc, sh, relu);
+    float4 o;
+    o.x = (((0.0f + a.x) + b.x) + d.x + f.x) / 4.0f;
+    o.y = (((0.0f + a.y) + b.y) + d.y + f.y) / 4.0f;
+    o.z = (((0.0f + a.z) + b.z) + d.z + f.z) / 4.0f;
+    o.w = (((0.0f + a.w) + b.w) + d.w + f.w) / 4.0f;
+    *reinterpret_cast<float4 *>(out + r * ld_out + 4 * c) = o;
+}
+
+__global__ __launch_bounds__(256) void affine_upsample2x_rows_kernel(const float *x, int n, int h, int w, int c4, int ld_x,
+                                                                     const float *scale, const float *shift, int relu, float *out,
+                                                                     int ld_out)
+{
+    const size_t e = (size_t)blockIdx.x * 256 + threadIdx.x;
+    if (e >= (size_t)n * 4 * h * w * c4) return;
+    const int c = (int)(e % c4);
+    const size_t row = e / c4;
+    size_t r = row;
+    const int ox = (int)(r % (2 * w));
+    r /= 2 * w;
+    const int oy = (int)(r % (2 * h));
+    const int img = (int)(r / (2 * h));
+    const float sx = fmaxf(((float)ox + 0.5f) * 0.5f - 0.5f, 0.0f);
+    const float sy = fmaxf(((float)oy + 0.5f) * 0.5f - 0.5f, 0.0f);
+    const int x0 = (int)sx, y0 = (int)sy;
+    const int x1 = min(x0 + 1, w - 1), y1 = min(y0 + 1, h - 1);
+    const float lx = sx - (float)x0, ly = sy - (float)y0;
+    const float4 sc = *reinterpret_cast<const float4 *>(scale + 4 * c), sh = *reinterpret_cast<const float4 *>(shift + 4 * c);
+    const float *base = x + (size_t)img * h * w * ld_x + 4 * c;
+    const float4 a = affine_quad(base + ((size_t)y0 * w + x0) * ld_x, sc, sh, relu), b = affine_quad(base + ((size_t)y0 * w + x1) * ld_x, sc, sh, relu);
+    const float4 d = affine_quad(base + ((size_t)y1 * w + x0) * ld_x, sc, sh, relu), f = affine_quad(base + ((size_t)y1 * w + x1) * ld_x, sc, sh, relu);
+    const float w00 = (1.0f - ly) * (1.0f - lx), w01 = (1.0f - ly) * lx, w10 = ly * (1.0f - lx), w11 = ly * lx;
+    float4 o;
+    o.x = w00 * a.x + w01 * b.x + w10 * d.x + w11 * f.x;
+    o.y = w00 * a.y + w01 * b.y + w10 * d.y + w11 * f.y;
+    o.z = w00 * a.z + w01 * b.z + w10 * d.z + w11 * f.z;
+    o.w = w00 * a.w + w01 * b.w + w10 * d.w + w11 * f.w;
+    *reinterpret_cast<float4 *>(out + row * ld_out + 4 * c) = o;
+}
+
+bool join_args_ok(const float *x, int n, int h, int w, int channels, int ld_x, const float *scale, const float *shift,
+                  const float *out, int ld_out)
+{
+    const auto al = [](const void *p) { return (reinterpret_cast<uintptr_t>(p) & 15) == 0; };
+    return x && out && scale && shift && n > 0 && h > 0 && w > 0 && channels > 0 && channels % 4 == 0 && ld_x >= channels &&
+           ld_out >= channels && ld_x % 4 == 0 && ld_out % 4 == 0 && al(x) && al(out) && al(scale) && al(shift);
+}
+}
+
+extern "C" int eprecon_affine_pool2x_rows_async(const float *x, int n, int h, int w, int channels, int ld_x, const float *scale,
+                                                const float *shift, int relu, float *out, int ld_out, void *stream)
+{
+    if (!join_args_ok(x, n, h, w, channels, ld_x, scale, shift, out, ld_out)) return EPRECON_ERR_ARG;
+    const size_t total = (size_t)n * (h / 2) * (w / 2) * (channels / 4);
+    if (total == 0) return EPRECON_OK;
+    if (total > 0x7fffffffull * 256) return EPRECON_ERR_ARG;
+    hipLaunchKernelGGL(affine_pool2x_rows_kernel, dim3((unsigned)ceil_div((int64_t)total, 256)), dim3(256), 0, (hipStream_t)stream, x,
+                       n, h, w, channels / 4, ld_x, scale, shift, relu, out, ld_out);
+    EP_LAUNCH_CHECK();
+    return EPRECON_OK;
+}
+
+extern "C" int eprecon_affine_upsample2x_rows_async(const float *x, int n, int h, int w, int channels, int ld_x, const float *scale,
+                                                    const float *shift, int relu, float *out, int ld_out, void *stream)
+{
+    if (!join_args_ok(x, n, h, w, channels, ld_x, scale, shift, out, ld_out)) return EPRECON_ERR_ARG;
+    const size_t total = (size_t)n * 4 * h * w * (channels / 4);
+    if (total > 0x7fffffffull * 256) return EPRECON_ERR_ARG;
+    hipLaunchKernelGGL(affine_upsample2x_rows_kernel, dim3((unsigned)ceil_div((int64_t)total, 256)), dim3(256), 0, (hipStream_t)stream,
+                       x, n, h, w, channels / 4, ld_x, scale, shift, relu, out, ld_out);
+    EP_LAUNCH_CHECK();
+    return EPRECON_OK;
+}
+
+namespace {
 constexpr int kSpTile = 256;
 constexpr int kSpMaxBatch = 32;
 
diff --git a/eprecon_amd/csrc/sparse_conv.hip b/eprecon_amd/csrc/sparse_conv.hip
--- a/eprecon_amd/csrc/sparse_conv.hip
+++ b/eprecon_amd/csrc/sparse_conv.hip
@@ -1901,6 +1901,10 @@
         }
         if (!p.nbr && p.K != 1) return EPRECON_ERR_ARG;
     }
+    if (pointwise_stream_ok(p)) {
+        g_last_conv_kernel = "spconv_direct16_kernel";
+        return launch_pointwise_stream(p, st);
+    }
     if (tile2d16_ok(p)) {
         g_last_conv_kernel = "conv2d_tile16_kernel";
         return launch_tile2d16(p, st);
@@ -2037,14 +2041,14 @@
 
 extern "C" size_t eprecon_conv_pack_weight16_floats(int kvol, int cin, int cout)
 {
-    if (kvol <= 0 || cin <= 0 || cout <= 0 || cout > 80) return 0;
+    if (kvol <= 0 || cin <= 0 || cout <= 0 || cout > 160) return 0;
     const int rem = cout - 16 * ((cout + 15) / 16 - 1);
     return (size_t)kvol * ((cin + 15) / 16) * ((cout + 15) / 16) * 256 + (rem <= 8 ? (size_t)kvol * ((cin + 15) / 16) * 128 : 0);
 }
 
 extern "C" int eprecon_conv_pack_weight16_async(const float *weight, int kvol, int cin, int cout, float *packed, void *stream)
 {
-    if (!weight || !packed || kvol <= 0 || cin <= 0 || cout <= 0 || cout > 80) return EPRECON_ERR_ARG;
+    if (!weight || !packed || kvol <= 0 || cin <= 0 || cout <= 0 || cout > 160) return EPRECON_ERR_ARG;
     const size_t total = eprecon_conv_pack_weight16_floats(kvol, cin, cout);
     hipLaunchKernelGGL(pack_weights16_kernel, dim3((unsigned)min((size_t)1024, (total + 255) / 256)), dim3(256), 0, (hipStream_t)stream,
                        weight, kvol, cin, cout, (cin + 15) / 16, (cout + 15) / 16, packed);
@@ -2099,6 +2103,7 @@
     p.flex_partial = 1;
     p.bn_acc = d->bn_acc; p.bn_acc_ld = d->bn_acc_ld; p.bn_acc_c0 = d->bn_acc_c0; p.bn_gamma = d->bn_gamma; p.bn_beta = d->bn_beta;
     p.in_acc = d->in_acc; p.in_acc_ld = d->in_acc_ld; p.in_acc_c0 = d->in_acc_c0; p.in_eps = d->in_eps;
+    p.pointwise_stream = d->pointwise_stream;
 }
 
 extern "C" int eprecon_batchnorm_acc_affine_async(const long long *acc, int acc_ld, int acc_c0, int channels, float eps,
@@ -2118,6 +2123,15 @@
     params_from_desc(p, d);
     p.n_out = (int)d->n_out;
     return !p.ln && !p.accumulate && bn_acc_family(p) ? 1 : 0;
+}
+
+extern "C" int eprecon_conv_desc_takes_pointwise_stream(const eprecon_conv_desc *d)
+{
+    if (!d || d->n_out <= 0 || d->n_out > 0x7fffffff || d->n_in != d->n_out) return 0;
+    ConvParams p = {};
+    params_from_desc(p, d);
+    p.n_out = (int)d->n_out;
+    return pointwise_stream_ok(p) ? 1 : 0;
 }
 
 extern "C" int64_t eprecon_conv_desc_partial_rows(const eprecon_conv_desc *d);
@@ -2171,6 +2185,7 @@
     int64_t blocks;
     if (const int kind = conv3d_kind(p)) return d3_tiles_kind(p, kind);
     p.x_bytes = d->n_in > 0 ? ((d->n_in - 1) * (int64_t)p.ld_x + ((p.Cin + 3) & ~3)) * 4 : 0;
+    if (pointwise_stream_ok(p)) return pointwise_stream_partial_rows(p);
     if (tile2d16_ok(p)) return tile2d16_partial_rows(p);
     if (tile2d_short_ok(p)) return tile2d_short_partial_rows(p);
     if (p.K == 9 && direct16_ok(p) && !tile2d_short_list(p)) return ep::ceil_div(d->n_out, (int64_t)direct16_partial_block_rows(p));
diff --git a/eprecon_amd/csrc/sparse_conv_direct_impl.hpp b/eprecon_amd/csrc/sparse_conv_direct_impl.hpp
--- a/eprecon_amd/csrc/sparse_conv_direct_impl.hpp
+++ b/eprecon_amd/csrc/sparse_conv_direct_impl.hpp
@@ -16,18 +16,6 @@
 #ifndef EP_DIRECT_ABL
 #define EP_DIRECT_ABL 0
 #endif
-
-__device__ __forceinline__ float relu_nc(float x)
-{
-    float r;
-    asm("v_max_f32 %0, 0, %1" : "=v"(r) : "v"(x));
-    return r;
-}
-__device__ __forceinline__ float relu_sel(float x, unsigned mask)
-{
-    const unsigned r = __float_as_uint(relu_nc(x)), b = __float_as_uint(x);
-    return __uint_as_float((r & mask) | (b & ~mask));
-}
 
 typedef __bf16 bf16x8 __attribute__((ext_vector_type(8)));
 typedef __bf16 bf16x2 __attribute__((ext_vector_type(2)));
diff --git a/eprecon_amd/csrc/sparse_conv_pointwise.hip b/eprecon_amd/csrc/sparse_conv_pointwise.hip
--- /dev/null
+++ b/eprecon_amd/csrc/sparse_conv_pointwise.hip
@@ -0,0 +1,263 @@
+#include "conv_common.hpp"
+
+namespace epconv {
+
+#ifndef EP_PW_ABL
+#define EP_PW_ABL 0
+#endif
+
+namespace {
+
+constexpr int kPwWaves = 4;
+constexpr int kPwLongRows = 32768;
+
+typedef float f32x2 __attribute__((ext_vector_type(2)));
+
+template <int CTRL>
+__device__ __forceinline__ float row_dpp(float v)
+{
+    return __int_as_float(__builtin_amdgcn_update_dpp(0, __float_as_int(v), CTRL, 0xf, 0xf, false));
+}
+__device__ __forceinline__ float row16_sum(float v)
+{
+    v += row_dpp<0xB1>(v);
+    v += row_dpp<0x4E>(v);
+    v += row_dpp<0x141>(v);
+    v += row_dpp<0x140>(v);
+    return v;
+}
+
+template <int CT, int RT>
+struct PwChunk {
+    f32x4 x[RT];
+    f32x4 sc, sh;
+    f32x4 w[CT];
+};
+
+template <int CT, int KCH, bool T8, bool AFF, int RT>
+__global__ __launch_bounds__(64 * kPwWaves) void spconv_pointwise_kernel(ConvParams p)
+{
+    constexpr int ROWS = 16 * RT * kPwWaves;
+    __shared__ float sStat[kPwWaves * 3 * 16 * CT];
+    const int tid = threadIdx.x, lane = tid & 63, wave = tid >> 6;
+    const int px = lane & 15, q = lane >> 4;
+    const int base = blockIdx.x * ROWS + wave * (16 * RT);
+    if (EP_PW_ABL & 4) {
+        const int c0 = 16 * CT * blockIdx.y, c1 = min(p.Cout, c0 + 16 * CT);
+        for (int r = blockIdx.x * ROWS + (tid >> 4); r < min(p.n_out, (int)(blockIdx.x + 1) * ROWS); r += 16)
+            for (int c = c0 + 4 * (tid & 15); c < c1; c += 64) *reinterpret_cast<f32x4 *>(p.out + (size_t)r * p.ld_out + c) = f32x4{0.0f, 0.0f, 0.0f, 0.0f};
+        if (p.bn_partial && c0 + tid < c1) bn_partial_store(p, blockIdx.x, c0 + tid, 1.0f, 0.0f, 0.0f);
+        return;
+    }
+    int orow[RT];
+    const float *xrow[RT];
+#pragma unroll
+    for (int rt = 0; rt < RT; ++rt) {
+        const int r = base + 16 * rt + px;
+        orow[rt] = r < p.n_out ? r : -1;
+        xrow[rt] = p.x + (size_t)(r < p.n_out ? r : p.n_out - 1) * p.ld_x;
+    }
+    const int t0 = blockIdx.y * CT, ctt = gridDim.y * CT;
+    const f32x4 *wq = reinterpret_cast<const f32x4 *>(p.wq16) + (size_t)t0 * 64 + lane;
+    const unsigned relu_mask = p.in_relu ? 0xffffffffu : 0u;
+
+    f32x4 acc[RT][CT];
+#pragma unroll
+    for (int rt = 0; rt < RT; ++rt)
+#pragma unroll
+        for (int t = 0; t < CT; ++t) acc[rt][t] = f32x4{0.0f, 0.0f, 0.0f, 0.0f};
+
+    auto load = [&](int kc, PwChunk<CT, RT> &c) {
+        const bool t8 = T8 && kc == KCH - 1;
+        const int ch0 = 16 * kc + (t8 ? 2 : 4) * q;
+        const int ch = (kc < KCH - 1 || ch0 < p.Cin) ? ch0 : 0;
+#pragma unroll
+        for (int rt = 0; rt < RT; ++rt) {
+            if (EP_PW_ABL & 2) {
+                c.x[rt] = f32x4{(float)lane, 1.0f, 2.0f, 3.0f};
+            } else if (t8) {
+                const f32x2 v = *reinterpret_cast<const f32x2 *>(xrow[rt] + ch);
+                c.x[rt] = f32x4{v.x, v.y, 0.0f, 0.0f};
+            } else {
+                c.x[rt] = *reinterpret_cast<const f32x4 *>(xrow[rt] + ch);
+            }
+        }
+        if (AFF) {
+            if (t8) {
+                const f32x2 s = *reinterpret_cast<const f32x2 *>(p.in_scale + ch), h = *reinterpret_cast<const f32x2 *>(p.in_shift + ch);
+                c.sc = f32x4{s.x, s.y, 0.0f, 0.0f};
+                c.sh = f32x4{h.x, h.y, 0.0f, 0.0f};
+            } else {
+                c.sc = *reinterpret_cast<const f32x4 *>(p.in_scale + ch);
+                c.sh = *reinterpret_cast<const f32x4 *>(p.in_shift + ch);
+            }
+        }
+#pragma unroll
+        for (int t = 0; t < CT; ++t) c.w[t] = wq[(kc * ctt + t) * 64];
+    };
+    auto consume = [&](int kc, const PwChunk<CT, RT> &c) {
+        const bool t8 = T8 && kc == KCH - 1;
+        constexpr int kFull = 4;
+        const int steps = t8 ? 2 : kFull;
+        const bool cok = kc < KCH - 1 || 16 * kc + (t8 ? 2 : 4) * q < p.Cin;
+        f32x4 a[RT];
+#pragma unroll
+        for (int rt = 0; rt < RT; ++rt) {
+            a[rt] = c.x[rt];
+            if (AFF) {
+#pragma unroll
+                for (int s = 0; s < kFull; ++s)
+                    if (s < steps) a[rt][s] = relu_sel(fmaf(a[rt][s], c.sc[s], c.sh[s]), relu_mask);
+            }
+            if (kc == KCH - 1 && !cok) a[rt] = f32x4{0.0f, 0.0f, 0.0f, 0.0f};
+        }
+#pragma unroll
+        for (int s = 0; s < kFull; ++s) {
+            if (s >= steps) continue;
+#pragma unroll
+            for (int t = 0; t < CT; ++t)
+#pragma unroll
+                for (int rt = 0; rt < RT; ++rt)
+                    acc[rt][t] = __builtin_amdgcn_mfma_f32_16x16x4f32(c.w[t][s], a[rt][s], acc[rt][t], 0, 0, 0);
+        }
+    };
+
+    PwChunk<CT, RT> cur, nxt;
+    load(0, cur);
+#pragma unroll
+    for (int kc = 0; kc < KCH; ++kc) {
+        if (kc + 1 < KCH) load(kc + 1, nxt);
+        consume(kc, cur);
+        if (kc + 1 < KCH) cur = nxt;
+    }
+
+    f32x4 v[RT][CT];
+#pragma unroll
+    for (int t = 0; t < CT; ++t) {
+        const int cb = 16 * (t0 + t) + 4 * q;
+        const bool colok = cb < p.Cout;
+        f32x4 b = {0.0f, 0.0f, 0.0f, 0.0f};
+        if (p.bias && colok) b = f32x4{p.bias[cb], p.bias[cb + 1], p.bias[cb + 2], p.bias[cb + 3]};
+#pragma unroll
+        for (int rt = 0; rt < RT; ++rt) {
+            f32x4 val = acc[rt][t] + b;
+            if (p.relu) {
+#pragma unroll
+                for (int j = 0; j < 4; ++j) val[j] = fmaxf(val[j], 0.0f);
+            }
+            const bool ok = colok && orow[rt] >= 0;
+            v[rt][t] = ok ? val : f32x4{0.0f, 0.0f, 0.0f, 0.0f};
+            if (ok && !(EP_PW_ABL & 1)) *reinterpret_cast<f32x4 *>(p.out + (size_t)orow[rt] * p.ld_out + cb) = val;
+        }
+    }
+    if (EP_PW_ABL & 1) {
+#pragma unroll
+        for (int t = 0; t < CT; ++t)
+#pragma unroll
+            for (int rt = 0; rt < RT; ++rt) asm volatile("" ::"v"(v[rt][t]));
+    }
+
+    if (p.bn_partial || p.bn_acc) {
+        const int live = min(max(p.n_out - base, 0), 16 * RT);
+        const float n = (float)live;
+#pragma unroll
+        for (int t = 0; t < CT; ++t) {
+            f32x4 mean, m2;
+#pragma unroll
+            for (int j = 0; j < 4; ++j) {
+                float s = v[0][t][j];
+#pragma unroll
+                for (int rt = 1; rt < RT; ++rt) s += v[rt][t][j];
+                s = row16_sum(s);
+                const float m = live > 0 ? s / n : 0.0f;
+                float sq = 0.0f;
+#pragma unroll
+                for (int rt = 0; rt < RT; ++rt) {
+                    const float d = orow[rt] >= 0 ? v[rt][t][j] - m : 0.0f;
+                    sq = fmaf(d, d, sq);
+                }
+                mean[j] = m;
+                m2[j] = row16_sum(sq);
+            }
+            if (px == 0) {
+                float *d = sStat + (wave * 3) * 16 * CT + 16 * t + 4 * q;
+#pragma unroll
+                for (int j = 0; j < 4; ++j) { d[j] = n; d[16 * CT + j] = mean[j]; d[2 * 16 * CT + j] = m2[j]; }
+            }
+        }
+        __syncthreads();
+        const int col = 16 * t0 + tid;
+        if (tid < 16 * CT && col < p.Cout) {
+            float a_n = 0.0f, a_mean = 0.0f, a_m2 = 0.0f;
+#pragma unroll
+            for (int w = 0; w < kPwWaves; ++w)
+                chan_merge(a_n, a_mean, a_m2, sStat[(w * 3) * 16 * CT + tid], sStat[(w * 3 + 1) * 16 * CT + tid], sStat[(w * 3 + 2) * 16 * CT + tid]);
+            if (p.bn_partial) bn_partial_store(p, blockIdx.x, col, a_n, a_mean, a_m2);
+            if (p.bn_acc) bn_acc_publish(p, col, blockIdx.x, blockIdx.x == 0, a_n, a_mean, a_m2);
+        }
+    }
+}
+
+#define EP_PW_SHAPES(X) X(2, 1, false) X(2, 2, true) X(2, 6, false) X(3, 3, true) X(3, 10, false) X(2, 9, false) X(5, 5, false) X(5, 20, false) \
+                        X(3, 2, true) X(5, 3, true)
+constexpr int kPwGroupTiles = 5;
+
+struct PwShape { int ct, kch; bool t8; int groups; };
+PwShape pw_shape(const ConvParams &p)
+{
+    const int kch = (p.Cin + 15) / 16, ct = (p.Cout + 15) / 16;
+    const int groups = (ct > kPwGroupTiles && ct % kPwGroupTiles == 0) ? ct / kPwGroupTiles : 1;
+    return {ct / groups, kch, p.Cin - 16 * (kch - 1) <= 8, groups};
+}
+bool pw_shape_built(const PwShape &s)
+{
+#define X(CT, KCH, T8) if (s.ct == CT && s.kch == KCH && s.t8 == T8) return true;
+    EP_PW_SHAPES(X)
+#undef X
+    return false;
+}
+int pw_rows(const ConvParams &p) { return 16 * kPwWaves * (p.n_out >= kPwLongRows ? 2 : 1); }
+
+template <int CT, int KCH, bool T8>
+int launch_pw(const ConvParams &p, int groups, hipStream_t st)
+{
+    const dim3 grid((unsigned)ep::ceil_div(p.n_out, pw_rows(p)), (unsigned)groups), block(64 * kPwWaves);
+    const bool two = p.n_out >= kPwLongRows;
+    if (p.in_scale) {
+        if (two) hipLaunchKernelGGL((spconv_pointwise_kernel<CT, KCH, T8, true, 2>), grid, block, 0, st, p);
+        else hipLaunchKernelGGL((spconv_pointwise_kernel<CT, KCH, T8, true, 1>), grid, block, 0, st, p);
+    } else {
+        if (two) hipLaunchKernelGGL((spconv_pointwise_kernel<CT, KCH, T8, false, 2>), grid, block, 0, st, p);
+        else hipLaunchKernelGGL((spconv_pointwise_kernel<CT, KCH, T8, false, 1>), grid, block, 0, st, p);
+    }
+    EP_LAUNCH_CHECK();
+    return EPRECON_OK;
+}
+
+bool aligned16(const void *ptr) { return (reinterpret_cast<uintptr_t>(ptr) & 15) == 0; }
+
+}
+
+bool pointwise_stream_ok(const ConvParams &p)
+{
+    if (!p.pointwise_stream || p.K != 1 || p.nbr || p.n_out <= 0) return false;
+    if (p.ln || p.accumulate || p.res || p.in_acc) return false;
+    if (!p.wq16 || !aligned16(p.wq16)) return false;
+    if (p.Cin % 4 != 0 || p.Cout % 4 != 0 || p.Cout > 160) return false;
+    if (!aligned16(p.x) || p.ld_x % 4 != 0 || !aligned16(p.out) || p.ld_out % 4 != 0) return false;
+    if (p.in_scale && (!aligned16(p.in_scale) || !aligned16(p.in_shift))) return false;
+    return pw_shape_built(pw_shape(p));
+}
+
+int64_t pointwise_stream_partial_rows(const ConvParams &p) { return ep::ceil_div(p.n_out, pw_rows(p)); }
+
+int launch_pointwise_stream(const ConvParams &p, hipStream_t st)
+{
+    const PwShape s = pw_shape(p);
+#define X(CT, KCH, T8) if (s.ct == CT && s.kch == KCH && s.t8 == T8) return launch_pw<CT, KCH, T8>(p, s.groups, st);
+    EP_PW_SHAPES(X)
+#undef X
+    return EPRECON_ERR_UNSUPPORTED;
+}
+
+}
diff --git a/eprecon_amd/dense2d.py b/eprecon_amd/dense2d.py
--- a/eprecon_amd/dense2d.py
+++ b/eprecon_amd/dense2d.py
@@ -57,10 +57,27 @@
     return cached[1]
 
 
+def twin_layers(owner, a, b):
+    params = [t for conv, bn in (a, b) for t in (conv.weight, conv.bias, bn.weight, bn.bias)]
+    tag = tuple((t._version, t.data_ptr(), str(t.device)) for t in params)
+    cached = getattr(owner, "_eprecon_twin", None)
+    if cached is None or cached[0] != tag:
+        assert a[0].kernel_size == b[0].kernel_size == (1, 1) and a[0].in_channels == b[0].in_channels and a[1].eps == b[1].eps
+        cat = lambda i: torch.cat([params[i].detach(), params[4 + i].detach()]).contiguous()
+        weight = torch.cat([packed_weight(a[0]), packed_weight(b[0])], dim=2).contiguous()
+        cached = (tag, (weight, cat(1), cat(2), cat(3)))
+        owner._eprecon_twin = cached
+    return cached[1]
+
+
 DIRECT_2D_MIN_ROWS = 40000
 K1_DIRECT_2D_MIN_ROWS = 20000
 SHORT_2D_MAX_ROWS = 20000
 SHORT_2D_MAX_COUT = 80
+POINTWISE_STREAM = os.environ.get("EPRECON_CONV_POINTWISE", "1") != "0"
+POINTWISE_MAX_COUT = 160
+TWIN_LAYERS = True
+FUSED_JOINS = True
 
 
 BN_ACC = os.environ.get("EPRECON_BN_ACC", "0") == "1"
@@ -148,6 +165,27 @@
 def conv_bn_act(conv, bn, x, grid, out=None, aff=None, relu=True, pre_relu=False, residual=None):
     return conv_bn_launch(packed_weight(conv), conv.bias, bn.weight, bn.bias, bn.eps, conv.kernel_size[0], x, grid,
                           out=out, aff=aff, relu=relu, pre_relu=pre_relu, residual=residual)
+
+
+def _takes_pointwise_stream(lib, d, w):
+    d.packed_weight16 = SP.packed_weight16(w).data_ptr()
+    d.pointwise_stream = 1
+    if lib.eprecon_conv_desc_takes_pointwise_stream(ctypes.byref(d)):
+        return True
+    d.packed_weight16, d.pointwise_stream = None, 0
+    return False
+
+
+def pointwise_stream_takes(w, x, out):
+    if not POINTWISE_STREAM or w.shape[0] != 1 or w.shape[2] > POINTWISE_MAX_COUT or (x.acc is not None and x.scale is None):
+        return False
+    d = _lib.ConvDesc()
+    d.x, d.n_in, d.ld_x = x.rows.data_ptr(), x.rows.shape[0], x.rows.stride(0)
+    d.kvol, d.n_out = 1, x.rows.shape[0]
+    d.weight, d.cin, d.cout = w.data_ptr(), w.shape[1], w.shape[2]
+    d.out, d.ld_out = out.data_ptr(), out.stride(0)
+    d.in_scale, d.in_shift = _dptr(x.scale), _dptr(x.shift)
+    return _takes_pointwise_stream(_lib.load(), d, w)
 
 
 def conv_bn_launch(w, bias, gamma, beta, eps, k, x, grid, out=None, aff=None, relu=True, pre_relu=False,
@@ -189,6 +227,8 @@
         if cout <= SP.DIRECT_MAX_COUT and n >= DIRECT_2D_MIN_ROWS:
             pw = SP.packed_weight16(w)
             d.packed_weight16 = pw.data_ptr()
+    elif k == 1 and POINTWISE_STREAM and cout <= POINTWISE_MAX_COUT and _takes_pointwise_stream(lib, d, w):
+        pass
     elif k == 1 and cout <= SP.DIRECT_MAX_COUT and n >= K1_DIRECT_2D_MIN_ROWS:
         pw = SP.packed_weight16(w)
         d.packed_weight16 = pw.data_ptr()
@@ -238,3 +278,24 @@
 def conv_bn(conv, bn, x, grid, out=None, relu=True, pre_relu=False, pre_residual=None):
     res = Act(pre_residual) if pre_residual is not None else None
     return materialize(conv_bn_act(conv, bn, Act(x), grid, relu=relu, pre_relu=pre_relu, residual=res), out=out)
+
+
+def _join(entry, act, grid, out):
+    scale, shift = act.affine()
+    assert scale is not None, "the joins take an activation whose BatchNorm is still pending"
+    rows = act.rows
+    assert rows.shape[0] == grid.n and rows.dtype == torch.float32 and rows.stride(1) == 1 and out.stride(1) == 1
+    _lib.check(getattr(_lib.load(), entry)(rows.data_ptr(), grid.maps, grid.height, grid.width, rows.shape[1], rows.stride(0),
+                                           scale.data_ptr(), shift.data_ptr(), int(act.relu), out.data_ptr(), out.stride(0),
+                                           _lib.current_stream()), entry)
+    return out
+
+
+def pool2x_into(act, grid, out):
+    assert out.shape == (grid.maps * (grid.height // 2) * (grid.width // 2), act.rows.shape[1])
+    return _join("eprecon_affine_pool2x_rows_async", act, grid, out)
+
+
+def upsample2x_into(act, grid, out):
+    assert out.shape == (grid.maps * 4 * grid.height * grid.width, act.rows.shape[1])
+    return _join("eprecon_affine_upsample2x_rows_async", act, grid, out)
diff --git a/eprecon_amd/modules.py b/eprecon_amd/modules.py
--- a/eprecon_amd/modules.py
+++ b/eprecon_amd/modules.py
@@ -281,7 +281,7 @@
             parts.append(layer(parts[-1]))
         return self.conv7(torch.cat(parts, dim=1))
 
-    def run_act(self, x, grid):
+    def run_act(self, x, grid, out=None, out_aff=None):
         d = x.rows.shape[1]
         h = d // 2
         dev = x.rows.device
@@ -295,13 +295,23 @@
             aff = torch.empty((2, 4 * d), dtype=torch.float32, device=dev)
             part = lambda a, b: D2.Act(cat[:, a:b], aff[0, a:b], aff[1, a:b], True)
             sl = lambda a, b: dict(out=cat[:, a:b], aff=(aff[0, a:b], aff[1, a:b]))
-        self.conv1.run_act(x, grid, **sl(0, d))
-        self.conv2.run_act(x, grid, **sl(d, 2 * d))
+        twin = None
+        if D2.POINTWISE_STREAM and D2.TWIN_LAYERS and D2._ARENA is None and x.rows.is_cuda \
+                and 2 * d <= D2.POINTWISE_MAX_COUT and self.conv1.bn.eps == self.conv2.bn.eps:
+            twin = D2.twin_layers(self, (self.conv1.conv, self.conv1.bn), (self.conv2.conv, self.conv2.bn))
+            if not D2.pointwise_stream_takes(twin[0], x, cat[:, 0:2 * d]):
+                twin = None
+        if twin is not None:
+            w, bias, gamma, beta = twin
+            D2.conv_bn_launch(w, bias, gamma, beta, self.conv1.bn.eps, 1, x, grid, relu=True, **sl(0, 2 * d))
+        else:
+            self.conv1.run_act(x, grid, **sl(0, d))
+            self.conv2.run_act(x, grid, **sl(d, 2 * d))
         self.conv3.run_act(part(d, 2 * d), grid, **sl(2 * d, 2 * d + h))
         self.conv4.run_act(part(2 * d, 2 * d + h), grid, **sl(2 * d + h, 3 * d))
         self.conv5.run_act(part(2 * d + h, 3 * d), grid, **sl(3 * d, 3 * d + h))
         self.conv6.run_act(part(3 * d, 3 * d + h), grid, **sl(3 * d + h, 4 * d))
-        return self.conv7.run_act(part(0, 4 * d), grid)
+        return self.conv7.run_act(part(0, 4 * d), grid, out=out, aff=out_aff)
 
     def run_rows(self, x, grid, out=None):
         return D2.materialize(self.run_act(D2.Act(x), grid), out=out)
@@ -323,10 +333,13 @@
         x = bn2d_train(self.bn2, self.conv2(x), relu=True)
         return self.ELAN(x)
 
-    def run_rows(self, x, grid, out=None):
+    def run_act(self, x, grid, out=None, aff=None):
         a = D2.conv_bn_act(self.conv1, self.bn1, D2.Act(x), grid, relu=True)
         a = D2.conv_bn_act(self.conv2, self.bn2, a, grid, relu=True)
-        return D2.materialize(self.ELAN.run_act(a, grid), out=out)
+        return self.ELAN.run_act(a, grid, out=out, out_aff=aff)
+
+    def run_rows(self, x, grid, out=None):
+        return D2.materialize(self.run_act(x, grid), out=out)
 
 
 def _ln_rows(norm, y, residual=None, pre_relu=False, post_relu=False):
diff --git a/eprecon_amd/occupancy_initialization.py b/eprecon_amd/occupancy_initialization.py
--- a/eprecon_amd/occupancy_initialization.py
+++ b/eprecon_amd/occupancy_initialization.py
@@ -44,6 +44,7 @@
         self.use_hip_conv = os.environ.get("EPRECON_MIOPEN_CONV2D", "0") != "1"
         self._channels_last = False
         self._side_streams = None
+        self._join_aff = {}
         self._bn_arena = None
 
     def feat_fusion_pre(self, feats_1x, feats_2x, feats_4x):
@@ -84,20 +85,38 @@
         with D2.bn_pass(self._bn_arena if D2.BN_ACC else None):
             s1.wait_stream(main)
             s4.wait_stream(main)
-            with torch.cuda.stream(s4):
-                f4 = self.self_fusion_4x.run_rows(rows[2], g4)
-                cat[:, c1 + c2:] = D2.rows_of(self.pool4x(D2.maps_of(f4, g4.maps, g4.height, g4.width)))
-            with torch.cuda.stream(s1):
-                f1 = self.self_fusion_1x.run_rows(rows[0], g1)
-                up = upsample2x_bilinear(D2.maps_of(f1, g1.maps, g1.height, g1.width))
-                cat[:, 0:c1] = D2.rows_of(up)
-            self.self_fusion_2x.run_rows(rows[1], g2, out=cat[:, c1:c1 + c2])
+            if D2.BN_ACC or not D2.FUSED_JOINS:
+                with torch.cuda.stream(s4):
+                    f4 = self.self_fusion_4x.run_rows(rows[2], g4)
+                    cat[:, c1 + c2:] = D2.rows_of(self.pool4x(D2.maps_of(f4, g4.maps, g4.height, g4.width)))
+                with torch.cuda.stream(s1):
+                    f1 = self.self_fusion_1x.run_rows(rows[0], g1)
+                    up = upsample2x_bilinear(D2.maps_of(f1, g1.maps, g1.height, g1.width))
+                    cat[:, 0:c1] = D2.rows_of(up)
+                self.self_fusion_2x.run_rows(rows[1], g2, out=cat[:, c1:c1 + c2])
+                joined = D2.Act(cat)
+            else:
+                aff = self._join_affine(c1 + c2 + c4, dev)
+                with torch.cuda.stream(s4):
+                    D2.pool2x_into(self.self_fusion_4x.run_act(rows[2], g4), g4, cat[:, c1 + c2:])
+                with torch.cuda.stream(s1):
+                    D2.upsample2x_into(self.self_fusion_1x.run_act(rows[0], g1), g1, cat[:, 0:c1])
+                self.self_fusion_2x.run_act(rows[1], g2, out=cat[:, c1:c1 + c2], aff=(aff[0, c1:c1 + c2], aff[1, c1:c1 + c2]))
+                joined = D2.Act(cat, aff[0], aff[1], True)
             main.wait_stream(s1)
             main.wait_stream(s4)
-            a = self.fusion_down.run_act(D2.Act(cat), g2)
+            a = self.fusion_down.run_act(joined, g2)
             for blk in (self.post_fusion_1, self.post_fusion_2, self.post_fusion_3, self.post_fusion_4):
                 a = blk.run_act(a, g2)
             return D2.maps_of(D2.materialize(a), g2.maps, g2.height, g2.width)
+
+    def _join_affine(self, channels, dev):
+        key = (channels, str(dev))
+        aff = self._join_aff.get(key)
+        if aff is None:
+            aff = self._join_aff[key] = torch.stack([torch.ones(channels, dtype=torch.float32, device=dev),
+                                                     torch.zeros(channels, dtype=torch.float32, device=dev)])
+        return aff
 
     def _fusion_graphed(self, views):
         key = tuple(tuple(v[0].shape) + (len(v),) for v in views) + (views[0][0].device,)
diff --git a/eprecon_amd/sparse.py b/eprecon_amd/sparse.py
--- a/eprecon_amd/sparse.py
+++ b/eprecon_amd/sparse.py
@@ -287,7 +287,7 @@
             if hasattr(p_, attr):
                 delattr(p_, attr)
     for m in module.modules():
-        for attr in ("_wt_cache", "_eprecon_packed", "_eprecon_merged", "_native", "_native_params"):
+        for attr in ("_wt_cache", "_eprecon_packed", "_eprecon_merged", "_eprecon_twin", "_native", "_native_params"):
             if hasattr(m, attr):
                 delattr(m, attr)
 
diff --git a/include/eprecon_hip.h b/include/eprecon_hip.h
--- a/include/eprecon_hip.h
+++ b/include/eprecon_hip.h
@@ -123,9 +123,11 @@
     void *workspace; size_t workspace_bytes;
     long long *bn_acc; int bn_acc_ld; int bn_acc_c0; const float *bn_gamma; const float *bn_beta;
     const long long *in_acc; int in_acc_ld; int in_acc_c0; float in_eps; float *in_affine_scratch;
+    int pointwise_stream;
 } eprecon_conv_desc;
 size_t eprecon_bn_acc_words(int ld);
 int eprecon_conv_desc_takes_bn_acc(const eprecon_conv_desc *desc);
+int eprecon_conv_desc_takes_pointwise_stream(const eprecon_conv_desc *desc);
 int eprecon_batchnorm_acc_affine_async(const long long *acc, int acc_ld, int acc_c0, int channels, float eps, float *scale_out,
                                        float *shift_out, void *stream);
 int eprecon_affine_rows_acc_async(const float *x, int64_t n, int channels, int ld_x, const long long *acc, int acc_ld, int acc_c0,
@@ -458,6 +460,10 @@
 
 int eprecon_upsample2x_nhwc_async(const float *in, float *out, int n, int h, int w, int channels,
                                   void *stream);
+int eprecon_affine_pool2x_rows_async(const float *x, int n, int h, int w, int channels, int ld_x, const float *scale,
+                                     const float *shift, int relu, float *out, int ld_out, void *stream);
+int eprecon_affine_upsample2x_rows_async(const float *x, int n, int h, int w, int channels, int ld_x, const float *scale,
+                                         const float *shift, int relu, float *out, int ld_out, void *stream);
 
 size_t eprecon_sparse_conv_wgrad_workspace_bytes(int kvol, int64_t n_out, int cin, int cout);
 int eprecon_sparse_conv_wgrad_async(const float *x, int ld_x, const float *dy, int ld_dy, const int32_t *nbr, int kvol,
```
